# ESandML/SSL4GIE

Hardware: AMD Instinct MI355X
Metric: images/sec/GPU (fwd+bwd) ViT-B 224² bs=256 at 1/2/4/8 MI355X; % MFMA peak (higher is better)
Workload: dtype bf16; 1 GPU; ViT-B MAE pretrain (mae_vit_base_patch16, norm_pix_loss, mask 0.75) fwd+bwd+grad-allreduce+AdamW, 224x224 synthetic N(0,1) images resident in HBM; batch_per_gpu=256, global_batch=256, parallelism=dp1, optimizer=AdamW(0.9,0.95) wd 0.05 (ssl4gie_amd.optim.ArenaAdamW)

## Files before the change

### include/ssl4gie_hip.h

```cpp
#ifndef SSL4GIE_HIP_H
#define SSL4GIE_HIP_H
#include <stddef.h>
#include <stdint.h>
#ifdef __cplusplus
extern "C" {
#endif

#define SSL4GIE_F32 0
#define SSL4GIE_BF16 1
#define SSL4GIE_EARG 1000
#define SSL4GIE_EPEER 1001

int ssl4gie_abi_version(void);

int ssl4gie_layernorm_fwd(const float* x, const float* gamma, const float* beta, void* y,
                          int y_dtype, float* mean, float* rstd, int rows, int cols, float eps,
                          void* stream);
size_t ssl4gie_layernorm_bwd_workspace_bytes(int rows, int cols);
int ssl4gie_layernorm_bwd(const void* dy, int dy_dtype, const float* x, const float* gamma,
                          const float* mean, const float* rstd, const float* dres, float* dx,
                          void* dx_lp, int lp_dtype, float* dgamma, float* dbeta, int accumulate,
                          float* workspace, int rows, int cols, void* stream);

size_t ssl4gie_colsum_workspace_bytes(int rows, int cols);
int ssl4gie_colsum(const void* x, int dtype, float* out, int accumulate, float* workspace,
                   int rows, int cols, long long ld, void* stream);

enum {
    SSL4GIE_EPI_NONE = 0,
    SSL4GIE_EPI_BIAS = 1,
    SSL4GIE_EPI_BIAS_GELU = 2,
    SSL4GIE_EPI_BIAS_RESIDUAL = 3,
    SSL4GIE_EPI_DGELU = 4,
    SSL4GIE_EPI_BIAS_GELU_GRAD = 5,
    SSL4GIE_EPI_MUL_AUX = 6,
    SSL4GIE_EPI_RELU_MASK_AUX = 7,
    SSL4GIE_EPI_ADD_AUX = 8,
    SSL4GIE_EPI_AFFINE_AUX_RELU = 9
};
typedef struct ssl4gie_conv3x3_geom {
    int B, H, W, C;
    int stride;
    int relu;
} ssl4gie_conv3x3_geom;

typedef struct ssl4gie_gemm_desc {
    int M, N, K;
    int batch1, batch2;
    const void* A;
    long long sAm, sAk, sAb1, sAb2;
    const void* B;
    long long sBk, sBn, sBb1, sBb2;
    void* C;
    long long ldc, sCb1, sCb2;
    int dtype_ab;
    int dtype_c;
    float alpha;
    int epilogue;
    const float* bias;
    const float* residual;
    long long ldr;
    const void* aux;
    void* out2;
    int accumulate;
    float* colsum_a;
    const ssl4gie_conv3x3_geom* conv;
    float* colstats;
    const float* scale;
    int relu;
} ssl4gie_gemm_desc;
size_t ssl4gie_gemm_workspace_bytes(const ssl4gie_gemm_desc* d);
int ssl4gie_gemm(const ssl4gie_gemm_desc* d, void* workspace, size_t workspace_bytes,
                 void* stream);
size_t ssl4gie_gemm_tn_pair_workspace_bytes(const ssl4gie_gemm_desc* a, const ssl4gie_gemm_desc* b);
int ssl4gie_gemm_tn_pair(const ssl4gie_gemm_desc* a, const ssl4gie_gemm_desc* b, void* workspace,
                         size_t workspace_bytes, void* stream);
size_t ssl4gie_gemm_tn_group_workspace_bytes(const ssl4gie_gemm_desc* descs, int n);
int ssl4gie_gemm_tn_group(const ssl4gie_gemm_desc* descs, int n, void* workspace,
                          size_t workspace_bytes, void* stream);

size_t ssl4gie_attn_workspace_bytes(int dtype, int B, int N, int H, int hd);
int ssl4gie_attn_fwd(const void* qkv, void* out, float* lse, int dtype, int B, int N, int H,
                     int hd, void* workspace, void* stream);
int ssl4gie_attn_bwd(const void* qkv, const void* out, const void* dout, const float* lse,
                     void* dqkv, int dtype, int B, int N, int H, int hd, void* workspace,
                     void* stream);

int ssl4gie_cast(const float* src, void* dst, int dst_dtype, long long n, void* stream);
int ssl4gie_cast_transpose(const float* src, void* dst, int dst_dtype, int rows, int cols,
                           void* stream);
int ssl4gie_cast_transpose_batch(const float* src, void* dst, const long long* mat_off,
                                 const int* mat_rows, const int* mat_cols, const int* tile_start,
                                 int S, int total_tiles, void* stream);
int ssl4gie_add_cast(const float* a, const float* b, float* out, void* out_lp, int lp_dtype,
                     long long n, void* stream);

int ssl4gie_mask_argsort(const float* noise, long long* ids_shuffle, long long* ids_restore,
                         float* mask, int B, int L, int len_keep, void* stream);
int ssl4gie_patch_gather(const float* img, const long long* ids, void* out, int out_dtype,
                         int B, int C, int H, int W, int p, int nsel, long long ids_stride,
                         int order, void* stream);
int ssl4gie_tokens_assemble(const void* y, int y_dtype, const float* cls, const float* pos,
                            const long long* ids, long long ids_stride, float* x, int B,
                            int nsel, int D, void* stream);
int ssl4gie_tokens_assemble_bwd(const float* dx, void* dy, int dy_dtype, float* dcls,
                                int accumulate, int B, int nsel, int D, void* stream);
int ssl4gie_decoder_assemble(const void* y, int y_dtype, const float* mask_token,
                             const float* dpos, const long long* ids_restore, float* xd, int B,
                             int L, int nkeep, int D, void* stream);
size_t ssl4gie_decoder_assemble_bwd_workspace_bytes(int B, int L, int D);
int ssl4gie_decoder_assemble_bwd(const float* dxd, const long long* ids_shuffle, void* dy,
                                 int dy_dtype, float* dmask_token, int accumulate,
                                 float* workspace, int B, int L, int nkeep, int D, void* stream);
int ssl4gie_mae_loss(const float* pred, const float* img, const float* mask, float* per_patch,
                     float* dpred, const float* gpp, float gscale_host, int norm_pix,
                     int has_cls, int B, int C, int H, int W, int p, void* stream);

typedef struct ssl4gie_block_weights {
    const float *ln1_g, *ln1_b, *ln2_g, *ln2_b;
    const float *bqkv, *bproj, *bfc1, *bfc2;
    const void *wqkv, *wproj, *wfc1, *wfc2;
    const void *wqkv_t, *wproj_t, *wfc1_t, *wfc2_t;
} ssl4gie_block_weights;
typedef struct ssl4gie_block_grads {
    float *ln1_g, *ln1_b, *ln2_g, *ln2_b;
    float *bqkv, *bproj, *bfc1, *bfc2;
    float *wqkv, *wproj, *wfc1, *wfc2;
} ssl4gie_block_grads;
typedef struct ssl4gie_block_act {
    float *mean1, *rstd1, *mean2, *rstd2;
    void* h1;
    void* qkv;
    void* attn;
    float* lse;
    float* xmid;
    void* h2;
    void* u;
    void* g;
} ssl4gie_block_act;
typedef struct ssl4gie_block_dims {
    int B, N, D, H, F;
    int dtype;
    float eps;
} ssl4gie_block_dims;
size_t ssl4gie_block_workspace_bytes(const ssl4gie_block_dims* d);
int ssl4gie_block_fwd(const ssl4gie_block_dims* d, const ssl4gie_block_weights* w,
                      const ssl4gie_block_act* a, const float* x_in, float* x_out,
                      void* workspace, void* stream);
#define SSL4GIE_BWD_ACCUMULATE 1
#define SSL4GIE_BWD_NO_JOIN 4
#define SSL4GIE_BWD_SLOT(s) (((s) & 3) << 4)
int ssl4gie_block_bwd(const ssl4gie_block_dims* d, const ssl4gie_block_weights* w,
                      const ssl4gie_block_act* a, const ssl4gie_block_grads* g,
                      const float* x_in, const float* dx_out, const void* dx_out_lp,
                      float* dx_in, void* dx_in_lp, int accumulate, void* workspace,
                      void* stream);
size_t ssl4gie_block_dp_workspace_bytes(const ssl4gie_block_dims* d);
int ssl4gie_block_fwd_dp(const ssl4gie_block_dims* d, const ssl4gie_block_weights* w,
                         const ssl4gie_block_act* a, const float* x_in, float* x_out,
                         const float* s_attn, const float* s_mlp, void* workspace, void* stream);
int ssl4gie_block_bwd_dp(const ssl4gie_block_dims* d, const ssl4gie_block_weights* w,
                         const ssl4gie_block_act* a, const ssl4gie_block_grads* g,
                         const float* x_in, const float* dx_out, const void* dx_out_lp,
                         float* dx_in, void* dx_in_lp, const float* s_attn, const float* s_mlp,
                         int accumulate, void* workspace, void* stream);
int ssl4gie_drop_path_add(const float* res, const float* t, const float* s, float* out, int B,
                          long long per_sample, void* stream);
int ssl4gie_drop_path_scale_cast(const float* dx, const float* s, void* out, int out_dtype, int B,
                                 long long per_sample, void* stream);
int ssl4gie_mixup(float* x, const float* lam, const int* box, const unsigned char* use_cutmix, int B, int C,
                  int H, int W, void* stream);
int ssl4gie_mixup_target(const long long* target, const float* lam, float* out, int B, int C,
                         float on, float off, void* stream);
int ssl4gie_set_wgrad_stream(int on);
int ssl4gie_wgrad_wait(int slot, void* stream);
int ssl4gie_set_compute_cus(int n);

int ssl4gie_conv3x3_weight_pack(const float* w, void* out, int dtype, int Cout, int Cin, int mode, int ld,
                                void* stream);
int ssl4gie_conv3x3_weight_pack_batch(const void* const* w, void* const* out, const int* Cout, const int* Cin,
                                      const int* mode, const int* ld, int n, int dtype, void* stream);
int ssl4gie_conv3x3_wgrad_unpack(const float* dw2, float* dw, int Cout, int Cin, int ld, int accumulate,
                                 void* stream);
int ssl4gie_im2col3x3(const void* x, void* cols, int dtype, int B, int H, int W, int C, int stride,
                      int relu, long long ld, void* stream);
int ssl4gie_col2im3x3(const void* dcols, void* dx, int dtype, int B, int H, int W, int C,
                      int stride, long long ld, void* stream);
int ssl4gie_conv3x3_direct_ok(int B, int H, int W, int Cin, int Cout);
int ssl4gie_conv3x3_direct_tiles(int B, int H, int W);
int ssl4gie_conv3x3_direct_fwd(const void* x, const void* w2, const float* bias,
                               const void* relu_mask, void* y, float* colstats, int B, int H, int W,
                               int Cin, int Cout, int relu_in, void* stream);
int ssl4gie_conv3x3_direct_wgrad_ok(int B, int H, int W, int Cin, int Cout);
size_t ssl4gie_conv3x3_direct_wgrad_workspace_bytes(int B, int H, int W, int Cin, int Cout);
int ssl4gie_conv3x3_direct_wgrad(const void* dy, const void* x, float* dw2, float* dbias,
                                 void* workspace, size_t workspace_bytes, int B, int H, int W, int Cin,
                                 int Cout, int relu_in, int accumulate, void* stream);
size_t ssl4gie_stem7x7_packed_bytes(int B, int H, int W);
int ssl4gie_stem7x7_pack(const float* img, void* packed, int B, int H, int W, void* stream);
int ssl4gie_stem7x7_tiles(int B, int H, int W);
int ssl4gie_stem7x7_fwd(const void* packed, const void* w2s, void* y, float* colstats, int B, int H,
                        int W, void* stream);
size_t ssl4gie_stem7x7_wgrad_workspace_bytes(int B, int H, int W);
int ssl4gie_stem7x7_wgrad(const void* dy, const void* packed, float* dw2s, void* workspace,
                          size_t workspace_bytes, int B, int H, int W, int accumulate, void* stream);
int ssl4gie_stem3x3_tiles(int B, int H, int W);
int ssl4gie_stem3x3_fwd(const float* img, const float* weight, void* y, float* colstats, int dtype, int B,
                        int H, int W, int C0, void* stream);
size_t ssl4gie_stem3x3_wgrad_workspace_bytes(int dtype, int B, int H, int W, int C0);
int ssl4gie_stem3x3_wgrad(const void* dy, const float* img, float* dweight, void* workspace,
                          size_t workspace_bytes, int dtype, int B, int H, int W, int C0, int accumulate,
                          void* stream);
int ssl4gie_bilinear2x_fwd(const void* x, void* y, int dtype, int B, int H, int W, int C,
                           void* stream);
int ssl4gie_bilinear2x_bwd(const void* dy, void* dx, int dtype, int B, int H, int W, int C,
                           void* stream);
int ssl4gie_im2col3x3_dil(const void* x, void* cols, int dtype, int B, int H, int W, int C, int dilation,
                          long long ld, void* stream);
int ssl4gie_dwconv3x3_fwd(const void* x, const float* w, void* y, int dtype, int B, int H, int W, int C,
                          int dilation, int flip, void* stream);
size_t ssl4gie_dwconv3x3_wgrad_workspace_bytes(int dtype, int B, int H, int W, int C);
int ssl4gie_dwconv3x3_wgrad(const void* dy, const void* x, float* dweight, void* workspace, size_t workspace_bytes,
                            int dtype, int B, int H, int W, int C, int dilation, int accumulate, void* stream);
int ssl4gie_bilinear_up_ac_fwd(const void* x, void* y, int dtype, int B, int H, int W, int C, int scale,
                               void* stream);
int ssl4gie_bilinear_up_ac_bwd(const void* dy, void* dx, int dtype, int B, int H, int W, int C, int scale,
                               void* stream);
int ssl4gie_chan_copy(const void* src, long long lds, void* dst, long long ldd, int dtype, long long rows, int C,
                      long long rep, void* stream);
int ssl4gie_pixel_shuffle(const void* g, const float* bias, void* y, int dtype, int B, int H, int W,
                          int k, int C, void* stream);
int ssl4gie_pixel_unshuffle(const void* dy, void* dg, int dtype, int B, int H, int W, int k, int C,
                            void* stream);
int ssl4gie_tokens_to_map(const float* z, void* x, int dtype, int B, int L, int D, void* stream);
int ssl4gie_map_to_tokens(const void* dx, float* dz, int dtype, int B, int L, int D, void* stream);
int ssl4gie_eltwise(int op, const void* a, const void* b, const void* c, void* out, int dtype,
                    long long n, void* stream);
int ssl4gie_depth_head_fwd(const void* x, const float* w, const float* bias, float* y, int dtype,
                           long long M, int C, void* stream);
size_t ssl4gie_depth_head_bwd_workspace_bytes(long long M, int C);
int ssl4gie_depth_head_bwd(const void* x, const float* w, const float* y, const float* dy, void* dx,
                           float* dw, float* db, int accumulate, float* workspace, int dtype,
                           long long M, int C, void* stream);

int ssl4gie_stem_im2col7x7(const float* img, void* cols, int dtype, int B, int H, int W,
                           long long ld, void* stream);
int ssl4gie_subsample2(const void* x, void* y, int dtype, int B, int H, int W, int C, int backward,
                       void* stream);
enum { SSL4GIE_BN_FROM_X = 0, SSL4GIE_BN_FROM_PARTIALS = 1, SSL4GIE_BN_FROM_STATS = 2, SSL4GIE_BN_FROM_COEF = 3 };
enum { SSL4GIE_BN_MASK_NONE = 0, SSL4GIE_BN_MASK_Y = 1, SSL4GIE_BN_MASK_X = 2, SSL4GIE_BN_MASK_BITS = 3 };
size_t ssl4gie_bn_workspace_bytes(long long rows, int C);
int ssl4gie_bn_fwd(int source, const void* x, const float* partial, int parts, const float* gamma,
                   const float* beta, const void* res, void* y, unsigned char* relu_bits, float* coef, float* mean,
                   float* rstd, float* running_mean, float* running_var, float momentum, float eps, int relu,
                   float* workspace, int dtype, long long rows, int C, void* stream);
int ssl4gie_bn_stats(const void* x, const float* partial, int parts, float* mean, float* var, float* workspace,
                     int dtype, long long rows, int C, void* stream);
int ssl4gie_bn_bwd(const void* dy, int mask_kind, const void* mask, const void* x, const float* gamma,
                   const float* beta, const float* mean, const float* rstd, void* dx, void* dres, float* dgamma,
                   float* dbeta, int accumulate, float* workspace, int dtype, long long rows, int C, void* stream);
int ssl4gie_bn_bwd_reduce(const void* dy, int mask_kind, const void* mask, const void* x, const float* gamma,
                          const float* beta, const float* mean, const float* rstd, void* dres, float* sums,
                          float* workspace, int dtype, long long rows, int C, void* stream);
int ssl4gie_bn_bwd_apply(const void* dy, int mask_kind, const void* mask, const void* x, const float* gamma,
                         const float* beta, const float* mean, const float* rstd, const float* sums, float inv_count,
                         void* dx, float* workspace, int dtype, long long rows, int C, void* stream);
int ssl4gie_bn_combine_stats(const float* gathered, int world, int C, float eps, float momentum,
                             float* running_mean, float* running_var, float* mean, float* rstd, float* total,
                             void* stream);
int ssl4gie_ema_update(float* dst, const float* src, float m, long long n, void* stream);
int ssl4gie_maxpool3x3s2_fwd(const void* x, void* y, unsigned char* arg, int dtype, int B, int H,
                             int W, int C, void* stream);
int ssl4gie_maxpool3x3s2_bwd(const void* dy, const unsigned char* arg, void* dx, int dtype, int B,
                             int H, int W, int C, void* stream);
int ssl4gie_bn_maxpool3x3s2_fwd(const void* x, const float* coef, int relu, void* y, unsigned char* arg,
                                int dtype, int B, int H, int W, int C, void* stream);
int ssl4gie_avgpool_fwd(const void* x, float* y, int dtype, int B, int HW, int C, void* stream);
int ssl4gie_avgpool_bwd(const float* dy, void* dx, int dtype, int B, int HW, int C, void* stream);

int ssl4gie_adamw_arena(float* p, const float* g, float* m, float* v, const long long* seg_start,
                        const float* seg_lr, const float* seg_wd, int S, float beta1, float beta2,
                        float eps, int step, long long n, void* stream);
int ssl4gie_adamw_arena_lp(float* p, const float* g, float* m, float* v, const long long* seg_start,
                           const float* seg_lr, const float* seg_wd, int S, float beta1, float beta2,
                           float eps, int step, long long n, void* lp_bf16, void* stream);
int ssl4gie_adamw_arena_range(float* p, const float* g, float* m, float* v, const long long* seg_start,
                              const float* seg_lr, const float* seg_wd, int S, float beta1, float beta2,
                              float eps, int step, long long lo, long long hi, void* lp_bf16,
                              void* stream);
size_t ssl4gie_grad_norm_workspace_bytes(void);
int ssl4gie_grad_norm_arena(const float* g, const long long* seg_start, const float* seg_mask, int S,
                            float inv_scale, float max_norm, void* workspace, float* ctl, long long n,
                            void* stream);
int ssl4gie_grad_scale_arena(float* g, const long long* seg_start, const float* seg_mask, int S,
                             const float* ctl, long long n, void* stream);
int ssl4gie_adamw_arena_range_ctl(float* p, const float* g, float* m, float* v, const long long* seg_start,
                                  const float* seg_lr, const float* seg_wd, int S, float beta1, float beta2,
                                  float eps, int* applied, long long lo, long long hi, void* lp_bf16,
                                  const float* ctl, int skip_nonfinite, int advance, void* stream);
size_t ssl4gie_lars_workspace_bytes(int S);
int ssl4gie_lars_arena(float* p, const float* g, float* mu, const long long* seg_start,
                       const float* seg_lr, const float* seg_wd, const float* seg_mat, int S,
                       float momentum, float trust, float* workspace, long long n, void* stream);

int ssl4gie_normalize_u8(const unsigned char* img, float* out, const float* mean, const float* std,
                         int B, int H, int W, void* stream);
#define SSL4GIE_FILTER_BILINEAR 0
#define SSL4GIE_FILTER_BICUBIC 1
int ssl4gie_view_sample_u8(const unsigned char* bank, long long n, int Hs, int Ws, const long long* index,
                           const int* box, const unsigned char* flip, float* out, int B, int S, int filter,
                           const float* mean, const float* std, void* stream);
size_t ssl4gie_color_augment_workspace_bytes(int B, int S);
int ssl4gie_color_augment(const float* x, float* out, int B, int S, const float* factors,
                          const unsigned char* order, const unsigned char* flags, const float* sigma,
                          const float* mean, const float* std, void* workspace, size_t workspace_bytes,
                          void* stream);
int ssl4gie_color_augment_ft(const float* x, float* out, int B, int S, const float* factors,
                             const unsigned char* order, const unsigned char* flags, const float* sigma,
                             const float* mean, const float* std, void* workspace, size_t workspace_bytes,
                             void* stream);
#define SSL4GIE_TGT_U8 0
#define SSL4GIE_TGT_U16 1
#define SSL4GIE_TGT_F32 2
int ssl4gie_paired_warp(const float* img, float* img_out, const void* tgt_bank, int tgt_dtype, long n,
                        const int64_t* index, float* tgt_out, const float* matrix, const uint8_t* flip,
                        const float fill_img[3], float fill_tgt, int B, int S, void* stream);
size_t ssl4gie_det_color_workspace_bytes(int B);
int ssl4gie_det_color(const unsigned char* pixels, long long total, const long long* offsets, const int* sizes,
                      long long n, const long long* index, int B, int max_h, int max_w, const float* factors,
                      const unsigned char* order, const float* sigma, float* scratch, long long plane_stride,
                      void* workspace, size_t workspace_bytes, void* stream);
int ssl4gie_det_geometry(const float* scratch, long long plane_stride, const unsigned char* pixels, long long total,
                         const long long* offsets, const int* sizes, long long n, const long long* index,
                         const unsigned char* geom, float* out, int B, int F, const float* mean, const float* std,
                         void* stream);
int ssl4gie_det_boxes(const float* boxes, const long long* labels, const long long* box_offsets, long long m,
                      const int* sizes, long long n, const long long* index, const unsigned char* geom,
                      const long long* out_start, float* out_boxes, long long* out_labels, long long m_out, int B, int F,
                      int max_boxes, void* stream);

#define SSL4GIE_ERASE_CONST 0
#define SSL4GIE_ERASE_RAND 1
#define SSL4GIE_ERASE_PIXEL 2
int ssl4gie_quantize_u8(const float* x, unsigned char* out, int B, int S, void* stream);
size_t ssl4gie_randaug_layer_workspace_bytes(int B);
int ssl4gie_randaug_layer(const unsigned char* in, unsigned char* out, const unsigned char* op, const float* arg,
                          const double* matrix, const unsigned char* fill, void* workspace, int B, int S, void* stream);
int ssl4gie_normalize_erase_u8(const unsigned char* img, float* out, const float* mean, const float* std,
                               const int* box, int mode, unsigned long long seed, int B, int S, void* stream);

int ssl4gie_maxpool2x2_fwd(const void* x, void* y, int dtype, int B, int H, int W, int C,
                           void* stream);
int ssl4gie_maxpool2x2_bwd(const void* x, const void* dy, void* dx, int dtype, int B, int H, int W,
                           int C, void* stream);
int ssl4gie_gelu_map(const void* x, const void* dy, void* out, int dtype, long long n, void* stream);
size_t ssl4gie_map_layernorm_workspace_bytes(int B);
int ssl4gie_map_layernorm_fwd(const void* x, const float* w, const float* bias, void* y, float* mean,
                              float* rstd, float eps, float* workspace, int dtype, int B, long long M,
                              void* stream);
int ssl4gie_map_layernorm_bwd(const void* x, const void* dy, const float* w, const float* mean,
                              const float* rstd, void* dx, float* dw, float* db, int accumulate,
                              float* workspace, int dtype, int B, long long M, void* stream);

#define SSL4GIE_PROF_KINDS 7
int ssl4gie_prof_begin(int max_launches);
int ssl4gie_prof_collect(double* ms, double* flops, long long* launches);
int ssl4gie_prof_end(void);

size_t ssl4gie_ssi_loss_workspace_bytes(int B, int H, int W);
int ssl4gie_ssi_loss(const float* pred, const float* target, float* loss, float* dpred, int B, int H,
                     int W, float alpha, int scales, void* workspace, void* stream);
size_t ssl4gie_dice_loss_workspace_bytes(int B);
int ssl4gie_dice_loss(const float* logits, const float* target, float* loss, float* dlogits, int B,
                      long long n, float smooth, void* workspace, void* stream);

size_t ssl4gie_infonce_workspace_bytes(int N, int M, int C);
int ssl4gie_infonce_loss(const float* q, const float* k, float* loss, float* dq, int N, int M, int C, float T,
                         int label_offset, void* workspace, void* stream);
size_t ssl4gie_cross_entropy_workspace_bytes(int B, int C);
int ssl4gie_cross_entropy(const float* logits, const long long* target, const float* weight, float* loss,
                          float* dlogits, int B, int C, void* workspace, void* stream);
size_t ssl4gie_soft_cross_entropy_workspace_bytes(int B, int C);
int ssl4gie_soft_cross_entropy(const float* logits, const float* soft_target, const long long* label,
                               float conf, float off, float* loss, float* dlogits, int B, int C,
                               void* workspace, void* stream);
size_t ssl4gie_bt_loss_workspace_bytes(int D);
int ssl4gie_bt_loss(const float* c, float* loss, int D, float lambd, void* workspace, void* stream);
int ssl4gie_bt_loss_grad(const float* c, const float* scale, void* w, void* wt, int dtype, int D, float lambd,
                         void* stream);

#define SSL4GIE_PRED_I64 2
int ssl4gie_seg_counts(const void* logits, int logits_dtype, const void* target, int target_dtype, long long* counts,
                       int B, int Hin, int Win, int H, int W, int sigmoid, void* stream);
int ssl4gie_seg_scores(const long long* counts, int B, float smooth, float* scores, double* accum, void* stream);
int ssl4gie_confusion_update(const void* input, int input_kind, const long long* target, long long* conf,
                             long long* rejected, int B, int C, void* stream);
int ssl4gie_confusion_scores(const long long* conf, int C, float smooth, float* scores, void* stream);
size_t ssl4gie_lower_median_workspace_bytes(void);
int ssl4gie_lower_median_f32(const float* x, long long n, float* out, void* workspace, void* stream);
size_t ssl4gie_depth_eval_workspace_bytes(int B, int S, int H, int W);
int ssl4gie_depth_eval(const float* pred, const float* target, const float* target_og, float* out, int B, int Sh,
                       int Sw, int H, int W, float scale_, void* workspace, void* stream);

#define SSL4GIE_DET_MAP_MAX_PER_IMAGE 1024
#define SSL4GIE_DET_MAP_CLASSES 256
#define SSL4GIE_DET_MAP_CHUNK 256
#define SSL4GIE_DET_MAP_MAX_TOTAL (1 << 24)
size_t ssl4gie_det_map_workspace_bytes(int n_img, long long n_det, long long n_gt);
int ssl4gie_det_map_match(const float* det_boxes, const float* det_scores, const long long* det_labels,
                          const int* det_off, const float* gt_boxes, const long long* gt_labels, const int* gt_off,
                          int n_img, long long n_det, long long n_gt, const double* iou_thresholds, int* rank,
                          unsigned long long* matched, unsigned long long* ignored, int* npig, int* present, int* flag,
                          void* stream);
int ssl4gie_det_map_order(const float* det_scores, const long long* det_labels, const int* rank, long long n_det,
                          unsigned* sorted_idx, int* seg_off, void* workspace, void* stream);
int ssl4gie_det_map_accumulate(const unsigned* sorted_idx, const int* seg_off, const int* rank,
                               const unsigned long long* matched, const unsigned long long* ignored, const int* npig,
                               const int* present, const int* flag, long long n_det, const double* rec_thresholds,
                               double* stats, double* out64, float* out32, int* outi, void* stream);

#define SSL4GIE_NMS_MAX_PER_SEGMENT 4096
#define SSL4GIE_NMS_MAX_TOTAL (1 << 24)
#define SSL4GIE_RPN_MAX_LEVELS 8
#define SSL4GIE_RPN_MAX_ANCHORS 3
size_t ssl4gie_nms_workspace_bytes(long long n, int max_seg);
int ssl4gie_nms_segments(const float* boxes, const unsigned char* valid, const int* seg_off, int n_seg, long long n,
                         int max_seg, float thr, int* keep_rank, int* count, void* workspace, void* stream);
int ssl4gie_rpn_decode(const float* const* head, const int* grids, const int* k_off, const float* base_anchors, int L,
                       int A, int ld, const long long* topk_idx, int B, int F, float min_size, float score_thresh,
                       float* boxes, float* scores, unsigned char* valid, void* stream);
int ssl4gie_roi_decode(const float* proposals, const float* logits, int ld_logits, const float* deltas, int ld_deltas,
                       int K, int C, float wx, float wy, float ww, float wh, float W, float H, float min_size,
                       float score_thresh, float* boxes, float* scores, unsigned char* valid, void* stream);
int ssl4gie_roi_align_fwd(const float* const* maps, const int* map_hw, const float* scales, int B, int C,
                          const float* rois, const int* roi_batch, int K, void* out, int out_dtype, int* levels,
                          void* stream);
int ssl4gie_roi_align_bwd(float* const* dmaps, const int* map_hw, const float* scales, int B, int C, const float* rois,
                          const int* roi_batch, int K, const void* dy, int dy_dtype, void* stream);

typedef struct ssl4gie_ar_handle ssl4gie_ar_handle;
size_t ssl4gie_allreduce_direct_blob_bytes(void);
int ssl4gie_allreduce_direct_init(int rank, int world, size_t max_elems, void* export_blob,
                                  ssl4gie_ar_handle** out);
int ssl4gie_allreduce_direct_connect(ssl4gie_ar_handle* h, const void* all_blobs);
int ssl4gie_allreduce_direct_enqueue(ssl4gie_ar_handle* h, float* grad, size_t n_elems, float scale,
                                     void* stream);
int ssl4gie_allgather_direct_enqueue(ssl4gie_ar_handle* h, const float* src, size_t n_elems, float* dst,
                                     void* stream);
unsigned ssl4gie_allreduce_direct_error(const ssl4gie_ar_handle* h);
int ssl4gie_allreduce_direct_set_timeout(ssl4gie_ar_handle* h, double seconds);
int ssl4gie_allreduce_direct_destroy(ssl4gie_ar_handle* h);

// ... 5 lines not shown
```

### ssl4gie_amd/Models/mae/models_mae.py

```python
from __future__ import annotations

from functools import partial

import torch
import torch.nn as nn

from ... import ops
from ...engine import DecoderAssembleFn, EngineModule, MaeLossFn, PatchEmbedFn
from ..vit_layers import Block, PatchEmbed
from .util.pos_embed import get_2d_sincos_pos_embed


class MaskedAutoencoderViT(EngineModule):

    def __init__(self, img_size=224, patch_size=16, in_chans=3,
                 embed_dim=1024, depth=24, num_heads=16,
                 decoder_embed_dim=512, decoder_depth=8, decoder_num_heads=16,
                 mlp_ratio=4., norm_layer=nn.LayerNorm, norm_pix_loss=False):
        super().__init__()
        self.in_chans = in_chans
        self.num_heads = num_heads
        self.decoder_num_heads = decoder_num_heads

        self.patch_embed = PatchEmbed(img_size, patch_size, in_chans, embed_dim)
        n = self.patch_embed.num_patches
        self.cls_token = nn.Parameter(torch.zeros(1, 1, embed_dim))
        self.pos_embed = nn.Parameter(torch.zeros(1, n + 1, embed_dim), requires_grad=False)
        self.blocks = nn.ModuleList([Block(embed_dim, num_heads, mlp_ratio, qkv_bias=True,
                                           norm_layer=norm_layer) for _ in range(depth)])
        self.norm = norm_layer(embed_dim)

        self.decoder_embed = nn.Linear(embed_dim, decoder_embed_dim, bias=True)
        self.mask_token = nn.Parameter(torch.zeros(1, 1, decoder_embed_dim))
        self.decoder_pos_embed = nn.Parameter(torch.zeros(1, n + 1, decoder_embed_dim),
                                              requires_grad=False)
        self.decoder_blocks = nn.ModuleList([Block(decoder_embed_dim, decoder_num_heads, mlp_ratio,
                                                   qkv_bias=True, norm_layer=norm_layer)
                                             for _ in range(decoder_depth)])
        self.decoder_norm = norm_layer(decoder_embed_dim)
        self.decoder_pred = nn.Linear(decoder_embed_dim, patch_size ** 2 * in_chans, bias=True)

        self.norm_pix_loss = norm_pix_loss
        self.initialize_weights()

    def initialize_weights(self):
        grid = int(self.patch_embed.num_patches ** .5)
        with torch.no_grad():
            for name in ("pos_embed", "decoder_pos_embed"):
                prm = getattr(self, name)
                table = get_2d_sincos_pos_embed(prm.shape[-1], grid, cls_token=True)
                prm.copy_(torch.from_numpy(table).float().unsqueeze(0))
        w = self.patch_embed.proj.weight.data
        nn.init.xavier_uniform_(w.view(w.shape[0], -1))
        nn.init.normal_(self.cls_token, std=.02)
        nn.init.normal_(self.mask_token, std=.02)
        for m in self.modules():
            if isinstance(m, nn.Linear):
                nn.init.xavier_uniform_(m.weight)
                if m.bias is not None:
                    nn.init.zeros_(m.bias)
            elif isinstance(m, nn.LayerNorm):
                nn.init.ones_(m.weight)
                nn.init.zeros_(m.bias)

    def patchify(self, imgs):
        p = self.patch_embed.patch_size[0]
        assert imgs.shape[2] == imgs.shape[3] and imgs.shape[2] % p == 0
        n, c = imgs.shape[0], imgs.shape[1]
        out = ops.patch_gather(imgs.contiguous().float(), p, order=1)
        return out.view(n, -1, p * p * c)

    def unpatchify(self, x):
        p = self.patch_embed.patch_size[0]
        h = w = int(x.shape[1] ** .5)
        assert h * w == x.shape[1]
        c = x.shape[2] // (p * p)
        return x.reshape(x.shape[0], h, w, p, p, c).permute(0, 5, 1, 3, 2, 4).reshape(
            x.shape[0], c, h * p, w * p)

    def _masking(self, n, mask_ratio, device, noise=None):
        L = self.patch_embed.num_patches
        keep = int(L * (1 - mask_ratio))
        if noise is None:
            noise = torch.rand(n, L, device=device)
        noise = noise.to(device=device, dtype=torch.float32).contiguous()
        assert noise.shape == (n, L)
        ids_shuffle, ids_restore, mask = ops.mask_argsort(noise, keep)
        return ids_shuffle, ids_restore, mask, keep

    def random_masking(self, x, mask_ratio, noise=None):
        n, L, d = x.shape
        ids_shuffle, ids_restore, mask, keep = self._masking(n, mask_ratio, x.device, noise)
        idx = ids_shuffle[:, :keep].unsqueeze(-1).expand(-1, -1, d)
        return torch.gather(x, 1, idx), mask, ids_restore

    def forward_encoder(self, x, mask_ratio, noise=None):
        self._prepare()
        p = self.patch_embed.patch_size[0]
        assert x.shape[2] == self.patch_embed.img_size[0] and x.shape[3] == self.patch_embed.img_size[1]
        ids_shuffle, ids_restore, mask, keep = self._masking(x.shape[0], mask_ratio, x.device, noise)
        self._ids_shuffle = ids_shuffle
        tok = PatchEmbedFn.apply(x.float(), self.patch_embed.proj.weight, self.patch_embed.proj.bias,
                                 self.cls_token, self.pos_embed, ids_shuffle, keep, p, self.dtype_,
                                 self.sink(), self._lp)
        tok, _ = self._blocks(self.blocks, tok, self.num_heads, self.norm.eps)
        latent = self._ln(tok, self.norm)
        return latent, mask, ids_restore

    def forward_decoder(self, x, ids_restore, _full=False):
        self._prepare()
        keep = x.shape[1] - 1
        ids_shuffle = getattr(self, "_ids_shuffle", None)
        if ids_shuffle is None or ids_shuffle.shape != ids_restore.shape:
            ids_shuffle = torch.argsort(ids_restore, dim=1)
        if x.dtype != self.dtype_:
            x = x.to(self.dtype_)
        y = self._linear(x, self.decoder_embed)
        xd = DecoderAssembleFn.apply(y, self.mask_token, self.decoder_pos_embed, ids_restore,
                                     ids_shuffle, keep, self.sink())
        xd, _ = self._blocks(self.decoder_blocks, xd, self.decoder_num_heads, self.decoder_norm.eps)
        h = self._ln(xd, self.decoder_norm)
        full = self._linear(h, self.decoder_pred, out_dtype=torch.float32)
        return full if _full else full[:, 1:, :]

    def forward_loss(self, imgs, pred, mask):
        p = self.patch_embed.patch_size[0]
        per_patch = MaeLossFn.apply(pred, imgs.contiguous().float(), mask, p,
                                    bool(self.norm_pix_loss))
        return per_patch.sum() / mask.sum()

    def forward(self, imgs, mask_ratio=0.75, noise=None):
        latent, mask, ids_restore = self.forward_encoder(imgs, mask_ratio, noise=noise)
        full = self.forward_decoder(latent, ids_restore, _full=True)
        loss = self.forward_loss(imgs, full, mask)
        return loss, full[:, 1:, :], mask


def _mae(embed_dim, depth, num_heads, patch_size=16, **kwargs):
    return MaskedAutoencoderViT(patch_size=patch_size, embed_dim=embed_dim, depth=depth,
                                num_heads=num_heads, decoder_embed_dim=512, decoder_depth=8,
                                decoder_num_heads=16, mlp_ratio=4,
                                norm_layer=partial(nn.LayerNorm, eps=1e-6), **kwargs)


def mae_vit_base_patch16_dec512d8b(**kwargs):
    return _mae(768, 12, 12, **kwargs)


def mae_vit_large_patch16_dec512d8b(**kwargs):
    return _mae(1024, 24, 16, **kwargs)


def mae_vit_huge_patch14_dec512d8b(**kwargs):
    return _mae(1280, 32, 16, patch_size=14, **kwargs)


mae_vit_base_patch16 = mae_vit_base_patch16_dec512d8b
mae_vit_large_patch16 = mae_vit_large_patch16_dec512d8b
mae_vit_huge_patch14 = mae_vit_huge_patch14_dec512d8b
```

### ssl4gie_amd/_lib.py

```python
from __future__ import annotations

import ctypes as C
import os

_HERE = os.path.dirname(os.path.abspath(__file__))
LIB_PATH = os.path.join(_HERE, "libssl4gie_hip.so")
ABI_VERSION = 12

PROF_KINDS = 7

F32, BF16 = 0, 1
BWD_ACCUMULATE, BWD_NO_JOIN = 1, 4
EPI_NONE, EPI_BIAS, EPI_BIAS_GELU, EPI_BIAS_RESIDUAL, EPI_DGELU, EPI_BIAS_GELU_GRAD, EPI_MUL_AUX, \
    EPI_RELU_MASK_AUX, EPI_ADD_AUX, EPI_AFFINE_AUX_RELU = range(10)
BN_FROM_X, BN_FROM_PARTIALS, BN_FROM_STATS, BN_FROM_COEF = range(4)
FILTER_BILINEAR, FILTER_BICUBIC = 0, 1
TGT_U8, TGT_U16, TGT_F32 = range(3)
DET_MAP_MAX_PER_IMAGE, DET_MAP_CLASSES, DET_MAP_CHUNK = 1024, 256, 256
NMS_MAX_PER_SEGMENT = 4096
PRED_I64 = 2
ERASE_CONST, ERASE_RAND, ERASE_PIXEL = range(3)
BN_MASK_NONE, BN_MASK_Y, BN_MASK_X, BN_MASK_BITS = range(4)

vp, i32, i64, f32, sz = C.c_void_p, C.c_int, C.c_longlong, C.c_float, C.c_size_t


class Conv3x3Geom(C.Structure):
    _fields_ = [("B", i32), ("H", i32), ("W", i32), ("C", i32), ("stride", i32), ("relu", i32)]


class GemmDesc(C.Structure):
    _fields_ = [
        ("M", i32), ("N", i32), ("K", i32), ("batch1", i32), ("batch2", i32),
        ("A", vp), ("sAm", i64), ("sAk", i64), ("sAb1", i64), ("sAb2", i64),
        ("B", vp), ("sBk", i64), ("sBn", i64), ("sBb1", i64), ("sBb2", i64),
        ("C", vp), ("ldc", i64), ("sCb1", i64), ("sCb2", i64),
        ("dtype_ab", i32), ("dtype_c", i32), ("alpha", f32), ("epilogue", i32),
        ("bias", vp), ("residual", vp), ("ldr", i64), ("aux", vp), ("out2", vp),
        ("accumulate", i32), ("colsum_a", vp), ("conv", C.POINTER(Conv3x3Geom)),
        ("colstats", vp), ("scale", vp), ("relu", i32),
    ]


_W_F32 = ("ln1_g", "ln1_b", "ln2_g", "ln2_b", "bqkv", "bproj", "bfc1", "bfc2")
_W_LP = ("wqkv", "wproj", "wfc1", "wfc2", "wqkv_t", "wproj_t", "wfc1_t", "wfc2_t")
_G_ALL = _W_F32 + ("wqkv", "wproj", "wfc1", "wfc2")
_ACT = ("mean1", "rstd1", "mean2", "rstd2", "h1", "qkv", "attn", "lse", "xmid", "h2", "u", "g")


class BlockWeights(C.Structure):
    _fields_ = [(n, vp) for n in _W_F32 + _W_LP]


class BlockGrads(C.Structure):
    _fields_ = [(n, vp) for n in _G_ALL]


class BlockAct(C.Structure):
    _fields_ = [(n, vp) for n in _ACT]


class BlockDims(C.Structure):
    _fields_ = [("B", i32), ("N", i32), ("D", i32), ("H", i32), ("F", i32), ("dtype", i32),
                ("eps", f32)]


PROTOTYPES = {
    "ssl4gie_abi_version": (i32, []),
    "ssl4gie_layernorm_fwd": (i32, [vp, vp, vp, vp, i32, vp, vp, i32, i32, f32, vp]),
    "ssl4gie_layernorm_bwd_workspace_bytes": (sz, [i32, i32]),
    "ssl4gie_layernorm_bwd": (i32, [vp, i32, vp, vp, vp, vp, vp, vp, vp, i32, vp, vp, i32, vp,
                                    i32, i32, vp]),
    "ssl4gie_colsum_workspace_bytes": (sz, [i32, i32]),
    "ssl4gie_colsum": (i32, [vp, i32, vp, i32, vp, i32, i32, i64, vp]),
    "ssl4gie_gemm_workspace_bytes": (sz, [C.POINTER(GemmDesc)]),
    "ssl4gie_gemm": (i32, [C.POINTER(GemmDesc), vp, sz, vp]),
    "ssl4gie_attn_workspace_bytes": (sz, [i32, i32, i32, i32, i32]),
    "ssl4gie_attn_fwd": (i32, [vp, vp, vp, i32, i32, i32, i32, i32, vp, vp]),
    "ssl4gie_attn_bwd": (i32, [vp, vp, vp, vp, vp, i32, i32, i32, i32, i32, vp, vp]),
    "ssl4gie_cast": (i32, [vp, vp, i32, i64, vp]),
    "ssl4gie_cast_transpose": (i32, [vp, vp, i32, i32, i32, vp]),
    "ssl4gie_cast_transpose_batch": (i32, [vp, vp, vp, vp, vp, vp, i32, i32, vp]),
    "ssl4gie_add_cast": (i32, [vp, vp, vp, vp, i32, i64, vp]),
    "ssl4gie_mask_argsort": (i32, [vp, vp, vp, vp, i32, i32, i32, vp]),
    "ssl4gie_patch_gather": (i32, [vp, vp, vp, i32, i32, i32, i32, i32, i32, i32, i64, i32, vp]),
    "ssl4gie_tokens_assemble": (i32, [vp, i32, vp, vp, vp, i64, vp, i32, i32, i32, vp]),
    "ssl4gie_tokens_assemble_bwd": (i32, [vp, vp, i32, vp, i32, i32, i32, i32, vp]),
    "ssl4gie_decoder_assemble": (i32, [vp, i32, vp, vp, vp, vp, i32, i32, i32, i32, vp]),
    "ssl4gie_decoder_assemble_bwd_workspace_bytes": (sz, [i32, i32, i32]),
    "ssl4gie_decoder_assemble_bwd": (i32, [vp, vp, vp, i32, vp, i32, vp, i32, i32, i32, i32, vp]),
    "ssl4gie_mae_loss": (i32, [vp, vp, vp, vp, vp, vp, f32, i32, i32, i32, i32, i32, i32, i32, vp]),
    "ssl4gie_im2col3x3": (i32, [vp, vp, i32, i32, i32, i32, i32, i32, i32, i64, vp]),
    "ssl4gie_col2im3x3": (i32, [vp, vp, i32, i32, i32, i32, i32, i32, i64, vp]),
    "ssl4gie_conv3x3_direct_ok": (i32, [i32, i32, i32, i32, i32]),
    "ssl4gie_conv3x3_direct_tiles": (i32, [i32, i32, i32]),
    "ssl4gie_conv3x3_direct_fwd": (i32, [vp, vp, vp, vp, vp, vp, i32, i32, i32, i32, i32, i32, vp]),
    "ssl4gie_conv3x3_direct_wgrad_ok": (i32, [i32, i32, i32, i32, i32]),
    "ssl4gie_conv3x3_direct_wgrad_workspace_bytes": (sz, [i32, i32, i32, i32, i32]),
    "ssl4gie_conv3x3_direct_wgrad": (i32, [vp, vp, vp, vp, vp, sz, i32, i32, i32, i32, i32, i32, i32, vp]),
    "ssl4gie_stem7x7_packed_bytes": (sz, [i32, i32, i32]),
    "ssl4gie_stem7x7_pack": (i32, [vp, vp, i32, i32, i32, vp]),
    "ssl4gie_stem7x7_tiles": (i32, [i32, i32, i32]),
    "ssl4gie_stem7x7_fwd": (i32, [vp, vp, vp, vp, i32, i32, i32, vp]),
    "ssl4gie_stem7x7_wgrad_workspace_bytes": (sz, [i32, i32, i32]),
    "ssl4gie_stem7x7_wgrad": (i32, [vp, vp, vp, vp, sz, i32, i32, i32, i32, vp]),
    "ssl4gie_stem3x3_tiles": (i32, [i32, i32, i32]),
    "ssl4gie_stem3x3_fwd": (i32, [vp, vp, vp, vp, i32, i32, i32, i32, i32, vp]),
    "ssl4gie_stem3x3_wgrad_workspace_bytes": (sz, [i32, i32, i32, i32, i32]),
    "ssl4gie_stem3x3_wgrad": (i32, [vp, vp, vp, vp, sz, i32, i32, i32, i32, i32, i32, vp]),
    "ssl4gie_bilinear2x_fwd": (i32, [vp, vp, i32, i32, i32, i32, i32, vp]),
    "ssl4gie_bilinear2x_bwd": (i32, [vp, vp, i32, i32, i32, i32, i32, vp]),
    "ssl4gie_im2col3x3_dil": (i32, [vp, vp, i32, i32, i32, i32, i32, i32, i64, vp]),
    "ssl4gie_dwconv3x3_fwd": (i32, [vp, vp, vp, i32, i32, i32, i32, i32, i32, i32, vp]),
    "ssl4gie_dwconv3x3_wgrad_workspace_bytes": (sz, [i32, i32, i32, i32, i32]),
    "ssl4gie_dwconv3x3_wgrad": (i32, [vp, vp, vp, vp, sz, i32, i32, i32, i32, i32, i32, i32, vp]),
    "ssl4gie_bilinear_up_ac_fwd": (i32, [vp, vp, i32, i32, i32, i32, i32, i32, vp]),
    "ssl4gie_bilinear_up_ac_bwd": (i32, [vp, vp, i32, i32, i32, i32, i32, i32, vp]),
    "ssl4gie_chan_copy": (i32, [vp, i64, vp, i64, i32, i64, i32, i64, vp]),
    "ssl4gie_pixel_shuffle": (i32, [vp, vp, vp, i32, i32, i32, i32, i32, i32, vp]),
    "ssl4gie_pixel_unshuffle": (i32, [vp, vp, i32, i32, i32, i32, i32, i32, vp]),
    "ssl4gie_tokens_to_map": (i32, [vp, vp, i32, i32, i32, i32, vp]),
    "ssl4gie_map_to_tokens": (i32, [vp, vp, i32, i32, i32, i32, vp]),
    "ssl4gie_eltwise": (i32, [i32, vp, vp, vp, vp, i32, i64, vp]),
    "ssl4gie_depth_head_fwd": (i32, [vp, vp, vp, vp, i32, i64, i32, vp]),
    "ssl4gie_depth_head_bwd_workspace_bytes": (sz, [i64, i32]),
    "ssl4gie_depth_head_bwd": (i32, [vp, vp, vp, vp, vp, vp, vp, i32, vp, i32, i64, i32, vp]),
    "ssl4gie_stem_im2col7x7": (i32, [vp, vp, i32, i32, i32, i32, i64, vp]),
    "ssl4gie_subsample2": (i32, [vp, vp, i32, i32, i32, i32, i32, i32, vp]),
    "ssl4gie_bn_workspace_bytes": (sz, [i64, i32]),
    "ssl4gie_bn_fwd": (i32, [i32, vp, vp, i32, vp, vp, vp, vp, vp, vp, vp, vp, vp, vp, f32, f32, i32, vp, i32, i64, i32,
                             vp]),
    "ssl4gie_bn_stats": (i32, [vp, vp, i32, vp, vp, vp, i32, i64, i32, vp]),
    "ssl4gie_bn_bwd": (i32, [vp, i32, vp, vp, vp, vp, vp, vp, vp, vp, vp, vp, i32, vp, i32, i64, i32, vp]),
    "ssl4gie_bn_bwd_reduce": (i32, [vp, i32, vp, vp, vp, vp, vp, vp, vp, vp, vp, i32, i64, i32, vp]),
    "ssl4gie_bn_bwd_apply": (i32, [vp, i32, vp, vp, vp, vp, vp, vp, vp, f32, vp, vp, i32, i64, i32, vp]),
    "ssl4gie_ema_update": (i32, [vp, vp, f32, i64, vp]),
    "ssl4gie_maxpool3x3s2_fwd": (i32, [vp, vp, vp, i32, i32, i32, i32, i32, vp]),
    "ssl4gie_bn_maxpool3x3s2_fwd": (i32, [vp, vp, i32, vp, vp, i32, i32, i32, i32, i32, vp]),
    "ssl4gie_maxpool3x3s2_bwd": (i32, [vp, vp, vp, i32, i32, i32, i32, i32, vp]),
    "ssl4gie_avgpool_fwd": (i32, [vp, vp, i32, i32, i32, i32, vp]),
    "ssl4gie_avgpool_bwd": (i32, [vp, vp, i32, i32, i32, i32, vp]),
    "ssl4gie_adamw_arena": (i32, [vp, vp, vp, vp, vp, vp, vp, i32, f32, f32, f32, i32, i64, vp]),
    "ssl4gie_adamw_arena_lp": (i32, [vp, vp, vp, vp, vp, vp, vp, i32, f32, f32, f32, i32, i64, vp, vp]),
    "ssl4gie_adamw_arena_range": (i32, [vp, vp, vp, vp, vp, vp, vp, i32, f32, f32, f32, i32, i64, i64, vp, vp]),
    "ssl4gie_adamw_arena_range_ctl": (i32, [vp, vp, vp, vp, vp, vp, vp, i32, f32, f32, f32, vp, i64, i64, vp, vp,
                                            i32, i32, vp]),
    "ssl4gie_grad_norm_workspace_bytes": (sz, []),
    "ssl4gie_grad_norm_arena": (i32, [vp, vp, vp, i32, f32, f32, vp, vp, i64, vp]),
    "ssl4gie_grad_scale_arena": (i32, [vp, vp, vp, i32, vp, i64, vp]),
    "ssl4gie_lars_workspace_bytes": (sz, [i32]),
    "ssl4gie_lars_arena": (i32, [vp, vp, vp, vp, vp, vp, vp, i32, f32, f32, vp, i64, vp]),
    "ssl4gie_normalize_u8": (i32, [vp, vp, C.POINTER(C.c_float), C.POINTER(C.c_float), i32, i32, i32, vp]),
    "ssl4gie_view_sample_u8": (i32, [vp, i64, i32, i32, vp, vp, vp, vp, i32, i32, i32, C.POINTER(C.c_float),
                                     C.POINTER(C.c_float), vp]),
    "ssl4gie_quantize_u8": (i32, [vp, vp, i32, i32, vp]),
    "ssl4gie_randaug_layer_workspace_bytes": (sz, [i32]),
    "ssl4gie_randaug_layer": (i32, [vp, vp, vp, vp, vp, C.POINTER(C.c_ubyte), vp, i32, i32, vp]),
    "ssl4gie_normalize_erase_u8": (i32, [vp, vp, C.POINTER(C.c_float), C.POINTER(C.c_float), vp, i32, C.c_ulonglong, i32,
                                         i32, vp]),
    "ssl4gie_color_augment_workspace_bytes": (sz, [i32, i32]),
    "ssl4gie_color_augment": (i32, [vp, vp, i32, i32, vp, vp, vp, vp, C.POINTER(C.c_float), C.POINTER(C.c_float), vp, sz,
                                    vp]),
    "ssl4gie_color_augment_ft": (i32, [vp, vp, i32, i32, vp, vp, vp, vp, C.POINTER(C.c_float), C.POINTER(C.c_float), vp,
                                       sz, vp]),
    "ssl4gie_paired_warp": (i32, [vp, vp, vp, i32, C.c_long, vp, vp, vp, vp, C.POINTER(C.c_float), f32, i32, i32, vp]),
    "ssl4gie_det_color_workspace_bytes": (sz, [i32]),
    "ssl4gie_det_color": (i32, [vp, i64, vp, vp, i64, vp, i32, i32, i32, vp, vp, vp, vp, i64, vp, sz, vp]),
    "ssl4gie_det_geometry": (i32, [vp, i64, vp, i64, vp, vp, i64, vp, vp, vp, i32, i32, C.POINTER(C.c_float),
                                   C.POINTER(C.c_float), vp]),
    "ssl4gie_det_boxes": (i32, [vp, vp, vp, i64, vp, i64, vp, vp, vp, vp, vp, i64, i32, i32, i32, vp]),
    "ssl4gie_maxpool2x2_fwd": (i32, [vp, vp, i32, i32, i32, i32, i32, vp]),
    "ssl4gie_maxpool2x2_bwd": (i32, [vp, vp, vp, i32, i32, i32, i32, i32, vp]),
    "ssl4gie_gelu_map": (i32, [vp, vp, vp, i32, i64, vp]),
    "ssl4gie_map_layernorm_workspace_bytes": (sz, [i32]),
    "ssl4gie_map_layernorm_fwd": (i32, [vp, vp, vp, vp, vp, vp, f32, vp, i32, i32, i64, vp]),
    "ssl4gie_map_layernorm_bwd": (i32, [vp, vp, vp, vp, vp, vp, vp, vp, i32, vp, i32, i32, i64, vp]),
    "ssl4gie_gemm_tn_pair_workspace_bytes": (sz, [vp, vp]),
    "ssl4gie_gemm_tn_pair": (i32, [vp, vp, vp, sz, vp]),
    "ssl4gie_gemm_tn_group_workspace_bytes": (sz, [vp, i32]),
    "ssl4gie_gemm_tn_group": (i32, [vp, i32, vp, sz, vp]),
    "ssl4gie_wgrad_wait": (i32, [i32, vp]),
    "ssl4gie_set_wgrad_stream": (i32, [i32]),
    "ssl4gie_set_compute_cus": (i32, [i32]),
    "ssl4gie_ssi_loss_workspace_bytes": (sz, [i32, i32, i32]),
    "ssl4gie_ssi_loss": (i32, [vp, vp, vp, vp, i32, i32, i32, f32, i32, vp, vp]),
    "ssl4gie_dice_loss_workspace_bytes": (sz, [i32]),
    "ssl4gie_dice_loss": (i32, [vp, vp, vp, vp, i32, i64, f32, vp, vp]),
    "ssl4gie_infonce_workspace_bytes": (sz, [i32, i32, i32]),
    "ssl4gie_infonce_loss": (i32, [vp, vp, vp, vp, i32, i32, i32, f32, i32, vp, vp]),
    "ssl4gie_cross_entropy_workspace_bytes": (sz, [i32, i32]),
    "ssl4gie_cross_entropy": (i32, [vp, vp, vp, vp, vp, i32, i32, vp, vp]),
    "ssl4gie_bt_loss_workspace_bytes": (sz, [i32]),
    "ssl4gie_bt_loss": (i32, [vp, vp, i32, f32, vp, vp]),
    "ssl4gie_bt_loss_grad": (i32, [vp, vp, vp, vp, i32, i32, f32, vp]),
    "ssl4gie_seg_counts": (i32, [vp, i32, vp, i32, vp, i32, i32, i32, i32, i32, i32, vp]),
    "ssl4gie_seg_scores": (i32, [vp, i32, f32, vp, vp, vp]),
    "ssl4gie_confusion_update": (i32, [vp, i32, vp, vp, vp, i32, i32, vp]),
    "ssl4gie_confusion_scores": (i32, [vp, i32, f32, vp, vp]),
    "ssl4gie_lower_median_workspace_bytes": (sz, []),
    "ssl4gie_lower_median_f32": (i32, [vp, i64, vp, vp, vp]),
    "ssl4gie_depth_eval_workspace_bytes": (sz, [i32, i32, i32, i32]),
    "ssl4gie_depth_eval": (i32, [vp, vp, vp, vp, i32, i32, i32, i32, i32, f32, vp, vp]),
    "ssl4gie_det_map_workspace_bytes": (sz, [i32, i64, i64]),
    "ssl4gie_det_map_match": (i32, [vp, vp, vp, vp, vp, vp, vp, i32, i64, i64, C.POINTER(C.c_double), vp, vp, vp, vp, vp,
                                    vp, vp]),
    "ssl4gie_det_map_order": (i32, [vp, vp, vp, i64, vp, vp, vp, vp]),
    "ssl4gie_det_map_accumulate": (i32, [vp, vp, vp, vp, vp, vp, vp, vp, i64, C.POINTER(C.c_double), vp, vp, vp, vp,
                                         vp]),
    "ssl4gie_nms_workspace_bytes": (sz, [i64, i32]),
    "ssl4gie_nms_segments": (i32, [vp, vp, vp, i32, i64, i32, f32, vp, vp, vp, vp]),
    "ssl4gie_rpn_decode": (i32, [C.POINTER(vp), C.POINTER(i32), C.POINTER(i32), C.POINTER(f32), i32, i32, i32, vp, i32,
                                 i32, f32, f32, vp, vp, vp, vp]),
    "ssl4gie_roi_decode": (i32, [vp, vp, i32, vp, i32, i32, i32, f32, f32, f32, f32, f32, f32, f32, f32, vp, vp, vp, vp]),
    "ssl4gie_roi_align_fwd": (i32, [C.POINTER(vp), C.POINTER(i32), C.POINTER(f32), i32, i32, vp, vp, i32, vp, i32, vp,
                                    vp]),
    "ssl4gie_roi_align_bwd": (i32, [C.POINTER(vp), C.POINTER(i32), C.POINTER(f32), i32, i32, vp, vp, i32, vp, i32, vp]),
    "ssl4gie_allreduce_direct_blob_bytes": (sz, []),
    "ssl4gie_allreduce_direct_init": (i32, [i32, i32, sz, vp, C.POINTER(vp)]),
    "ssl4gie_allreduce_direct_connect": (i32, [vp, vp]),
    "ssl4gie_allreduce_direct_enqueue": (i32, [vp, vp, sz, f32, vp]),
    "ssl4gie_allgather_direct_enqueue": (i32, [vp, vp, sz, vp, vp]),
    "ssl4gie_bn_combine_stats": (i32, [vp, i32, i32, f32, f32, vp, vp, vp, vp, vp, vp]),
    "ssl4gie_allreduce_direct_error": (C.c_uint, [vp]),
    "ssl4gie_allreduce_direct_set_timeout": (i32, [vp, C.c_double]),
    "ssl4gie_allreduce_direct_destroy": (i32, [vp]),
    "ssl4gie_conv3x3_weight_pack_batch": (i32, [vp, vp, vp, vp, vp, vp, i32, i32, vp]),
    "ssl4gie_conv3x3_weight_pack": (i32, [vp, vp, i32, i32, i32, i32, i32, vp]),
    "ssl4gie_conv3x3_wgrad_unpack": (i32, [vp, vp, i32, i32, i32, i32, vp]),
    "ssl4gie_prof_begin": (i32, [i32]),
    "ssl4gie_prof_collect": (i32, [vp, vp, vp]),
    "ssl4gie_prof_end": (i32, []),
    "ssl4gie_block_workspace_bytes": (sz, [C.POINTER(BlockDims)]),
    "ssl4gie_block_fwd": (i32, [C.POINTER(BlockDims), C.POINTER(BlockWeights),
                                C.POINTER(BlockAct), vp, vp, vp, vp]),
    "ssl4gie_block_bwd": (i32, [C.POINTER(BlockDims), C.POINTER(BlockWeights),
                                C.POINTER(BlockAct), C.POINTER(BlockGrads), vp, vp, vp, vp, vp,
                                i32, vp, vp]),
    "ssl4gie_block_dp_workspace_bytes": (sz, [C.POINTER(BlockDims)]),
    "ssl4gie_block_fwd_dp": (i32, [C.POINTER(BlockDims), C.POINTER(BlockWeights),
                                   C.POINTER(BlockAct), vp, vp, vp, vp, vp, vp]),
    "ssl4gie_block_bwd_dp": (i32, [C.POINTER(BlockDims), C.POINTER(BlockWeights),
                                   C.POINTER(BlockAct), C.POINTER(BlockGrads), vp, vp, vp, vp, vp,
                                   vp, vp, i32, vp, vp]),
    "ssl4gie_drop_path_add": (i32, [vp, vp, vp, vp, i32, i64, vp]),
    "ssl4gie_drop_path_scale_cast": (i32, [vp, vp, vp, i32, i32, i64, vp]),
    "ssl4gie_mixup": (i32, [vp, vp, vp, vp, i32, i32, i32, i32, vp]),
    "ssl4gie_mixup_target": (i32, [vp, vp, vp, i32, i32, f32, f32, vp]),
    "ssl4gie_soft_cross_entropy_workspace_bytes": (sz, [i32, i32]),
    "ssl4gie_soft_cross_entropy": (i32, [vp, vp, vp, f32, f32, vp, vp, i32, i32, vp, vp]),
}

_lib = None


class HipExtensionMissing(RuntimeError):
    pass


def load():
    global _lib
    if _lib is not None:
        return _lib
    if not os.path.exists(LIB_PATH):
        raise HipExtensionMissing(
            f"{LIB_PATH} not found: build it with `make -C ssl4gie_amd/csrc` "
            "(or `python -c 'import __graft_entry__ as g; g.build()'`). "
            "ssl4gie_amd has no CPU / eager fallback.")
    lib = C.CDLL(LIB_PATH)
    for name, (res, args) in PROTOTYPES.items():
        fn = getattr(lib, name)
        fn.restype = res
        fn.argtypes = args
    got = lib.ssl4gie_abi_version()
    if got != ABI_VERSION:
        raise HipExtensionMissing(
            f"{LIB_PATH} has ABI revision {got}, this package binds revision {ABI_VERSION}: "
            "rebuild it (`make -C ssl4gie_amd/csrc`)")
    _lib = lib
    return lib


def check(rc: int, what: str):
    if rc != 0:
        kind = {1000: "invalid argument",
                1001: "a peer of the direct all-reduce did not arrive in time (sticky)"}.get(rc, f"hipError_t {rc}")
        raise RuntimeError(f"libssl4gie_hip: {what} failed ({kind})")
```

### ssl4gie_amd/csrc/mae_ops.hip

```cpp
#include "common.h"
#include "ssl4gie_hip.h"
#include "internal.h"

template <typename T>
__global__ void cast_kernel(const float* __restrict__ src, T* __restrict__ dst, long long n) {
    const long long i = ((long long)blockIdx.x * blockDim.x + threadIdx.x) * 4;
    if (i + 3 < n) {
        st4(dst + i, ld4(src + i));
    } else {
        for (long long j = i; j < n; ++j) Elem<T>::st(dst + j, src[j]);
    }
}
template <typename T>
__global__ __launch_bounds__(256) void cast_transpose_kernel(const float* __restrict__ src,
                                                             T* __restrict__ dst, int rows,
                                                             int cols) {
    __shared__ float tile[32][33];
    const int tx = threadIdx.x & 31, ty = threadIdx.x >> 5;
    const int r0 = blockIdx.y * 32, c0 = blockIdx.x * 32;
#pragma unroll
    for (int i = 0; i < 4; ++i) {
        const int r = r0 + ty + i * 8, c = c0 + tx;
        tile[ty + i * 8][tx] = (r < rows && c < cols) ? src[(size_t)r * cols + c] : 0.f;
    }
// ... 218 lines not shown
    if (B == 0) return 0;
    hipStream_t st = (hipStream_t)stream;
    dim3 grid(B * (nsel + 1)), block(D / 4 < 256 ? 64 * ((D / 4 + 63) / 64) : 256);
    if (y_dtype == SSL4GIE_BF16)
        hipLaunchKernelGGL(tokens_assemble_kernel<bf16_t>, grid, block, 0, st, (const bf16_t*)y,
                           cls, pos, ids, ids_stride, x, nsel, D);
    else if (y_dtype == SSL4GIE_F32)
        hipLaunchKernelGGL(tokens_assemble_kernel<float>, grid, block, 0, st, (const float*)y, cls,
                           pos, ids, ids_stride, x, nsel, D);
    else
        return ARG_ERR;
    LAUNCH_CHECK();
    return 0;
}

template <typename T>
__global__ void tokens_assemble_bwd_kernel(const float* __restrict__ dx, T* __restrict__ dy,
                                           int nsel, int D) {
    const int row = blockIdx.x;
    const int b = row / nsel, j = row % nsel;
    const float* s = dx + ((size_t)b * (nsel + 1) + 1 + j) * D;
    T* d = dy + (size_t)row * D;
    for (int k = threadIdx.x * 4; k < D; k += blockDim.x * 4) st4(d + k, ld4(s + k));
}
__global__ __launch_bounds__(1024) void strided_rowsum_kernel(const float* __restrict__ src, float* __restrict__ out,
                                                              int nrows, size_t stride, int D, int accumulate) {
    __shared__ float part[16][64];
    const int dl = threadIdx.x & 63, rg = threadIdx.x >> 6;
    const int d = blockIdx.x * 64 + dl;
    float s = 0.f;
    if (d < D)
        for (int b = rg; b < nrows; b += 16) s += src[(size_t)b * stride + d];
    part[rg][dl] = s;
    __syncthreads();
    if (rg == 0 && d < D) {
        float t = 0.f;
#pragma unroll
        for (int r = 0; r < 16; ++r) t += part[r][dl];
        out[d] = accumulate ? out[d] + t : t;
    }
}
extern "C" int ssl4gie_tokens_assemble_bwd(const float* dx, void* dy, int dy_dtype, float* dcls,
                                           int accumulate, int B, int nsel, int D, void* stream) {
    REQUIRE(dx && B >= 0 && nsel > 0 && D > 0 && D % 4 == 0);
    if (B == 0) return 0;
    hipStream_t st = (hipStream_t)stream;
    if (dy) {
        dim3 grid(B * nsel), block(D / 4 < 256 ? 64 * ((D / 4 + 63) / 64) : 256);
        if (dy_dtype == SSL4GIE_BF16)
            hipLaunchKernelGGL(tokens_assemble_bwd_kernel<bf16_t>, grid, block, 0, st, dx, (bf16_t*)dy, nsel, D);
        else if (dy_dtype == SSL4GIE_F32)
            hipLaunchKernelGGL(tokens_assemble_bwd_kernel<float>, grid, block, 0, st, dx, (float*)dy, nsel, D);
        else
            return ARG_ERR;
        LAUNCH_CHECK();
    }
    if (dcls) {
        hipLaunchKernelGGL(strided_rowsum_kernel, dim3((D + 63) / 64), dim3(1024), 0, st, dx, dcls,
                           B, (size_t)(nsel + 1) * D, D, accumulate);
        LAUNCH_CHECK();
    }
    return 0;
}

template <typename T>
__global__ void decoder_assemble_kernel(const T* __restrict__ y, const float* __restrict__ mtok,
                                        const float* __restrict__ dpos,
                                        const long long* __restrict__ ids_restore,
                                        float* __restrict__ xd, int L, int nkeep, int D) {
    const int row = blockIdx.x;
    const int b = row / (L + 1), t = row % (L + 1);
    float* xr = xd + (size_t)row * D;
    const float* pr = dpos + (size_t)t * D;
    const T* src = nullptr;
    if (t == 0) {
        src = y + (size_t)b * (nkeep + 1) * D;
    } else {
        const int r = (int)ids_restore[(size_t)b * L + t - 1];
        if (r < nkeep) src = y + ((size_t)b * (nkeep + 1) + 1 + r) * D;
    }
    for (int d = threadIdx.x * 4; d < D; d += blockDim.x * 4) {
        const f32x4 v = src ? ld4(src + d) : ld4(mtok + d);
        st4(xr + d, v + ld4(pr + d));
    }
}
extern "C" int ssl4gie_decoder_assemble(const void* y, int y_dtype, const float* mask_token,
                                        const float* dpos, const long long* ids_restore,
                                        float* xd, int B, int L, int nkeep, int D, void* stream) {
    REQUIRE(y && mask_token && dpos && ids_restore && xd && B >= 0 && L > 0 && nkeep >= 0);
    REQUIRE(nkeep <= L && D > 0 && D % 4 == 0);
    if (B == 0) return 0;
    hipStream_t st = (hipStream_t)stream;
    dim3 grid(B * (L + 1)), block(D / 4 < 256 ? 64 * ((D / 4 + 63) / 64) : 256);
    if (y_dtype == SSL4GIE_BF16)
        hipLaunchKernelGGL(decoder_assemble_kernel<bf16_t>, grid, block, 0, st, (const bf16_t*)y,
                           mask_token, dpos, ids_restore, xd, L, nkeep, D);
    else if (y_dtype == SSL4GIE_F32)
        hipLaunchKernelGGL(decoder_assemble_kernel<float>, grid, block, 0, st, (const float*)y,
                           mask_token, dpos, ids_restore, xd, L, nkeep, D);
    else
        return ARG_ERR;
    LAUNCH_CHECK();
    return 0;
}

#define DAB_Y 8
template <typename T>
__global__ void decoder_assemble_bwd_kernel(const float* __restrict__ dxd,
                                            const long long* __restrict__ ids_shuffle,
                                            T* __restrict__ dy, float* __restrict__ partial,
                                            int L, int nkeep, int D) {
    const int b = blockIdx.x, y = blockIdx.y;
    const float* base = dxd + (size_t)b * (L + 1) * D;
    T* dyb = dy + (size_t)b * (nkeep + 1) * D;
    for (int d = threadIdx.x * 4; d < D; d += blockDim.x * 4) {
        if (y == 0) st4(dyb + d, ld4(base + d));
        for (int j = y; j < nkeep; j += DAB_Y) {
            const int pos = (int)ids_shuffle[(size_t)b * L + j];
            st4(dyb + (size_t)(1 + j) * D + d, ld4(base + (size_t)(1 + pos) * D + d));
        }
        f32x4 acc = {0, 0, 0, 0};
        for (int j = nkeep + y; j < L; j += DAB_Y) {
            const int pos = (int)ids_shuffle[(size_t)b * L + j];
            acc += ld4(base + (size_t)(1 + pos) * D + d);
        }
        st4(partial + ((size_t)b * DAB_Y + y) * D + d, acc);
    }
}
extern "C" size_t ssl4gie_decoder_assemble_bwd_workspace_bytes(int B, int L, int D) {
    (void)L;
    return (size_t)B * DAB_Y * D * sizeof(float);
}
extern "C" int ssl4gie_decoder_assemble_bwd(const float* dxd, const long long* ids_shuffle,
                                            void* dy, int dy_dtype, float* dmask_token,
                                            int accumulate, float* workspace, int B, int L,
                                            int nkeep, int D, void* stream) {
    REQUIRE(dxd && ids_shuffle && dy && dmask_token && workspace && B >= 0 && L > 0);
    REQUIRE(nkeep >= 0 && nkeep <= L && D > 0 && D % 4 == 0);
    if (B == 0) return 0;
    hipStream_t st = (hipStream_t)stream;
    dim3 grid(B, DAB_Y), block(D / 4 < 256 ? 64 * ((D / 4 + 63) / 64) : 256);
    if (dy_dtype == SSL4GIE_BF16)
        hipLaunchKernelGGL(decoder_assemble_bwd_kernel<bf16_t>, grid, block, 0, st, dxd,
                           ids_shuffle, (bf16_t*)dy, workspace, L, nkeep, D);
    else if (dy_dtype == SSL4GIE_F32)
        hipLaunchKernelGGL(decoder_assemble_bwd_kernel<float>, grid, block, 0, st, dxd,
                           ids_shuffle, (float*)dy, workspace, L, nkeep, D);
    else
        return ARG_ERR;
    LAUNCH_CHECK();
    return ssl4gie_internal_reduce_partials(workspace, dmask_token, B * DAB_Y, D, (size_t)D, accumulate, st);
}

template <int NV>
__global__ __launch_bounds__(256) void mae_loss_kernel(
    const float* __restrict__ pred, const float* __restrict__ img, const float* __restrict__ mask,
    float* __restrict__ per_patch, float* __restrict__ dpred, const float* __restrict__ gpp,
    float gscale_host, int norm_pix, int has_cls, int B, int C, int H, int W, int p) {
    const int lane = threadIdx.x & 63;
    const int gw = W / p, L = (H / p) * gw, P = C * p * p, R = L + has_cls;
    const long long row = (long long)blockIdx.x * 4 + (threadIdx.x >> 6);
    if (row >= (long long)B * R) return;
    const int b = (int)(row / R), t = (int)(row % R);
    float* dr = dpred ? dpred + (size_t)row * P : nullptr;
    if (has_cls && t == 0) {
        if (dr)
            for (int k = 4 * lane; k < P; k += 256) st4(dr + k, f32x4{0.f, 0.f, 0.f, 0.f});
        return;
    }
    const int l = t - has_cls, gy = l / gw, gx = l % gw;
    const float* ib = img + (size_t)b * C * H * W + (size_t)(gy * p) * W + gx * p;
    const float* pr = pred + (size_t)row * P;
    f32x4 tv[NV], pv[NV];
    float s = 0.f;
#pragma unroll
    for (int i = 0; i < NV; ++i) {
        const int k = 4 * lane + 256 * i;
        tv[i] = f32x4{0.f, 0.f, 0.f, 0.f};
        pv[i] = f32x4{0.f, 0.f, 0.f, 0.f};
        if (k < P) {
            pv[i] = ld4(pr + k);
#pragma unroll
            for (int j = 0; j < 4; ++j) {
                const int kk = k + j, c = kk % C, pix = kk / C, py = pix / p, px = pix - py * p;
                tv[i][j] = ib[((size_t)c * H + py) * W + px];
            }
            s += (tv[i][0] + tv[i][1]) + (tv[i][2] + tv[i][3]);
        }
    }
    if (norm_pix) {
        const float mean = wave_sum(s) / (float)P;
        float q = 0.f;
#pragma unroll
        for (int i = 0; i < NV; ++i)
            if (4 * lane + 256 * i < P) {
                const f32x4 d = tv[i] - mean;
                q += (d[0] * d[0] + d[1] * d[1]) + (d[2] * d[2] + d[3] * d[3]);
            }
        const float inv = rsqrtf(wave_sum(q) / (float)(P - 1) + 1.0e-6f);
#pragma unroll
        for (int i = 0; i < NV; ++i) tv[i] = (tv[i] - mean) * inv;
    }
    const float m = mask[(size_t)b * L + l];
    float e = 0.f;
#pragma unroll
    for (int i = 0; i < NV; ++i)
        if (4 * lane + 256 * i < P) {
            const f32x4 d = pv[i] - tv[i];
            e += (d[0] * d[0] + d[1] * d[1]) + (d[2] * d[2] + d[3] * d[3]);
        }
    e = wave_sum(e) / (float)P;
    if (per_patch && lane == 0) per_patch[(size_t)b * L + l] = e * m;
    if (dr) {
        const float gs = gscale_host * (gpp ? gpp[(size_t)b * L + l] : 1.f) * m * 2.0f / (float)P;
#pragma unroll
        for (int i = 0; i < NV; ++i)
            if (4 * lane + 256 * i < P) st4(dr + 4 * lane + 256 * i, (pv[i] - tv[i]) * gs);
    }
}
extern "C" int ssl4gie_mae_loss(const float* pred, const float* img, const float* mask,
                                float* per_patch, float* dpred, const float* gpp,
                                float gscale_host, int norm_pix, int has_cls, int B, int C, int H,
                                int W, int p, void* stream) {
    REQUIRE(pred && img && mask && B >= 0 && C > 0 && p > 0 && H % p == 0 && W % p == 0);
    REQUIRE(has_cls == 0 || has_cls == 1);
    const int P = C * p * p;
    REQUIRE(P <= 64 * 16 && P % 4 == 0);
    if (B == 0) return 0;
    const long long rows = (long long)B * ((H / p) * (W / p) + has_cls);
    dim3 grid((unsigned)((rows + 3) / 4)), block(256);
    hipStream_t st = (hipStream_t)stream;
    if (P <= 64 * 4)
        hipLaunchKernelGGL(mae_loss_kernel<1>, grid, block, 0, st, pred, img, mask, per_patch, dpred,
                           gpp, gscale_host, norm_pix, has_cls, B, C, H, W, p);
    else if (P <= 64 * 12)
        hipLaunchKernelGGL(mae_loss_kernel<3>, grid, block, 0, st, pred, img, mask, per_patch,
                           dpred, gpp, gscale_host, norm_pix, has_cls, B, C, H, W, p);
    else
        hipLaunchKernelGGL(mae_loss_kernel<4>, grid, block, 0, st, pred, img, mask, per_patch,
                           dpred, gpp, gscale_host, norm_pix, has_cls, B, C, H, W, p);
    LAUNCH_CHECK();
    return 0;
}


__global__ void normalize_u8_kernel(const unsigned char* __restrict__ img, float* __restrict__ out,
                                    f32x4 scale, f32x4 shift, int HW, long long total4) {
    const long long idx = (long long)blockIdx.x * blockDim.x + threadIdx.x;
    if (idx >= total4) return;
    const long long b = idx / (HW / 4);
    const int p = (int)(idx % (HW / 4)) * 4;
    const unsigned* src = (const unsigned*)(img + ((size_t)b * HW + p) * 3);
    const unsigned w0 = src[0], w1 = src[1], w2 = src[2];
    unsigned char px[12];
#pragma unroll
    for (int j = 0; j < 4; ++j) { px[j] = (w0 >> (8 * j)) & 0xff; px[4 + j] = (w1 >> (8 * j)) & 0xff; px[8 + j] = (w2 >> (8 * j)) & 0xff; }
#pragma unroll
    for (int c = 0; c < 3; ++c) {
        f32x4 v;
#pragma unroll
        for (int j = 0; j < 4; ++j) v[j] = (float)px[3 * j + c] * scale[c] + shift[c];
        st4(out + ((size_t)b * 3 + c) * HW + p, v);
    }
}
extern "C" int ssl4gie_normalize_u8(const unsigned char* img, float* out, const float* mean,
                                    const float* std, int B, int H, int W, void* stream) {
    REQUIRE(img && out && mean && std && B > 0 && H > 0 && W > 0 && ((long long)H * W) % 4 == 0);
    for (int c = 0; c < 3; ++c) REQUIRE(std[c] > 0.f);
    const int HW = H * W;
    const long long total4 = (long long)B * (HW / 4);
    f32x4 scale = {1.f / (255.f * std[0]), 1.f / (255.f * std[1]), 1.f / (255.f * std[2]), 0.f};
    f32x4 shift = {-mean[0] / std[0], -mean[1] / std[1], -mean[2] / std[2], 0.f};
    hipLaunchKernelGGL(normalize_u8_kernel, dim3((unsigned)((total4 + 255) / 256)), dim3(256), 0,
                       (hipStream_t)stream, img, out, scale, shift, HW, total4);
    LAUNCH_CHECK();
    return 0;
}
```

### ssl4gie_amd/csrc/optim_ops.hip

```cpp
#include "reduce.h"
#include "ssl4gie_hip.h"

namespace {
DEVI int find_seg(const long long* __restrict__ seg_start, int S, long long i) {
    int lo = 0, hi = S;
    while (hi - lo > 1) {
        const int mid = (lo + hi) >> 1;
        if (seg_start[mid] <= i) lo = mid;
        else hi = mid;
    }
    return lo;
}
DEVI int block_seg(const long long* __restrict__ seg_start, int S, long long i, long long block_first) {
    __shared__ int s0;
    if (threadIdx.x == 0) s0 = find_seg(seg_start, S, block_first);
    __syncthreads();
    int s = s0;
    while (s + 1 < S && seg_start[s + 1] <= i) ++s;
    return s;
}
}

template <bool CTL>
__global__ __launch_bounds__(256) void adamw_arena_kernel(
    float* __restrict__ p, const float* __restrict__ g, float* __restrict__ m, float* __restrict__ v,
    const long long* __restrict__ seg_start, const float* __restrict__ seg_lr,
    const float* __restrict__ seg_wd, int S, float b1, float b2, float eps, float bc1, float rsqrt_bc2,
    long long n, bf16_t* __restrict__ lp, long long lo, const float* __restrict__ ctl,
    const int* __restrict__ applied, int skip) {
    __shared__ float bc[2];
    float coef = 1.f;
    if (CTL) {
        if (skip && ctl[2] != 0.f) return;
        coef = ctl[1];
        if (threadIdx.x == 0) {
            const float t = (float)(*applied + 1);
            bc[0] = 1.f - powf(b1, t);
            bc[1] = 1.f / sqrtf(1.f - powf(b2, t));
        }
    }
    const long long first = lo + (long long)blockIdx.x * blockDim.x * 4;
    const long long i = first + threadIdx.x * 4;
    const int s = block_seg(seg_start, S, i < n ? i : n - 4, first);
    if (i >= n) return;
    const float lr = seg_lr[s];
    if (lr < 0.f) return;
    if (CTL) { bc1 = bc[0]; rsqrt_bc2 = bc[1]; }
    const float wd = seg_wd[s];
    f32x4 pp = ld4(p + i), mm = ld4(m + i), vv = ld4(v + i);
    f32x4 gg = ld4(g + i);
    if (CTL) gg *= coef;
    const float step = lr / bc1;
#pragma unroll
    for (int j = 0; j < 4; ++j) {
        float x = pp[j] * (1.f - lr * wd);
        const float mj = b1 * mm[j] + (1.f - b1) * gg[j];
        const float vj = b2 * vv[j] + (1.f - b2) * gg[j] * gg[j];
        x -= step * mj / (sqrtf(vj) * rsqrt_bc2 + eps);
        pp[j] = x; mm[j] = mj; vv[j] = vj;
    }
    st4(p + i, pp);
    st4(m + i, mm);
    st4(v + i, vv);
    if (lp) st4(lp + i, pp);
}
__global__ void adamw_advance_kernel(int* __restrict__ applied, const float* __restrict__ ctl, int skip) {
    if (!(skip && ctl[2] != 0.f)) *applied += 1;
}

#define GN_BLOCKS 2048
__global__ __launch_bounds__(256) void grad_norm_partial_kernel(
    const float* __restrict__ g, const long long* __restrict__ seg_start,
    const float* __restrict__ seg_mask, int S, float inv_scale, long long n, long long per_block,
    double* __restrict__ part_sum, int* __restrict__ part_bad) {
    __shared__ double red[4];
    __shared__ int redb[4];
    f32x4 acc = {0.f, 0.f, 0.f, 0.f};
    unsigned bad = 0;
    const long long lo = (long long)blockIdx.x * per_block;
    const long long hi = lo + per_block < n ? lo + per_block : n;
    long long i = lo + threadIdx.x * 4;
    if (i < hi) {
        int s = find_seg(seg_start, S, i);
        long long next = seg_start[s + 1];
        bool active = seg_mask[s] >= 0.f;
        for (; i < hi; i += 4096) {
            bool on[4];
#pragma unroll
            for (int u = 0; u < 4; ++u) {
                const long long k = i + u * 1024;
                on[u] = false;
                if (k < hi) {
                    while (k >= next && s + 1 < S) {
                        ++s;
                        next = seg_start[s + 1];
                        active = seg_mask[s] >= 0.f;
                    }
                    on[u] = active;
                }
            }
            f32x4 gg[4];
#pragma unroll
            for (int u = 0; u < 4; ++u) {
                gg[u] = f32x4{0.f, 0.f, 0.f, 0.f};
                if (on[u]) gg[u] = ld4(g + i + u * 1024);
            }
#pragma unroll
            for (int u = 0; u < 4; ++u)
#pragma unroll
                for (int j = 0; j < 4; ++j) {
                    bad |= ((__float_as_uint(gg[u][j]) & 0x7f800000u) == 0x7f800000u);
                    const float x = inv_scale * gg[u][j];
                    acc[j] += x * x;
                }
        }
    }
    double a = ((double)acc[0] + (double)acc[1]) + ((double)acc[2] + (double)acc[3]);
#pragma unroll
    for (int o = 32; o > 0; o >>= 1) a += __shfl_xor(a, o, 64);
    const int wbad = __any((int)bad);
    if ((threadIdx.x & 63) == 0) { red[threadIdx.x >> 6] = a; redb[threadIdx.x >> 6] = wbad; }
    __syncthreads();
    if (threadIdx.x == 0) {
        part_sum[blockIdx.x] = block_get<SumOrder::Pairwise>(red);
        part_bad[blockIdx.x] = (redb[0] | redb[1] | redb[2] | redb[3]) != 0;
    }
}
__global__ __launch_bounds__(256) void grad_norm_final_kernel(
    const double* __restrict__ part_sum, const int* __restrict__ part_bad, float max_norm,
    float* __restrict__ ctl) {
    __shared__ double red[4];
    __shared__ int redb[4];
    double a = 0.0;
    int bad = 0;
    for (int k = threadIdx.x; k < GN_BLOCKS; k += 256) {
        a += part_sum[k];
        bad |= part_bad[k];
    }
#pragma unroll
    for (int o = 32; o > 0; o >>= 1) a += __shfl_xor(a, o, 64);
    bad = __any(bad);
    if ((threadIdx.x & 63) == 0) { red[threadIdx.x >> 6] = a; redb[threadIdx.x >> 6] = bad; }
    __syncthreads();
    if (threadIdx.x == 0) {
        const float norm = (float)sqrt(block_get<SumOrder::Pairwise>(red));
        float coef = 1.f;
        if (max_norm > 0.f) {
            coef = max_norm / (norm + 1e-6f);
            coef = coef > 1.f ? 1.f : coef;
        }
        ctl[0] = norm;
        ctl[1] = coef;
        ctl[2] = (redb[0] | redb[1] | redb[2] | redb[3]) ? 1.f : 0.f;
        ctl[3] = 0.f;
    }
}
__global__ __launch_bounds__(256) void grad_scale_kernel(
    float* __restrict__ g, const long long* __restrict__ seg_start, const float* __restrict__ seg_mask,
    int S, const float* __restrict__ ctl, long long n) {
    const float coef = ctl[1];
    if (coef == 1.f) return;
    const long long first = (long long)blockIdx.x * blockDim.x * 4;
    const long long i = first + threadIdx.x * 4;
    const int s = block_seg(seg_start, S, i < n ? i : n - 4, first);
    if (i >= n) return;
    if (seg_mask[s] < 0.f) return;
    st4(g + i, ld4(g + i) * coef);
}

#define LARS_PARTS 32
__global__ __launch_bounds__(256) void lars_norm_partial_kernel(
    const float* __restrict__ p, const float* __restrict__ g, const long long* __restrict__ seg_start,
    const float* __restrict__ seg_lr, const float* __restrict__ seg_wd, const float* __restrict__ seg_mat,
    float* __restrict__ partial) {
    __shared__ float red[2][4];
    const int s = blockIdx.y, part = blockIdx.x;
    float a = 0.f, b = 0.f;
    if (seg_lr[s] >= 0.f && seg_mat[s] != 0.f) {
        const long long lo = seg_start[s], hi = seg_start[s + 1];
        const float wd = seg_wd[s];
        for (long long i = lo + ((long long)part * 256 + threadIdx.x) * 4; i < hi; i += (long long)LARS_PARTS * 1024) {
            const f32x4 pp = ld4(p + i), gg = ld4(g + i);
#pragma unroll
            for (int j = 0; j < 4; ++j) {
                const float d = gg[j] + wd * pp[j];
                a += pp[j] * pp[j];
                b += d * d;
            }
        }
    }
    a = wave_sum(a);
    b = wave_sum(b);
    block_put(a, red[0]); block_put(b, red[1]);
    __syncthreads();
    if (threadIdx.x == 0) {
        partial[((size_t)s * LARS_PARTS + part) * 2] = block_get<SumOrder::Sequential>(red[0]);
        partial[((size_t)s * LARS_PARTS + part) * 2 + 1] = block_get<SumOrder::Sequential>(red[1]);
    }
}
__global__ void lars_trust_kernel(const float* __restrict__ partial, const float* __restrict__ seg_mat,
                                  float* __restrict__ q, float trust, int S) {
    const int s = blockIdx.x * blockDim.x + threadIdx.x;
    if (s >= S) return;
    float a = 0.f, b = 0.f;
    for (int k = 0; k < LARS_PARTS; ++k) {
        a += partial[((size_t)s * LARS_PARTS + k) * 2];
        b += partial[((size_t)s * LARS_PARTS + k) * 2 + 1];
    }
    const float pn = sqrtf(a), un = sqrtf(b);
    q[s] = (seg_mat[s] != 0.f && pn > 0.f && un > 0.f) ? trust * pn / un : 1.f;
}
__global__ __launch_bounds__(256) void lars_apply_kernel(
    float* __restrict__ p, const float* __restrict__ g, float* __restrict__ mu,
    const long long* __restrict__ seg_start, const float* __restrict__ seg_lr,
    const float* __restrict__ seg_wd, const float* __restrict__ seg_mat, const float* __restrict__ q,
    int S, float momentum, long long n) {
    const long long first = (long long)blockIdx.x * blockDim.x * 4;
    const long long i = first + threadIdx.x * 4;
    const int s = block_seg(seg_start, S, i < n ? i : n - 4, first);
    if (i >= n) return;
    const float lr = seg_lr[s];
    if (lr < 0.f) return;
    const bool mat = seg_mat[s] != 0.f;
    const float wd = mat ? seg_wd[s] : 0.f, qq = mat ? q[s] : 1.f;
    f32x4 pp = ld4(p + i), mm = ld4(mu + i);
    const f32x4 gg = ld4(g + i);
#pragma unroll
    for (int j = 0; j < 4; ++j) {
        const float dp = (gg[j] + wd * pp[j]) * qq;
        mm[j] = momentum * mm[j] + dp;
        pp[j] -= lr * mm[j];
    }
    st4(p + i, pp);
    st4(mu + i, mm);
}

extern "C" int ssl4gie_adamw_arena_range(float* p, const float* g, float* m, float* v,
                                         const long long* seg_start, const float* seg_lr,
                                         const float* seg_wd, int S, float beta1, float beta2, float eps,
                                         int step, long long lo, long long hi, void* lp_bf16,
                                         void* stream) {
    REQUIRE(p && g && m && v && seg_start && seg_lr && seg_wd && S > 0 && step > 0 && lo >= 0 && hi >= lo &&
            lo % 4 == 0 && hi % 4 == 0);
    if (hi == lo) return 0;
    const float bc1 = 1.f - powf(beta1, (float)step), bc2 = 1.f - powf(beta2, (float)step);
    hipLaunchKernelGGL(adamw_arena_kernel<false>, dim3((unsigned)(((hi - lo) / 4 + 255) / 256)), dim3(256), 0,
                       (hipStream_t)stream, p, g, m, v, seg_start, seg_lr, seg_wd, S, beta1, beta2, eps,
                       bc1, 1.f / sqrtf(bc2), hi, (bf16_t*)lp_bf16, lo, (const float*)nullptr,
                       (const int*)nullptr, 0);
    LAUNCH_CHECK();
    return 0;
}
extern "C" int ssl4gie_adamw_arena_range_ctl(float* p, const float* g, float* m, float* v,
                                             const long long* seg_start, const float* seg_lr,
                                             const float* seg_wd, int S, float beta1, float beta2,
                                             float eps, int* applied, long long lo, long long hi,
                                             void* lp_bf16, const float* ctl, int skip_nonfinite,
                                             int advance, void* stream) {
    REQUIRE(p && g && m && v && seg_start && seg_lr && seg_wd && S > 0 && applied && ctl && lo >= 0 &&
            hi >= lo && lo % 4 == 0 && hi % 4 == 0);
    if (hi > lo) {
        hipLaunchKernelGGL(adamw_arena_kernel<true>, dim3((unsigned)(((hi - lo) / 4 + 255) / 256)), dim3(256),
                           0, (hipStream_t)stream, p, g, m, v, seg_start, seg_lr, seg_wd, S, beta1, beta2,
                           eps, 0.f, 0.f, hi, (bf16_t*)lp_bf16, lo, ctl, (const int*)applied,
                           skip_nonfinite != 0);
        LAUNCH_CHECK();
    }
    if (advance) {
        hipLaunchKernelGGL(adamw_advance_kernel, dim3(1), dim3(1), 0, (hipStream_t)stream, applied, ctl,
                           skip_nonfinite != 0);
        LAUNCH_CHECK();
    }
    return 0;
}
extern "C" size_t ssl4gie_grad_norm_workspace_bytes(void) {
    return (size_t)GN_BLOCKS * (sizeof(double) + sizeof(int));
}
extern "C" int ssl4gie_grad_norm_arena(const float* g, const long long* seg_start, const float* seg_mask,
                                       int S, float inv_scale, float max_norm, void* workspace,
                                       float* ctl, long long n, void* stream) {
    REQUIRE(g && seg_start && seg_mask && S > 0 && workspace && ctl && n > 0 && n % 4 == 0 &&
            (uintptr_t)workspace % 8 == 0);
    double* part_sum = (double*)workspace;
    int* part_bad = (int*)(part_sum + GN_BLOCKS);
    const long long per_block = ((n + 1023) / 1024 + GN_BLOCKS - 1) / GN_BLOCKS * 1024;
    hipLaunchKernelGGL(grad_norm_partial_kernel, dim3(GN_BLOCKS), dim3(256), 0, (hipStream_t)stream, g,
                       seg_start, seg_mask, S, inv_scale, n, per_block, part_sum, part_bad);
    LAUNCH_CHECK();
    hipLaunchKernelGGL(grad_norm_final_kernel, dim3(1), dim3(256), 0, (hipStream_t)stream,
                       (const double*)part_sum, (const int*)part_bad, max_norm, ctl);
    LAUNCH_CHECK();
    return 0;
}
extern "C" int ssl4gie_grad_scale_arena(float* g, const long long* seg_start, const float* seg_mask, int S,
                                        const float* ctl, long long n, void* stream) {
    REQUIRE(g && seg_start && seg_mask && S > 0 && ctl && n > 0 && n % 4 == 0);
    hipLaunchKernelGGL(grad_scale_kernel, dim3((unsigned)((n / 4 + 255) / 256)), dim3(256), 0,
                       (hipStream_t)stream, g, seg_start, seg_mask, S, ctl, n);
    LAUNCH_CHECK();
    return 0;
}
extern "C" int ssl4gie_adamw_arena_lp(float* p, const float* g, float* m, float* v,
                                      const long long* seg_start, const float* seg_lr,
                                      const float* seg_wd, int S, float beta1, float beta2, float eps,
                                      int step, long long n, void* lp_bf16, void* stream) {
    REQUIRE(n >= 0);
    return ssl4gie_adamw_arena_range(p, g, m, v, seg_start, seg_lr, seg_wd, S, beta1, beta2, eps, step, 0, n,
                                     lp_bf16, stream);
}
extern "C" int ssl4gie_adamw_arena(float* p, const float* g, float* m, float* v,
                                   const long long* seg_start, const float* seg_lr,
                                   const float* seg_wd, int S, float beta1, float beta2, float eps,
                                   int step, long long n, void* stream) {
    return ssl4gie_adamw_arena_lp(p, g, m, v, seg_start, seg_lr, seg_wd, S, beta1, beta2, eps, step, n,
                                  nullptr, stream);
}
extern "C" size_t ssl4gie_lars_workspace_bytes(int S) {
    return ((size_t)S * LARS_PARTS * 2 + S) * sizeof(float);
}
extern "C" int ssl4gie_lars_arena(float* p, const float* g, float* mu, const long long* seg_start,
                                  const float* seg_lr, const float* seg_wd, const float* seg_mat, int S,
                                  float momentum, float trust, float* workspace, long long n,
                                  void* stream) {
    REQUIRE(p && g && mu && seg_start && seg_lr && seg_wd && seg_mat && workspace && S > 0 && S <= 65535 &&
            n >= 0 && n % 4 == 0);
    if (n == 0) return 0;
    hipStream_t st = (hipStream_t)stream;
    float* partial = workspace;
    float* q = workspace + (size_t)S * LARS_PARTS * 2;
    hipLaunchKernelGGL(lars_norm_partial_kernel, dim3(LARS_PARTS, S), dim3(256), 0, st, p, g, seg_start,
                       seg_lr, seg_wd, seg_mat, partial);
    LAUNCH_CHECK();
    hipLaunchKernelGGL(lars_trust_kernel, dim3((S + 255) / 256), dim3(256), 0, st, partial, seg_mat, q,
                       trust, S);
    LAUNCH_CHECK();
    hipLaunchKernelGGL(lars_apply_kernel, dim3((unsigned)((n / 4 + 255) / 256)), dim3(256), 0, st, p, g, mu,
                       seg_start, seg_lr, seg_wd, seg_mat, q, S, momentum, n);
    LAUNCH_CHECK();
    return 0;
}
```

### ssl4gie_amd/engine.py

```python
from __future__ import annotations

import ctypes as C
import contextlib
import os
import weakref
from dataclasses import dataclass
from typing import Callable, List, Optional, Sequence

import torch
import torch.nn as nn

from . import _lib, ops
from ._lib import BlockAct, BlockDims, BlockGrads, BlockWeights


def default_dtype():
    v = os.environ.get("SSL4GIE_PRECISION", "bf16").lower()
    return torch.float32 if v in ("fp32", "f32", "float32") else torch.bfloat16


def _align(n, a=256):
    return (n + a - 1) // a * a


_ARENAS = weakref.WeakSet()


def arena_of(params):
    params = list(params)
    if not params:
        return None
    for a in list(_ARENAS):
        if all(a.owns(p) for p in params):
            return a
    return None


class ParamArena:

    def __init__(self, params: Sequence[nn.Parameter]):
        params = [p for p in params]
        assert params, "no parameters"
        dev = params[0].device
        self.params = params
        self.offsets = []
        off = 0
        for p in params:
            assert p.dtype == torch.float32 and p.device == dev
            self.offsets.append(off)
            off += _align(p.numel(), 64)
        self.numel = off
        self.data = torch.zeros(off, dtype=torch.float32, device=dev)
        self.grad = torch.zeros(off, dtype=torch.float32, device=dev)
        self._index = {}
        with torch.no_grad():
            for p, o in zip(params, self.offsets):
                v = self._shaped(self.data[o:o + p.numel()], p)
                v.copy_(p.data)
                p.data = v
                self._index[id(p)] = o
        self.device = dev
        self._grad_norm_state = None
        _ARENAS.add(self)

    @staticmethod
    def _shaped(flat, p):
        if p.ndim == 3 and not p.is_contiguous() and p.permute(1, 2, 0).is_contiguous():
            C, H, W = p.shape
            return flat.view(H, W, C).permute(2, 0, 1)
        return flat.view(p.shape)

    def owns(self, p) -> bool:
        o = self._index.get(id(p))
        return o is not None and p.data_ptr() == self.data.data_ptr() + 4 * o

    def intact(self) -> bool:
        return all(self.owns(p) for p in self.params)

    def grad_view(self, p) -> torch.Tensor:
        o = self._index[id(p)]
        return self._shaped(self.grad[o:o + p.numel()], p)

    def lp_views(self, p, dtype):
        assert dtype == torch.bfloat16
        if getattr(self, "_lp_stamp", None) != weights_epoch():
            self._refresh_lp()
        o = self._index[id(p)]
        rows = p.shape[0]
        cols = p.numel() // rows
        return (self._lp[o:o + p.numel()].view(rows, cols), self._lpt[o:o + p.numel()].view(cols, rows))

    def lp_flat_for_update(self):
        if getattr(self, "_lp_stamp", None) != weights_epoch():
            self._refresh_lp()
        return self._lp

    def lp_flat_is_current(self):
        self._lp_flat_stamp = weights_epoch()
        self._lp_flat_versions = [p._version for p in self.params]

    def _refresh_lp(self):
        L = _lib.load()
        if getattr(self, "_lp", None) is None:
            self._lp = torch.empty(self.numel, dtype=torch.bfloat16, device=self.device)
            self._lpt = torch.zeros(self.numel, dtype=torch.bfloat16, device=self.device)
            mats = [(o, p.shape[0], p.numel() // p.shape[0]) for p, o in zip(self.params, self.offsets)
                    if p.ndim >= 2]
            starts = [0]
            for _, r, c in mats:
                starts.append(starts[-1] + ((r + 63) // 64) * ((c + 63) // 64))
            dev = self.device
            self._lp_tab = (torch.tensor([m[0] for m in mats], dtype=torch.int64, device=dev),
                            torch.tensor([m[1] for m in mats], dtype=torch.int32, device=dev),
                            torch.tensor([m[2] for m in mats], dtype=torch.int32, device=dev),
                            torch.tensor(starts, dtype=torch.int32, device=dev), len(mats), starts[-1])
        flat_ok = getattr(self, "_lp_flat_stamp", None) == weights_epoch() and \
            getattr(self, "_lp_flat_versions", None) == [p._version for p in self.params]
        if not flat_ok:
            _lib.check(L.ssl4gie_cast(ops.ptr(self.data), ops.ptr(self._lp), _lib.BF16, self.numel,
                                      ops.stream()), "cast(arena)")
        off, rows, cols, ts, S, total = self._lp_tab
        if S:
            _lib.check(L.ssl4gie_cast_transpose_batch(ops.ptr(self.data), ops.ptr(self._lpt), ops.ptr(off),
                                                      ops.ptr(rows), ops.ptr(cols), ops.ptr(ts), S, total,
                                                      ops.stream()), "cast_transpose_batch")
        self._lp_stamp = weights_epoch()
        self._lp_versions = {id(p): p._version for p in self.params}

    def span(self, params: Sequence[nn.Parameter]):
        os_ = [self._index[id(p)] for p in params]
        ends = [self._index[id(p)] + _align(p.numel(), 64) for p in params]
        return min(os_), max(ends)


_WEIGHTS_EPOCH = [0]


def weights_epoch() -> int:
    return _WEIGHTS_EPOCH[0]


_EPOCH_TOUCHED = {}


def bump_weights_epoch(touched=None):
    _WEIGHTS_EPOCH[0] += 1
    _EPOCH_TOUCHED[_WEIGHTS_EPOCH[0]] = None if touched is None else frozenset(id(p) for p in touched)
    for e in [e for e in _EPOCH_TOUCHED if e < _WEIGHTS_EPOCH[0] - 16]:
        del _EPOCH_TOUCHED[e]


def touched_since(epoch: int):
    out = set()
    for e in range(epoch + 1, _WEIGHTS_EPOCH[0] + 1):
        t = _EPOCH_TOUCHED.get(e, None)
        if t is None:
            return None
        out |= t
    return out


try:
    from torch.optim.optimizer import register_optimizer_step_post_hook as _reg_post_hook
    _reg_post_hook(lambda opt, _args, _kwargs: bump_weights_epoch(
        touched=[p for g in opt.param_groups for p in g["params"]]))
except ImportError:
    pass


class LPCache:

    def __init__(self, arena_fn=None):
        self._c = {}
        self._arena_fn = arena_fn
        self._conv_recipes, self._conv_epoch = {}, None

    def get(self, p: torch.Tensor, dtype, need_t: bool = True):
        w2d = p.detach()
        w2d = w2d.view(w2d.shape[0], -1)
        if dtype == torch.float32:
            return w2d, None
        key = id(p)
        ver = (p._version, p.data_ptr(), dtype, weights_epoch())
        ent = self._c.get(key)
        if ent is None or ent[0] != ver or ent[3]() is not p:
            a = self._arena_fn() if self._arena_fn is not None else None
            if a is not None and dtype == torch.bfloat16 and a.owns(p):
                w, wt = a.lp_views(p, dtype)
                if a._lp_versions.get(key) != p._version:
                    ops.cast(w2d, dtype, out=w)
                    ops.cast_transpose(w2d, dtype, out=wt)
                    a._lp_versions[key] = p._version
            else:
                w = ops.cast(w2d, dtype)
                wt = ops.cast_transpose(w2d, dtype)
            ent = (ver, w, wt, weakref.ref(p))
            self._c[key] = ent
        return ent[1], ent[2]

    def derived(self, params, tag: str, dtype, fn, recipe=None):
        ps = params if isinstance(params, tuple) else (params,)
        key = (id(ps[0]), tag)
        ver = (tuple((p._version, p.data_ptr()) for p in ps), dtype, weights_epoch())
        if recipe is not None and key not in self._conv_recipes:
            self._conv_recipes[key] = (weakref.ref(ps[0]), recipe[0], recipe[1], dtype)
        ent = self._c.get(key)
        if ent is None or ent[0] != ver:
            with torch.no_grad():
                t = fn(*[p.detach() for p in ps])
                if isinstance(t, torch.Tensor):
                    t = ops.cast(t.contiguous(), dtype) if t.dtype != dtype else t.contiguous()
            ent = self._c[key] = (ver, t)
        return ent[1]

    def refresh_conv_operands(self):
        epoch = weights_epoch()
        seen = self._conv_epoch
        if not self._conv_recipes or seen == epoch:
            return
        self._conv_epoch = epoch
        moved = touched_since(seen) if seen is not None else None
        items, dead = [], []
        for key, (ref, mode, ld, dtype) in self._conv_recipes.items():
            p = ref()
            if p is None:
                dead.append(key)
                continue
            ver = (((p._version, p.data_ptr()),), dtype, epoch)
            ent = self._c.get(key)
            if ent is not None and ent[0] == ver:
                continue
            if ent is not None and moved is not None and key[0] not in moved and ent[0][:2] == ver[:2]:
                self._c[key] = (ver, ent[1])
                continue
            if not p.is_cuda or p.dtype != torch.float32 or not p.is_contiguous() or p.dim() != 4:
                continue
            items.append((key, ver, p, mode, ld, dtype))
        for key in dead:
            self._conv_recipes.pop(key, None)
            self._c.pop(key, None)
        for dtype in {it[5] for it in items}:
            group = [it for it in items if it[5] == dtype]
            outs = ops.conv3x3_weight_pack_batch([it[2].detach() for it in group], dtype, [it[3] for it in group],
                                                 [it[4] for it in group])
            for it, t in zip(group, outs):
                self._c[it[0]] = (it[1], t)


_GLOBAL_LP = LPCache()


class GradSink:

    def __init__(self, arena: Optional[ParamArena]):
        self.arena = arena
        self._written = set()
        self.tracker = None

    def note_done(self, params):
        if self.tracker is not None:
            self.tracker(params)

    def new_pass(self):
        self._written.clear()

    def plan(self, params: Sequence[Optional[torch.Tensor]]):
        live = [p for p in params if p is not None and p.requires_grad]
        arena = self.arena
        if arena is not None and all(arena.owns(p) for p in live):
            views = {id(p): arena.grad_view(p) for p in live}
            tg = [views[id(p)] if (p is not None and p.requires_grad) else None for p in params]
            has = [p.grad is not None for p in live]
            if live and all(has):
                if not all(p.grad.data_ptr() == views[id(p)].data_ptr() for p in live):
                    raise RuntimeError("p.grad was replaced by a tensor outside the gradient arena")
                return tg, True, [None] * len(params)
            if any(has):
                raise RuntimeError("mixed .grad state (some None, some set) is not supported")
            seen = [id(p) in self._written for p in live]
            if live and all(seen):
                return tg, True, [None] * len(params)
            if any(seen):
                raise RuntimeError("parameters of one node were written by different earlier nodes")
            self._written.update(id(p) for p in live)
            return tg, False, list(tg)
        tg = [torch.empty_like(p) if (p is not None and p.requires_grad) else None for p in params]
        return tg, False, list(tg)


BLOCK_PARAM_ORDER = ("norm1.weight", "norm1.bias", "attn.qkv.weight", "attn.qkv.bias",
                     "attn.proj.weight", "attn.proj.bias", "norm2.weight", "norm2.bias",
                     "mlp.fc1.weight", "mlp.fc1.bias", "mlp.fc2.weight", "mlp.fc2.bias")
_NP = len(BLOCK_PARAM_ORDER)


@dataclass
class StackCfg:
    heads: int
    eps: float
    dtype: torch.dtype
    taps: tuple
    need_bwd: bool
    sink: GradSink
    lp: LPCache
    on_block_grads: Optional[Callable[[int], None]] = None
    drop: Optional[tuple] = None


def _block_params(blk):
    return [blk.norm1.weight, blk.norm1.bias, blk.attn.qkv.weight, blk.attn.qkv.bias,
            blk.attn.proj.weight, blk.attn.proj.bias, blk.norm2.weight, blk.norm2.bias,
            blk.mlp.fc1.weight, blk.mlp.fc1.bias, blk.mlp.fc2.weight, blk.mlp.fc2.bias]


def _weights_struct(ps, cfg: StackCfg) -> tuple:
    n1w, n1b, wqkv, bqkv, wproj, bproj, n2w, n2b, wfc1, bfc1, wfc2, bfc2 = ps
    keep = []
    w = BlockWeights()
    w.ln1_g, w.ln1_b, w.ln2_g, w.ln2_b = (ops.ptr(t) for t in (n1w, n1b, n2w, n2b))
    w.bqkv, w.bproj, w.bfc1, w.bfc2 = (ops.ptr(t) for t in (bqkv, bproj, bfc1, bfc2))
    for name, p in (("wqkv", wqkv), ("wproj", wproj), ("wfc1", wfc1), ("wfc2", wfc2)):
        a, at = cfg.lp.get(p, cfg.dtype)
        keep += [a, at]
        setattr(w, name, ops.ptr(a))
        setattr(w, name + "_t", ops.ptr(at))
    return w, keep


class _ActArena:

    def __init__(self, B, N, D, H, F, es):
        T = B * N
        self.sizes = [("mean1", T * 4), ("rstd1", T * 4), ("mean2", T * 4), ("rstd2", T * 4),
                      ("h1", T * D * es), ("qkv", T * 3 * D * es), ("attn", T * D * es),
                      ("lse", B * H * N * 4), ("xmid", T * D * 4), ("h2", T * D * es),
                      ("u", T * F * es), ("g", T * F * es)]
        self.total = sum(_align(s) for _, s in self.sizes)

    def struct(self, base_ptr: int) -> BlockAct:
        a = BlockAct()
        off = 0
        for name, s in self.sizes:
            setattr(a, name, base_ptr + off)
            off += _align(s)
        return a


class BlockStackFn(torch.autograd.Function):

    @staticmethod
    def forward(ctx, x, cfg: StackCfg, *params):
        L = _lib.load()
        depth = len(params) // _NP
        B, N, D = x.shape
        F = params[8].shape[0]
        assert x.dtype == torch.float32 and x.is_cuda
        assert D % cfg.heads == 0 and params[2].shape == (3 * D, D)
        x = x.contiguous()
        es = 2 if cfg.dtype == torch.bfloat16 else 4
        dims = BlockDims(B, N, D, cfg.heads, F, ops.code(cfg.dtype), float(cfg.eps))
        drop = cfg.drop
        if drop is not None:
            scales, use = drop
            assert scales.is_cuda and scales.dtype == torch.float32 and scales.is_contiguous() and \
                tuple(scales.shape) == (depth, 2, B) and len(use) == depth, "drop_scales: fp32 device [depth, 2, B]"
            sptr = [(scales[i, 0].data_ptr(), scales[i, 1].data_ptr()) if use[i] else (0, 0) for i in range(depth)]
        wsb = (L.ssl4gie_block_dp_workspace_bytes if drop is not None else L.ssl4gie_block_workspace_bytes)(C.byref(dims))
        assert wsb > 0
        ws = torch.empty(wsb, dtype=torch.uint8, device=x.device)
        layout = _ActArena(B, N, D, cfg.heads, F, es)
        nact = depth if cfg.need_bwd else 1
        acts = torch.empty(nact * layout.total, dtype=torch.uint8, device=x.device)
        xs = [x]
        keepalive = []
        wstructs = []
        st = ops.stream()
        for i in range(depth):
            w, keep = _weights_struct(params[i * _NP:(i + 1) * _NP], cfg)
            keepalive += keep
            wstructs.append(w)
            a = layout.struct(acts.data_ptr() + (i if cfg.need_bwd else 0) * layout.total)
            xo = torch.empty_like(x)
            if drop is not None:
                _lib.check(L.ssl4gie_block_fwd_dp(C.byref(dims), C.byref(w), C.byref(a), xs[-1].data_ptr(),
                                                  xo.data_ptr(), sptr[i][0], sptr[i][1], ws.data_ptr(), st),
                           f"block_fwd_dp[{i}]")
            else:
                _lib.check(L.ssl4gie_block_fwd(C.byref(dims), C.byref(w), C.byref(a), xs[-1].data_ptr(),
                                               xo.data_ptr(), ws.data_ptr(), st), f"block_fwd[{i}]")
            xs.append(xo)
        outs = [xs[depth]] + [xs[t + 1] for t in cfg.taps]
        if cfg.need_bwd:
            ctx.cfg, ctx.dims, ctx.layout = cfg, dims, layout
            ctx.acts, ctx.xs, ctx.ws = acts, xs, ws
            ctx.wstructs, ctx.keepalive = wstructs, keepalive
            ctx.params = params
            ctx.depth = depth
            ctx.sptr = sptr if drop is not None else None
        return tuple(outs)

    @staticmethod
    def backward(ctx, *gouts):
        L = _lib.load()
        cfg, dims, layout, depth = ctx.cfg, ctx.dims, ctx.layout, ctx.depth
        x0 = ctx.xs[0]
        lp = cfg.dtype if cfg.dtype != torch.float32 else None
        tap_g = {t: g for t, g in zip(cfg.taps, gouts[1:]) if g is not None}
        st = ops.stream()
        targets, accumulate, returns = cfg.sink.plan(ctx.params)
        dx = gouts[0]
        if dx is None:
            dx = torch.zeros_like(x0)
        dx = dx.contiguous()
        pending_tap = tap_g.pop(depth - 1, None)
        dx, dx_lp = ops.add_cast(dx, pending_tap, want_f32=True, lp_dtype=lp)
        nojoin = lp is not None and depth > 1
        if nojoin:
            ring = [ctx.ws, torch.empty_like(ctx.ws)]
            keep = [[], []]
        sptr = ctx.sptr

        def block_bwd(i, a, g, dx, dx_lp, dxn, dxn_lp, flags, ws):
            head = (C.byref(dims), C.byref(ctx.wstructs[i]), C.byref(a), C.byref(g), ctx.xs[i].data_ptr(),
                    dx.data_ptr(), ops.ptr(dx_lp), dxn.data_ptr(), ops.ptr(dxn_lp))
            if sptr is not None:
                return L.ssl4gie_block_bwd_dp(*head, sptr[i][0], sptr[i][1], flags, ws.data_ptr(), st)
            return L.ssl4gie_block_bwd(*head, flags, ws.data_ptr(), st)
        for i in range(depth - 1, -1, -1):
            if i != depth - 1 and i in tap_g:
                dx, dx_lp = ops.add_cast(dx, tap_g[i].contiguous(), want_f32=True, lp_dtype=lp)
            g = BlockGrads()
            tg = targets[i * _NP:(i + 1) * _NP]
            scratch = []
            for name, t, p in zip(("ln1_g", "ln1_b", "wqkv", "bqkv", "wproj", "bproj", "ln2_g",
                                   "ln2_b", "wfc1", "bfc1", "wfc2", "bfc2"), tg,
                                  ctx.params[i * _NP:(i + 1) * _NP]):
                if t is None:
                    t = torch.empty_like(p)
                    scratch.append(t)
                setattr(g, name, t.data_ptr())
            a = layout.struct(ctx.acts.data_ptr() + i * layout.total)
            dxn = torch.empty_like(x0)
            next_scales_dx = sptr is not None and i > 0 and sptr[i - 1][1] != 0
            dxn_lp = torch.empty(x0.shape, dtype=lp, device=x0.device) if lp and not next_scales_dx else None
            if nojoin:
                k = (depth - 1 - i) % 2
                _lib.check(L.ssl4gie_wgrad_wait(k, st), "wgrad_wait")
                keep[k].clear()
                _lib.check(block_bwd(i, a, g, dx, dx_lp, dxn, dxn_lp, int(accumulate) | _lib.BWD_NO_JOIN | (k << 4),
                                     ring[k]), f"block_bwd[{i}]")
                keep[k] += [dx, dx_lp, scratch]
                if cfg.on_block_grads is not None:
                    cfg.on_block_grads(i)
            else:
                _lib.check(block_bwd(i, a, g, dx, dx_lp, dxn, dxn_lp, int(accumulate), ctx.ws), f"block_bwd[{i}]")
                if cfg.on_block_grads is not None:
                    cfg.on_block_grads(i)
            dx, dx_lp = dxn, dxn_lp
        if nojoin:
            for slot in (0, 1):
                _lib.check(L.ssl4gie_wgrad_wait(slot, st), "wgrad_wait")
            keep[0].clear(); keep[1].clear()
        ctx.acts = ctx.xs = ctx.ws = ctx.keepalive = None
        return (dx, None) + tuple(returns)


_KEEP_TABLES = {}


def draw_drop_scales(rates: Sequence[float], B: int, device) -> torch.Tensor:
    rates = tuple(float(r) for r in rates)
    assert all(0.0 <= r < 1.0 for r in rates), "drop_path rates must lie in [0, 1)"
    key = (str(device), rates)
    keep = _KEEP_TABLES.get(key)
    if keep is None:
        keep = _KEEP_TABLES[key] = torch.tensor([1.0 - r for r in rates], dtype=torch.float32).view(-1, 1, 1).to(
            device, non_blocking=True)
    return torch.bernoulli(keep.expand(len(rates), 2, B)).div_(keep).contiguous()


def run_blocks(blocks: Sequence[nn.Module], x: torch.Tensor, heads: int, eps: float, dtype,
               sink: GradSink, taps: Sequence[int] = (), lp: LPCache = None,
               on_block_grads=None, drop_scales: Optional[torch.Tensor] = None):
    params: List[torch.Tensor] = []
    for b in blocks:
        params += _block_params(b)
    need = torch.is_grad_enabled() and (x.requires_grad or any(p.requires_grad for p in params))
    drop = None
    if drop_scales is not None:
        drop = (drop_scales.contiguous(), (True,) * len(blocks))
    elif need:
        rates = [float(getattr(b, "drop_path", 0.0)) if b.training else 0.0 for b in blocks]
        if any(r > 0.0 for r in rates):
            drop = (draw_drop_scales(rates, x.shape[0], x.device), tuple(r > 0.0 for r in rates))
    cfg = StackCfg(heads=heads, eps=eps, dtype=dtype, taps=tuple(taps), need_bwd=need, sink=sink,
                   lp=lp or _GLOBAL_LP, on_block_grads=on_block_grads, drop=drop)
    outs = BlockStackFn.apply(x, cfg, *params)
    return outs[0], list(outs[1:])


class LayerNormFn(torch.autograd.Function):

    @staticmethod
    def forward(ctx, x, gamma, beta, eps, out_dtype, sink):
        x = x.contiguous()
        y, mean, rstd = ops.layernorm_fwd(x, gamma.detach(), beta.detach(), eps, out_dtype)
        ctx.save_for_backward(x, gamma, beta, mean, rstd)
        ctx.sink = sink
        return y

    @staticmethod
    def backward(ctx, dy):
        x, gamma, beta, mean, rstd = ctx.saved_tensors
        (tg, tb), acc, rets = ctx.sink.plan([gamma, beta])
        if tg is None or tb is None:
            tg = tg if tg is not None else torch.empty_like(gamma)
            tb = tb if tb is not None else torch.empty_like(beta)
        dx, _, _, _ = ops.layernorm_bwd(dy.contiguous(), x, gamma.detach(), mean, rstd,
                                        dgamma=tg, dbeta=tb, accumulate=acc)
        return dx, rets[0], rets[1], None, None, None


class GradJoin:

    __slots__ = ("adder_claimed", "pending")

    def __init__(self):
        self.adder_claimed = False
        self.pending = None

    @staticmethod
    def for_tensor(x):
        return GradJoin() if (torch.is_grad_enabled() and x.requires_grad) else None

    def claim(self) -> str:
        if not self.adder_claimed:
            self.adder_claimed = True
            return "adder"
        return "depositor"

    def deposit(self, g):
        self.pending = g if self.pending is None else self.pending + g

    def take(self):
        g, self.pending = self.pending, None
        return g


_WGRAD_SIDE = os.environ.get("SSL4GIE_CONV_WGRAD_STREAM", "1") != "0"
_WG = {"stream": None}


def set_wgrad_side(on: bool) -> bool:
    global _WGRAD_SIDE
    prev, _WGRAD_SIDE = _WGRAD_SIDE, bool(on)
    return prev


SAFE_POST_ACC_HOOK_IDS = set()


def _wgrad_join():
    if _WG["stream"] is not None:
        torch.cuda.current_stream().wait_stream(_WG["stream"])


def wgrad_fork(sink, params, *operands):
    if not _WGRAD_SIDE or not operands or operands[0] is None or not operands[0].is_cuda:
        return None
    live = [p for p in params if p is not None and p.requires_grad]
    arena = getattr(sink, "arena", None)
    if arena is None or not live or not all(arena.owns(p) for p in live):
        return None
    if torch.is_grad_enabled() or any(getattr(p, "_backward_hooks", None) for p in live):
        return None
    for p in live:
        hooks = getattr(p, "_post_accumulate_grad_hooks", None)
        if hooks and any(k not in SAFE_POST_ACC_HOOK_IDS for k in hooks):
            return None
    if _WG["stream"] is None:
        _WG["stream"] = torch.cuda.Stream()
    side = _WG["stream"]
    side.wait_stream(torch.cuda.current_stream())
    for t in operands:
        if t is not None and t.is_cuda:
            t.record_stream(side)
    from torch.autograd import Variable
    Variable._execution_engine.queue_callback(_wgrad_join)
    return side


class LinearFn(torch.autograd.Function):

    @staticmethod
    def forward(ctx, x, weight, bias, dtype, out_dtype, sink, lp, want_stats=False, join=None):
        ctx.join, ctx.join_role = join, (join.claim() if join is not None else None)
        shp = x.shape
        x2 = x.contiguous().view(-1, shp[-1])
        assert x2.dtype == dtype
        w, wt = lp.get(weight, dtype)
        ctx.save_for_backward(x2, weight, bias)
        ctx.wlp, ctx.wt, ctx.sink, ctx.dtype, ctx.shp = w, wt, sink, dtype, shp
        if want_stats:
            stats = None
            if bias is None and out_dtype == dtype and ops.colstats_ok(x2.shape[0], w.shape[0], w.shape[1], dtype):
                y, stats = ops.linear_fwd(x2, w, None, out_dtype=out_dtype, colstats=True)
                ctx.mark_non_differentiable(stats)
                ctx.set_materialize_grads(False)
            else:
                y = ops.linear_fwd(x2, w, bias.detach() if bias is not None else None, out_dtype=out_dtype)
            return y.view(*shp[:-1], w.shape[0]), stats
        y = ops.linear_fwd(x2, w, bias.detach() if bias is not None else None, out_dtype=out_dtype)
        return y.view(*shp[:-1], w.shape[0])

    @staticmethod
    def backward(ctx, dy, *unused):
        if dy is None:
            return (None,) * 9
        x2, weight, bias = ctx.saved_tensors
        dy2 = dy.contiguous().view(-1, dy.shape[-1])
        if dy2.dtype != ctx.dtype:
            _, dy2 = ops.add_cast(dy2, None, want_f32=False, lp_dtype=ctx.dtype)
        (tw, tb), acc, rets = ctx.sink.plan([weight, bias])
        dx = None
        if ctx.needs_input_grad[0]:
            other = ctx.join.take() if ctx.join_role == "adder" else None
            if other is not None and ops.add_aux_ok(dy2.shape[0], x2.shape[1], dy2.shape[1], ctx.dtype,
                                                    ctx.wt is not None):
                dx = ops.linear_bwd_data(dy2, ctx.wlp, ctx.wt, add_aux=other.contiguous()).view(ctx.shp)
            else:
                dx = ops.linear_bwd_data(dy2, ctx.wlp, ctx.wt).view(ctx.shp)
                if other is not None:
                    dx = dx + other.view(ctx.shp)
            if ctx.join_role == "depositor":
                ctx.join.deposit(dx)
                dx = None
        if tw is not None:
            side = wgrad_fork(ctx.sink, (weight, bias), dy2, x2, weight, bias)
            with (torch.cuda.stream(side) if side is not None else contextlib.nullcontext()):
                ops.linear_bwd_weight(dy2, x2, out=tw, accumulate=acc, bias_out=tb)
        elif tb is not None:
            ops.colsum(dy2, out=tb, accumulate=acc)
        return dx, rets[0], rets[1], None, None, None, None, None, None


class MatmulNTFn(torch.autograd.Function):

    @staticmethod
    def forward(ctx, a, b):
        a2, b2 = a.contiguous().float(), b.contiguous().float()
        ctx.save_for_backward(a2, b2)
        return ops.linear_fwd(a2, b2, None, out_dtype=torch.float32)

    @staticmethod
    def backward(ctx, dy):
        a2, b2 = ctx.saved_tensors
        dy2 = dy.contiguous().float()
        da = ops.linear_bwd_data(dy2, b2, out_dtype=torch.float32) if ctx.needs_input_grad[0] else None
        db = ops.linear_bwd_weight(dy2, a2) if ctx.needs_input_grad[1] else None
        return da, db


def _assemble_tokens(y, cls, pos, B, nsel, ids=None):
    return ops.tokens_assemble(y, cls.detach().contiguous().view(-1),
                               pos.detach().contiguous().view(-1, pos.shape[-1]), B, nsel, ids=ids)


def _assemble_tokens_bwd(dx, dtype, tc, tpos, acc):
    if tpos is not None:
        dpos = dx.sum(0, keepdim=True)
        if acc:
            tpos.add_(dpos)
        else:
            tpos.copy_(dpos)
    return ops.tokens_assemble_bwd(dx, dtype, dcls_out=tc, accumulate=acc)


class TokensAssembleFn(torch.autograd.Function):

    @staticmethod
    def forward(ctx, y, cls, pos, B, dtype, sink):
        y = y.contiguous()
        x = _assemble_tokens(y, cls, pos, B, y.shape[0] // B)
        ctx.save_for_backward(cls, pos)
        ctx.sink, ctx.dtype = sink, dtype
        return x

    @staticmethod
    def backward(ctx, dx):
        cls, pos = ctx.saved_tensors
        pos_grad = pos.requires_grad
        tgs, acc, rets = ctx.sink.plan([cls] + ([pos] if pos_grad else []))
        dy = _assemble_tokens_bwd(dx.contiguous(), ctx.dtype, tgs[0], tgs[1] if pos_grad else None, acc)
        return dy, rets[0], (rets[1] if pos_grad else None), None, None, None


class PatchEmbedFn(torch.autograd.Function):

    @staticmethod
    def forward(ctx, imgs, weight, bias, cls, pos, ids, nsel, p, dtype, sink, lp):
        B = imgs.shape[0]
        imgs = imgs.contiguous()
        cols = ops.patch_gather(imgs, p, ids=ids, nsel=nsel, out_dtype=dtype)
        w, _ = lp.get(weight, dtype)
        y = ops.linear_fwd(cols, w, bias.detach(), out_dtype=dtype)
        nsel_eff = cols.shape[0] // B
        x = _assemble_tokens(y, cls, pos, B, nsel_eff, ids=ids)
        ctx.save_for_backward(cols, weight, bias, cls, pos)
        ctx.sink, ctx.dtype = sink, dtype
        ctx.pos_grad = pos.requires_grad and ids is None
        if pos.requires_grad and ids is not None:
            raise NotImplementedError("masked patch embedding with a trainable pos_embed")
        return x

    @staticmethod
    def backward(ctx, dx):
        cols, weight, bias, cls, pos = ctx.saved_tensors
        plist = [weight, bias, cls] + ([pos] if ctx.pos_grad else [])
        tgs, acc, rets = ctx.sink.plan(plist)
        tw, tb, tc = tgs[:3]
        dy = _assemble_tokens_bwd(dx.contiguous(), ctx.dtype, tc, tgs[3] if ctx.pos_grad else None, acc)
        if tw is not None:
            ops.linear_bwd_weight(dy, cols, out=tw, accumulate=acc, bias_out=tb)
        elif tb is not None:
            ops.colsum(dy, out=tb, accumulate=acc)
        return (None, rets[0], rets[1], rets[2], rets[3] if ctx.pos_grad else None) + (None,) * 6


class PatchEmbedDetFn(torch.autograd.Function):

    @staticmethod
    def forward(ctx, imgs, weight, bias, ids, p, dtype, sink, lp):
        cols = ops.patch_gather(imgs.contiguous(), p, ids=ids.contiguous(), out_dtype=dtype)
        w, _ = lp.get(weight, dtype)
        y = ops.linear_fwd(cols, w, bias.detach(), out_dtype=torch.float32)
        ctx.save_for_backward(cols, weight, bias)
        ctx.sink, ctx.dtype = sink, dtype
        return y

    @staticmethod
    def backward(ctx, dy):
        cols, weight, bias = ctx.saved_tensors
        (tw, tb), acc, rets = ctx.sink.plan([weight, bias])
        dy = dy.contiguous()
        dyl = dy if ctx.dtype == torch.float32 else ops.cast(dy, ctx.dtype)
        if tw is not None:
            ops.linear_bwd_weight(dyl, cols, out=tw, accumulate=acc, bias_out=tb)
        elif tb is not None:
            ops.colsum(dyl, out=tb, accumulate=acc)
        return (None, rets[0], rets[1]) + (None,) * 5


class DecoderAssembleFn(torch.autograd.Function):

    @staticmethod
    def forward(ctx, y, mask_token, dpos, ids_restore, ids_shuffle, nkeep, sink):
        xd = ops.decoder_assemble(y.contiguous(), mask_token.detach().contiguous().view(-1),
                                  dpos.detach().contiguous().view(-1, dpos.shape[-1]),
                                  ids_restore, nkeep)
        ctx.save_for_backward(mask_token, ids_shuffle)
        ctx.nkeep, ctx.sink, ctx.ydtype = nkeep, sink, y.dtype
        return xd

    @staticmethod
    def backward(ctx, dxd):
        mask_token, ids_shuffle = ctx.saved_tensors
        (tm,), acc, rets = ctx.sink.plan([mask_token])
        if tm is None:
            tm = torch.empty_like(mask_token)
        dy = ops.decoder_assemble_bwd(dxd.contiguous(), ids_shuffle, ctx.nkeep, ctx.ydtype,
                                      dmask_out=tm, accumulate=acc)
        return dy, rets[0], None, None, None, None, None


class MaeLossFn(torch.autograd.Function):

    @staticmethod
    def forward(ctx, pred_full, imgs, mask, p, norm_pix):
        pred_full = pred_full.contiguous()
        per_patch = ops.mae_loss_fwd(pred_full, imgs, mask, p, norm_pix)
        ctx.save_for_backward(pred_full, imgs, mask)
        ctx.p, ctx.norm_pix = p, norm_pix
        return per_patch

    @staticmethod
    def backward(ctx, gpp):
        pred_full, imgs, mask = ctx.saved_tensors
        dpred = ops.mae_loss_bwd(pred_full, imgs, mask, ctx.p, ctx.norm_pix, gpp.contiguous())
        return dpred, None, None, None, None


class EngineModule(nn.Module):

    engine_dtype = None

    def __init__(self):
        super().__init__()
        self._arena: Optional[ParamArena] = None
        self._lp = LPCache(self._arena_nocheck)
        self._sink = None
        object.__setattr__(self, "_root", None)

    def adopt(self, child: "EngineModule"):
        object.__setattr__(child, "_root", self)
        return child

    def set_precision(self, name_or_dtype):
        if isinstance(name_or_dtype, str):
            name_or_dtype = {"bf16": torch.bfloat16, "fp32": torch.float32,
                             "f32": torch.float32}[name_or_dtype.lower()]
        assert name_or_dtype in (torch.bfloat16, torch.float32)
        self.engine_dtype = name_or_dtype
        return self

    @property
    def dtype_(self):
        if self._root is not None:
            return self._root.dtype_
        return self.engine_dtype or default_dtype()

    def arena(self) -> ParamArena:
        if self._root is not None:
            return self._root.arena()
        ps = list(self.parameters())
        a = self._arena
        if a is None or len(a.params) != len(ps) or any(x is not y for x, y in zip(a.params, ps)) \
                or not a.intact():
            if not ps[0].is_cuda:
                raise RuntimeError("ssl4gie_amd models run on the HIP device only: call .cuda() "
                                   "first (there is no CPU fallback)")
            old = {id(p): p.grad for p in ps}
            self._arena = a = ParamArena(ps)
            self._sink = GradSink(a)
            for p in ps:
                g = old[id(p)]
                if g is not None:
                    v = a.grad_view(p)
                    v.copy_(g)
                    p.grad = v
        return a

    def _arena_nocheck(self) -> Optional[ParamArena]:
        return self._root._arena_nocheck() if self._root is not None else self._arena

    def _prepare(self):
        _lib.load()
        self.arena()
        self.sink().new_pass()
        self.lp_cache.refresh_conv_operands()

    def sink(self) -> GradSink:
        if self._root is not None:
            return self._root.sink()
        if self._arena is None:
            self.arena()
        return self._sink

    @property
    def lp_cache(self) -> LPCache:
        return self._root.lp_cache if self._root is not None else self._lp

    def _ln(self, x, norm: nn.LayerNorm, out_dtype=None):
        return LayerNormFn.apply(x, norm.weight, norm.bias, norm.eps, out_dtype or self.dtype_,
                                 self.sink())

    def _linear(self, x, lin: nn.Linear, out_dtype=None):
        return LinearFn.apply(x, lin.weight, lin.bias, self.dtype_, out_dtype or self.dtype_,
                              self.sink(), self._lp)

    def _blocks(self, blocks, x, heads, eps, taps=(), drop_scales=None):
        sink = self.sink()
        hook = None
        if sink.tracker is not None:
            blist = list(blocks)
            hook = lambda i: sink.note_done(_block_params(blist[i]))
        return run_blocks(blocks, x, heads, eps, self.dtype_, sink, taps=taps, lp=self._lp,
                          on_block_grads=hook, drop_scales=drop_scales)
```

### ssl4gie_amd/ops.py

```python
from __future__ import annotations

import ctypes as C

import os

import torch

from . import _lib
from ._lib import BF16, F32, GemmDesc
from .conv_plan import colstats_ok, conv_out_hw, gather_fwd_ok, gather_wgrad_ok, k_pad

_TORCH2CODE = {torch.float32: F32, torch.bfloat16: BF16}
_CODE2TORCH = {F32: torch.float32, BF16: torch.bfloat16}


def code(dtype) -> int:
    try:
        return _TORCH2CODE[dtype]
    except KeyError:
        raise TypeError(f"unsupported dtype {dtype}; the HIP path computes in fp32 or bf16")


def torch_dtype(c: int):
    return _CODE2TORCH[c]
# ... 334 lines not shown
    return out


def bt_loss(c, lambd):
    _dev(c)
    _f32(c)
    D = c.shape[0]
    assert c.shape == (D, D)
    L = _lib.load()
    ws = torch.empty(L.ssl4gie_bt_loss_workspace_bytes(D), dtype=torch.uint8, device=c.device)
    loss = torch.empty((), dtype=torch.float32, device=c.device)
    _lib.check(L.ssl4gie_bt_loss(ptr(c), ptr(loss), D, float(lambd), ptr(ws), stream()), "bt_loss")
    return loss


def bt_loss_grad(c, scale, dtype, lambd):
    _dev(c)
    _f32(c)
    D = c.shape[0]
    assert c.shape == (D, D)
    scale = scale.to(device=c.device, dtype=torch.float32).reshape(()).contiguous()
    w = torch.empty(D, D, dtype=dtype, device=c.device)
    wt = torch.empty(D, D, dtype=dtype, device=c.device)
    _lib.check(_lib.load().ssl4gie_bt_loss_grad(ptr(c), ptr(scale), ptr(w), ptr(wt), code(dtype), D, float(lambd),
                                                stream()), "bt_loss_grad")
    return w, wt


def add_cast(a, b=None, want_f32=True, lp_dtype=None):
    _dev(a, b)
    _f32(a, b)
    assert b is None or b.shape == a.shape
    out = torch.empty_like(a) if want_f32 else None
    out_lp = torch.empty(a.shape, dtype=lp_dtype, device=a.device) if lp_dtype is not None else None
    _lib.check(_lib.load().ssl4gie_add_cast(ptr(a), ptr(b), ptr(out), ptr(out_lp),
                                            code(lp_dtype) if lp_dtype is not None else 0,
                                            a.numel(), stream()), "add_cast")
    return out, out_lp


def mask_argsort(noise, len_keep):
    _dev(noise)
    _f32(noise)
    B, Lp = noise.shape
    ids_shuffle = torch.empty(B, Lp, dtype=torch.int64, device=noise.device)
    ids_restore = torch.empty_like(ids_shuffle)
    mask = torch.empty(B, Lp, dtype=torch.float32, device=noise.device)
    _lib.check(_lib.load().ssl4gie_mask_argsort(ptr(noise), ptr(ids_shuffle), ptr(ids_restore),
                                                ptr(mask), B, Lp, int(len_keep), stream()),
               "mask_argsort")
    return ids_shuffle, ids_restore, mask


def patch_gather(img, p, ids=None, nsel=None, out_dtype=torch.float32, order=0):
    _dev(img, ids)
    _f32(img)
    B, Cc, H, W = img.shape
    npatch = (H // p) * (W // p)
    if ids is not None:
        assert ids.dtype == torch.int64 and ids.shape[0] == B and ids.dim() == 2
        ids_stride = ids.shape[1]
        nsel = nsel if nsel is not None else ids.shape[1]
        assert nsel <= ids.shape[1]
    else:
        ids_stride, nsel = 0, npatch
    out = torch.empty(B * nsel, Cc * p * p, dtype=out_dtype, device=img.device)
    _lib.check(_lib.load().ssl4gie_patch_gather(ptr(img), ptr(ids), ptr(out), code(out_dtype), B,
                                                Cc, H, W, p, nsel, ids_stride, order, stream()),
               "patch_gather")
    return out


def tokens_assemble(y2d, cls, pos, B, nsel, ids=None):
    _dev(y2d, cls, pos, ids)
    _f32(cls, pos)
    D = y2d.shape[1]
    assert y2d.shape[0] == B * nsel and cls.numel() == D and pos.shape[-1] == D
    ids_stride = 0
    if ids is not None:
        assert ids.dtype == torch.int64 and ids.shape[0] == B and ids.shape[1] >= nsel
        ids_stride = ids.shape[1]
        assert pos.numel() // D >= 1 + ids.shape[1]
    else:
        assert pos.numel() // D >= 1 + nsel
    x = torch.empty(B, nsel + 1, D, dtype=torch.float32, device=y2d.device)
    _lib.check(_lib.load().ssl4gie_tokens_assemble(ptr(y2d), code(y2d.dtype), ptr(cls), ptr(pos),
                                                   ptr(ids), ids_stride, ptr(x), B, nsel, D,
                                                   stream()), "tokens_assemble")
    return x


def tokens_assemble_bwd(dx, lp_dtype, dcls_out=None, accumulate=False):
    _dev(dx, dcls_out)
    _f32(dx, dcls_out)
    B, n1, D = dx.shape
    assert dcls_out is None or dcls_out.numel() == D
    dy = torch.empty(B * (n1 - 1), D, dtype=lp_dtype, device=dx.device)
    _lib.check(_lib.load().ssl4gie_tokens_assemble_bwd(ptr(dx), ptr(dy), code(lp_dtype),
                                                       ptr(dcls_out), int(accumulate), B, n1 - 1,
                                                       D, stream()), "tokens_assemble_bwd")
    return dy


def decoder_assemble(y, mask_token, dpos, ids_restore, nkeep):
    _dev(y, mask_token, dpos, ids_restore)
    _f32(mask_token, dpos)
    B, Lp = ids_restore.shape
    D = y.shape[-1]
    assert y.numel() == B * (nkeep + 1) * D and mask_token.numel() == D
    assert dpos.numel() == (Lp + 1) * D and ids_restore.dtype == torch.int64
    xd = torch.empty(B, Lp + 1, D, dtype=torch.float32, device=y.device)
    _lib.check(_lib.load().ssl4gie_decoder_assemble(ptr(y), code(y.dtype), ptr(mask_token),
                                                    ptr(dpos), ptr(ids_restore), ptr(xd), B, Lp,
                                                    nkeep, D, stream()), "decoder_assemble")
    return xd


def decoder_assemble_bwd(dxd, ids_shuffle, nkeep, lp_dtype, dmask_out, accumulate=False):
    _dev(dxd, ids_shuffle, dmask_out)
    _f32(dxd, dmask_out)
    B, L1, D = dxd.shape
    Lp = L1 - 1
    assert ids_shuffle.shape == (B, Lp) and ids_shuffle.dtype == torch.int64
    assert dmask_out.numel() == D
    L = _lib.load()
    dy = torch.empty(B, nkeep + 1, D, dtype=lp_dtype, device=dxd.device)
    ws = torch.empty(L.ssl4gie_decoder_assemble_bwd_workspace_bytes(B, Lp, D), dtype=torch.uint8,
                     device=dxd.device)
    _lib.check(L.ssl4gie_decoder_assemble_bwd(ptr(dxd), ptr(ids_shuffle), ptr(dy), code(lp_dtype),
                                              ptr(dmask_out), int(accumulate), ptr(ws), B, Lp,
                                              nkeep, D, stream()), "decoder_assemble_bwd")
    return dy


def _loss_geom(pred, img, mask, p):
    B, Cc, H, W = img.shape
    Lp = (H // p) * (W // p)
    assert mask.shape == (B, Lp) and pred.dim() == 3 and pred.shape[0] == B
    assert pred.shape[2] == Cc * p * p and pred.shape[1] in (Lp, Lp + 1)
    return B, Cc, H, W, int(pred.shape[1] == Lp + 1)


def mae_loss_fwd(pred, img, mask, p, norm_pix):
    _dev(pred, img, mask)
    _f32(pred, img, mask)
    B, Cc, H, W, has_cls = _loss_geom(pred, img, mask, p)
    per_patch = torch.empty_like(mask)
    _lib.check(_lib.load().ssl4gie_mae_loss(ptr(pred), ptr(img), ptr(mask), ptr(per_patch), 0, 0,
                                            1.0, int(norm_pix), has_cls, B, Cc, H, W, p, stream()),
               "mae_loss")
    return per_patch


def mae_loss_bwd(pred, img, mask, p, norm_pix, gpp, gscale_host=1.0):
    _dev(pred, img, mask, gpp)
    _f32(pred, img, mask, gpp)
    assert gpp is None or gpp.shape == mask.shape
    B, Cc, H, W, has_cls = _loss_geom(pred, img, mask, p)
    dpred = torch.empty_like(pred)
    _lib.check(_lib.load().ssl4gie_mae_loss(ptr(pred), ptr(img), ptr(mask), 0, ptr(dpred),
                                            ptr(gpp), float(gscale_host), int(norm_pix), has_cls,
                                            B, Cc, H, W, p, stream()), "mae_loss(bwd)")
    return dpred


def _nhwc(x):
    _dev(x)
    assert x.dim() == 4, "expected [B, H, W, C]"
    return x.shape


def im2col3x3(x, stride=1, relu=False, ld=None):
    B, H, W, C = _nhwc(x)
    Ho, Wo = conv_out_hw(H, W, stride)
    ld = ld or k_pad(9 * C, x.dtype)
    cols = torch.empty(B * Ho * Wo, ld, dtype=x.dtype, device=x.device)
    _lib.check(_lib.load().ssl4gie_im2col3x3(ptr(x), ptr(cols), code(x.dtype), B, H, W, C, stride,
                                             int(relu), ld, stream()), "im2col3x3")
    return cols


def conv3x3_implicit_ok(x, stride, n_out=None, wgrad=False):
    return x.is_contiguous() and (gather_wgrad_ok if wgrad else gather_fwd_ok)(*x.shape, n_out, stride, x.dtype)


def _geom(x, stride, relu):
    B, H, W, C_ = x.shape
    g = _lib.Conv3x3Geom()
    g.B, g.H, g.W, g.C, g.stride, g.relu = B, H, W, C_, stride, int(relu)
    return g


def conv3x3_fwd(x, w2, bias=None, stride=1, relu=False, relu_mask=None, colstats=False):
    _dev(x, w2, bias, relu_mask)
    B, H, W, Cin = _nhwc(x)
    Cout, K = w2.shape
    assert K == 9 * Cin and w2.dtype == x.dtype and w2.is_contiguous()
    assert conv3x3_implicit_ok(x, stride, Cout)
    Ho, Wo = conv_out_hw(H, W, stride)
    M = B * Ho * Wo
    d = _desc(M, Cout, K, code(x.dtype), code(x.dtype))
    g = _geom(x, stride, relu)
    d.conv = C.pointer(g)
    d.A, d.sAm, d.sAk = ptr(x), K, 1
    d.B, d.sBk, d.sBn = ptr(w2), 1, K
    y = torch.empty(M, Cout, dtype=x.dtype, device=x.device)
    d.C, d.ldc = ptr(y), Cout
    if bias is not None:
        _f32(bias)
        assert bias.numel() == Cout
        d.epilogue, d.bias = _lib.EPI_BIAS, ptr(bias)
    if relu_mask is not None:
        assert bias is None and not relu and relu_mask.dtype == x.dtype and relu_mask.is_contiguous() \
            and relu_mask.numel() == M * Cout
        d.epilogue, d.aux = _lib.EPI_RELU_MASK_AUX, ptr(relu_mask)
    if colstats:
        assert bias is None and relu_mask is None
        stats = torch.empty((M + 127) // 128, 2, Cout, dtype=torch.float32, device=x.device)
        d.colstats = ptr(stats)
        gemm_raw(d, x.device)
        return y.view(B, Ho, Wo, Cout), stats
    gemm_raw(d, x.device)
    return y.view(B, Ho, Wo, Cout)


def conv3x3_bwd_weight(dy2d, x, stride=1, relu=False, bias_out=None):
    _dev(dy2d, x, bias_out)
    B, H, W, Cin = _nhwc(x)
    T, Cout = dy2d.shape
    Ho, Wo = conv_out_hw(H, W, stride)
    assert T == B * Ho * Wo and dy2d.dtype == x.dtype and dy2d.is_contiguous()
    assert conv3x3_implicit_ok(x, stride, Cout, wgrad=True)
    out = torch.empty(Cout, 9 * Cin, dtype=torch.float32, device=x.device)
    d = _desc(Cout, 9 * Cin, T, code(x.dtype), F32)
    g = _geom(x, stride, relu)
    d.conv = C.pointer(g)
    d.A, d.sAm, d.sAk = ptr(dy2d), 1, Cout
    d.B, d.sBk, d.sBn = ptr(x), 9 * Cin, 1
    d.C, d.ldc = ptr(out), 9 * Cin
    if bias_out is not None:
        assert bias_out.dtype == torch.float32 and bias_out.numel() == Cout
        d.colsum_a = ptr(bias_out)
    gemm_raw(d, x.device)
    return out


def conv3x3_direct_fwd(x, w2, bias=None, relu=False, relu_mask=None, colstats=False):
    _dev(x, w2, bias, relu_mask)
    B, H, W, Cin = _nhwc(x)
    Cout, K = w2.shape
    assert K == 9 * Cin and w2.dtype == x.dtype == torch.bfloat16 and w2.is_contiguous() and x.is_contiguous()
    if bias is not None:
        _f32(bias)
        assert bias.numel() == Cout
    if relu_mask is not None:
        assert relu_mask.dtype == x.dtype and relu_mask.is_contiguous() and relu_mask.numel() == B * H * W * Cout
    y = torch.empty(B, H, W, Cout, dtype=x.dtype, device=x.device)
    L = _lib.load()
    stats = None
    if colstats:
        assert relu_mask is None
        stats = torch.empty(L.ssl4gie_conv3x3_direct_tiles(B, H, W), 2, Cout, dtype=torch.float32, device=x.device)
    _lib.check(L.ssl4gie_conv3x3_direct_fwd(ptr(x), ptr(w2), ptr(bias), ptr(relu_mask), ptr(y), ptr(stats),
                                            B, H, W, Cin, Cout, int(relu), stream()), "conv3x3_direct_fwd")
    return (y, stats) if colstats else y


def conv3x3_direct_wgrad(dy, x, relu=False, bias_out=None):
    _dev(dy, x, bias_out)
    if bias_out is not None:
        assert bias_out.dtype == torch.float32 and bias_out.numel() == dy.shape[-1]
    B, H, W, Cin = _nhwc(x)
    Cout = dy.shape[-1]
    assert dy.numel() == B * H * W * Cout and dy.dtype == x.dtype and dy.is_contiguous()
    lib = _lib.load()
    nbytes = lib.ssl4gie_conv3x3_direct_wgrad_workspace_bytes(B, H, W, Cin, Cout)
    assert nbytes > 0, "conv3x3_direct_wgrad: unsupported geometry"
    ws = torch.empty(nbytes, dtype=torch.uint8, device=x.device)
    out = torch.empty(Cout, 9 * Cin, dtype=torch.float32, device=x.device)
    _lib.check(lib.ssl4gie_conv3x3_direct_wgrad(ptr(dy), ptr(x), ptr(out), ptr(bias_out), ptr(ws), nbytes, B, H, W, Cin,
                                                Cout, int(relu), 0, stream()), "conv3x3_direct_wgrad")
    return out


def stem7x7_pack(imgs):
    _dev(imgs)
    _f32(imgs)
    B, Cc, H, W = imgs.shape
    assert Cc == 3 and imgs.is_contiguous()
    L = _lib.load()
    nb = L.ssl4gie_stem7x7_packed_bytes(B, H, W)
    assert nb > 0, "stem7x7: unsupported image size"
    out = torch.empty(nb // 2, dtype=torch.bfloat16, device=imgs.device)
    _lib.check(L.ssl4gie_stem7x7_pack(ptr(imgs), ptr(out), B, H, W, stream()), "stem7x7_pack")
    return out


def _pack_shape(w, mode, ld):
    Cout, Cin = w.shape[:2]
    ld = 9 * (Cout if mode == 1 else Cin) if ld is None else ld
    return Cout, Cin, ld, ((Cout, ld) if mode == 0 else ((Cin, ld) if mode == 1 else (ld, Cout)))


def conv3x3_weight_pack(weight, dtype, mode, ld=None):
    _dev(weight)
    assert weight.dtype == torch.float32 and weight.dim() == 4 and weight.shape[2:] == (3, 3)
    w = weight.contiguous()
    Cout, Cin, ld, shape = _pack_shape(w, mode, ld)
    out = torch.empty(shape, dtype=dtype, device=w.device)
    _lib.check(_lib.load().ssl4gie_conv3x3_weight_pack(ptr(w), ptr(out), code(dtype), Cout, Cin, mode, ld, stream()),
               "conv3x3_weight_pack")
    return out


def conv3x3_weight_pack_batch(weights, dtype, modes, lds):
# ... 1236 lines not shown
```

### ssl4gie_amd/optim.py

```python
from __future__ import annotations

import ctypes as C

import torch

from . import _lib
from .engine import ParamArena, bump_weights_epoch
from .ops import ptr, stream


def _adopt_grads(a, params):
    base, index = a.grad.data_ptr(), a._index
    for p in params:
        g = p.grad
        if g is not None and g.data_ptr() != base + 4 * index[id(p)]:
            v = a.grad_view(p)
            v.copy_(g)
            p.grad = v


class _GradNorm:

    def __init__(self, dev):
        L = _lib.load()
# ... 17 lines not shown
        a = target._arena()
        start, mask, _, _, S = target._build_tables(a)
        gn = target._grad_norm(a)
    else:
        from .parallel import before_optimizer_step
        before_optimizer_step()
        if not isinstance(target, ParamArena) and not hasattr(target, "arena"):
            raise TypeError("get_grad_norm_ / clip_grad_norm_ take an engine model, a parallel.DataParallel "
                            f"or an arena optimizer, not {type(target).__name__}")
        a = target if isinstance(target, ParamArena) else target.arena()
        _adopt_grads(a, a.params)
        chosen = None if parameters is None else {id(p) for p in parameters}
        active = tuple(p.grad is not None and (chosen is None or id(p) in chosen) for p in a.params)
        st = a._grad_norm_state
        if st is None or st["active"] != active:
            host = (torch.tensor(list(a.offsets) + [a.numel], dtype=torch.int64).pin_memory(),
                    torch.tensor([1.0 if on else -1.0 for on in active]).pin_memory())
            gn = st["gn"] if st is not None else _GradNorm(a.data.device)
            st = {"active": active, "host": host, "gn": gn,
                  "dev": tuple(h.to(a.data.device, non_blocking=True) for h in host)}
            a._grad_norm_state = st
        (start, mask), S, gn = st["dev"], len(a.params), st["gn"]
    gn.run(a, start, mask, S, max_norm)
    if max_norm is not None:
        gn.scale(a, start, mask, S)
    return gn


@torch.no_grad()
def get_grad_norm_(model_or_optimizer):
    return _norm_pass(model_or_optimizer, None).norm


@torch.no_grad()
def clip_grad_norm_(model_or_optimizer, max_norm):
    return _norm_pass(model_or_optimizer, float(max_norm)).norm


class _ArenaOptimizer:
    def __init__(self, model, params, defaults):
        self.model = model
        if isinstance(params, (list, tuple)) and params and isinstance(params[0], dict):
            groups = [dict(g) for g in params]
        else:
            groups = [{"params": list(params)}]
        for g in groups:
            g["params"] = list(g["params"])
            for k, v in defaults.items():
                g.setdefault(k, v)
        self.param_groups = groups
        self.defaults = dict(defaults)
        self._tables_key = None
        self._hyper = None
        self._gn = None
        self.step_count = 0

    def _arena(self):
        from .parallel import before_optimizer_step
        before_optimizer_step()
        a = self.model.arena()
        own = [p for g in self.param_groups for p in g["params"]]
        assert all(a.owns(p) for p in own), "every optimised parameter must live in the model's arena"
        _adopt_grads(a, own)
        return a

    def _grad_norm(self, a):
        if self._gn is None or self._gn.ctl.device != a.data.device:
            self._gn = _GradNorm(a.data.device)
        return self._gn

    def _build_tables(self, a):
        n = len(a.params)
        group_of = {}
        for gi, g in enumerate(self.param_groups):
            for p in g["params"]:
                group_of[id(p)] = gi
        active = tuple(id(p) in group_of and p.requires_grad and p.grad is not None for p in a.params)
        hyper = tuple((g["lr"], g["weight_decay"]) for g in self.param_groups)
        layout_key = (id(a), active)
        if layout_key != self._tables_key:
            dev = a.data.device
            pin = dev.type == "cuda"
            start = torch.tensor(list(a.offsets) + [a.numel], dtype=torch.int64)
            mat = torch.tensor([1.0 if (active[i] and p.ndim > 1) else 0.0 for i, p in enumerate(a.params)])
            if pin:
                start, mat = start.pin_memory(), mat.pin_memory()
            self._host_layout = (start, mat)
            self._host = (torch.empty(n, pin_memory=pin), torch.empty(n, pin_memory=pin))
            self._dev = [start.to(dev, non_blocking=pin), torch.empty(n, device=dev), torch.empty(n, device=dev),
                         mat.to(dev, non_blocking=pin)]
            self._gidx = [group_of.get(id(p), -1) if active[i] else -1 for i, p in enumerate(a.params)]
            self._tables_key, self._hyper = layout_key, None
        if hyper != self._hyper:
            lr_h, wd_h = self._host
            lrs = [hyper[gi][0] if gi >= 0 else -1.0 for gi in self._gidx]
            wds = [hyper[gi][1] if gi >= 0 else 0.0 for gi in self._gidx]
            lr_h.copy_(torch.tensor(lrs))
            wd_h.copy_(torch.tensor(wds))
            self._dev[1].copy_(lr_h, non_blocking=True)
            self._dev[2].copy_(wd_h, non_blocking=True)
            self._hyper = hyper
        return tuple(self._dev) + (n,)

    def _state_buffers(self):
        raise NotImplementedError

    def state_dict(self):
        groups = [{k: v for k, v in g.items() if k != "params"} | {"n_params": len(g["params"])}
                  for g in self.param_groups]
        return {"kind": type(self).__name__, "step_count": self.step_count, "param_groups": groups,
                "state": {k: (v.detach().clone() if v is not None else None)
                          for k, v in self._state_buffers().items()}}

    def load_state_dict(self, sd):
        assert sd["kind"] == type(self).__name__, (sd["kind"], type(self).__name__)
        assert len(sd["param_groups"]) == len(self.param_groups)
        for g, saved in zip(self.param_groups, sd["param_groups"]):
            assert saved["n_params"] == len(g["params"]), "parameter groups differ from the saved ones"
            g.update({k: v for k, v in saved.items() if k != "n_params"})
        a = self._arena()
        for k, v in sd["state"].items():
            if v is not None:
                assert v.numel() == a.numel, "optimizer state was saved for a different arena layout"
                setattr(self, k, v.to(a.data.device, torch.float32).clone())
        self.step_count = int(sd["step_count"])
        self._hyper = None

    def zero_grad(self, set_to_none: bool = True):
        for g in self.param_groups:
            for p in g["params"]:
                if set_to_none:
                    p.grad = None
                elif p.grad is not None:
                    p.grad.zero_()


class ArenaAdamW(_ArenaOptimizer):

    def __init__(self, model, params, lr=1e-3, betas=(0.9, 0.999), eps=1e-8, weight_decay=1e-2,
                 overlap_backward=False):
        self._host_steps = 0
        self._dev_steps = None
        self._ctl_plain = None
        super().__init__(model, params, dict(lr=lr, weight_decay=weight_decay))
        self.betas, self.eps = betas, eps
        self.exp_avg = self.exp_avg_sq = None
        self._overlap = bool(overlap_backward)
        self._stream = None
        self._done = []
        self._tables = None
        self._seen = {}
        self._hooked = False
        self._lp = None
        self.last_grad_norm = self.last_found_inf = None

    def _state_buffers(self):
        return {"exp_avg": self.exp_avg, "exp_avg_sq": self.exp_avg_sq}

    @property
    def step_count(self):
        return self._host_steps if self._dev_steps is None else int(self._dev_steps.item())

    @step_count.setter
    def step_count(self, n):
        self._host_steps = int(n)
        if self._dev_steps is not None:
            self._dev_steps.fill_(int(n))

    def _hook(self):
        if self._overlap and not self._hooked:
            sink = self.model.sink()
            if sink.tracker is None:
                sink.tracker = self._on_use_done
                self._hooked = True
            else:
                self._overlap = False

    def zero_grad(self, set_to_none: bool = True):
        super().zero_grad(set_to_none)
        self._hook()
        self._done, self._seen, self._tables = [], {}, None

    def _launch(self, a, lo, hi, st):
        start, lr, wd, _, S = self._tables
        _lib.check(_lib.load().ssl4gie_adamw_arena_range(
            ptr(a.data), ptr(a.grad), ptr(self.exp_avg), ptr(self.exp_avg_sq), ptr(start), ptr(lr), ptr(wd), S,
            self.betas[0], self.betas[1], self.eps, self.step_count + 1, lo, hi, ptr(self._lp), st),
            "adamw_arena_range")

    @torch.no_grad()
    def _on_use_done(self, params):
        if not self._overlap or self.exp_avg is None or self._tables_key is None:
            return
        for p in params:
            n = self._seen.get(id(p), 0) + 1
            self._seen[id(p)] = n
            if n > 1:
                self._overlap = False
                return
        a = self.model.arena()
        lo, hi = a.span(params)
        inside = [q for q, o in zip(a.params, a.offsets) if lo <= o < hi]
        ids = {id(p) for p in params}
        if any(id(q) not in ids for q in inside) or any(lo < h and l < hi for l, h in self._done):
            return
        if self._tables is None:
            self._lp = a.lp_flat_for_update()
            self._tables = self._build_tables_cached(a)
        if self._stream is None:
            self._stream = torch.cuda.Stream(device=a.data.device)
        ev = torch.cuda.Event()
        ev.record(torch.cuda.current_stream(a.data.device))
        self._stream.wait_event(ev)
        L = _lib.load()
        for slot in (0, 1):
            L.ssl4gie_wgrad_wait(slot, self._stream.cuda_stream)
        self._launch(a, lo, hi, self._stream.cuda_stream)
        self._done.append((lo, hi))

    def _build_tables_cached(self, a):
        saved = self._tables_key
        n = len(a.params)
        group_of = {id(p): gi for gi, g in enumerate(self.param_groups) for p in g["params"]}
        hyper = tuple((g["lr"], g["weight_decay"]) for g in self.param_groups)
        if hyper != self._hyper:
            lr_h, wd_h = self._host
            lr_h.copy_(torch.tensor([hyper[gi][0] if gi >= 0 else -1.0 for gi in self._gidx]))
            wd_h.copy_(torch.tensor([hyper[gi][1] if gi >= 0 else 0.0 for gi in self._gidx]))
            self._dev[1].copy_(lr_h, non_blocking=True)
            self._dev[2].copy_(wd_h, non_blocking=True)
            self._hyper = hyper
        assert self._tables_key == saved and group_of is not None
        return tuple(self._dev) + (n,)

    def _step_ctl(self, a, clip_grad, skip_nonfinite):
        start, lr, wd, _, S = self._tables
        dev = a.data.device
        if self._dev_steps is None:
            self._dev_steps = torch.full((1,), self._host_steps, dtype=torch.int32, device=dev)
        elif self._dev_steps.device != dev:
            self._dev_steps = self._dev_steps.to(dev)
        if clip_grad is not None or skip_nonfinite:
            gn = self._grad_norm(a)
            gn.run(a, start, lr, S, clip_grad)
            self.last_grad_norm, self.last_found_inf = gn.norm, gn.found_inf
            ctl = gn.ctl
        else:
            if self._ctl_plain is None or self._ctl_plain.device != dev:
                self._ctl_plain = torch.zeros(4, device=dev)
                self._ctl_plain[1] = 1.0
            ctl = self._ctl_plain
        _lib.check(_lib.load().ssl4gie_adamw_arena_range_ctl(
            ptr(a.data), ptr(a.grad), ptr(self.exp_avg), ptr(self.exp_avg_sq), ptr(start), ptr(lr), ptr(wd), S,
            self.betas[0], self.betas[1], self.eps, ptr(self._dev_steps), 0, a.numel, ptr(self._lp), ptr(ctl),
            int(bool(skip_nonfinite)), 1, stream()), "adamw_arena_range_ctl")

    @torch.no_grad()
    def step(self, clip_grad=None, skip_nonfinite=False):
        ctl_path = clip_grad is not None or skip_nonfinite
        if ctl_path and self._overlap:
            raise ValueError("ArenaAdamW(overlap_backward=True) applies updates while the backward pass is "
                             "still running; clip_grad / skip_nonfinite need the norm of EVERY gradient first")
        a = self._arena()
        if self.exp_avg is None or self.exp_avg.numel() != a.numel:
            self.exp_avg = torch.zeros_like(a.data)
            self.exp_avg_sq = torch.zeros_like(a.data)
        key_before = self._tables_key
        tables = self._build_tables(a)
        if self._done and self._tables_key != key_before:
            raise RuntimeError("ArenaAdamW(overlap_backward=True): the set of parameters with gradients "
                               "changed between steps after part of this step was already applied")
        self._tables = tables
        self._lp = a.lp_flat_for_update() if a.data.is_cuda else None
        if ctl_path or self._dev_steps is not None:
            assert not self._done, "in-backward updates and the device-side step count do not mix"
            self._step_ctl(a, clip_grad, skip_nonfinite)
        else:
            st = stream()
            pos = 0
            for lo, hi in sorted(self._done) + [(a.numel, a.numel)]:
                if lo > pos:
                    self._launch(a, pos, lo, st)
                pos = max(pos, hi)
            if self._done:
                torch.cuda.current_stream(a.data.device).wait_stream(self._stream)
            self.step_count += 1
        self._done, self._seen, self._tables = [], {}, None
        bump_weights_epoch(touched=[p for g in self.param_groups for p in g["params"]])
        if self._lp is not None:
            a.lp_flat_is_current()


class ArenaLARS(_ArenaOptimizer):

    def __init__(self, model, params, lr=0.0, weight_decay=0.0, momentum=0.9, trust_coefficient=0.001):
        super().__init__(model, params, dict(lr=lr, weight_decay=weight_decay))
        self.momentum, self.trust = momentum, trust_coefficient
        self.mu = None
        self._ws = None

    def _state_buffers(self):
        return {"mu": self.mu}

    @torch.no_grad()
    def step(self):
        a = self._arena()
        if self.mu is None or self.mu.numel() != a.numel:
            self.mu = torch.zeros_like(a.data)
        start, lr, wd, mat, S = self._build_tables(a)
        L = _lib.load()
        nbytes = L.ssl4gie_lars_workspace_bytes(S)
        if self._ws is None or self._ws.numel() < nbytes:
            self._ws = torch.empty(nbytes, dtype=torch.uint8, device=a.data.device)
        self.step_count += 1
        _lib.check(L.ssl4gie_lars_arena(ptr(a.data), ptr(a.grad), ptr(self.mu), ptr(start), ptr(lr), ptr(wd),
                                        ptr(mat), S, self.momentum, self.trust, ptr(self._ws), a.numel,
                                        stream()), "lars_arena")
        bump_weights_epoch(touched=[p for g in self.param_groups for p in g["params"]])
```

Measured before the change: 11970 images/sec.

## Fuse decoder pred linear with MAE loss, add tiled AdamW writing transposed bf16 weights

Replaces the separate decoder_pred linear and loss with one autograd function whose backward produces the loss gradient directly in bf16, so an f32 dpred buffer and a cast are no longer needed. It adds a tiled AdamW kernel that updates matrix segments in 64x64 tiles and writes both the bf16 copy and its transpose, so the transposed low-precision weights need not be rebuilt separately each step. It also threads an LpHandoff through blocks and layernorm to pass low-precision activations between layers, and lets a broadcast loss gradient be read with stride 0 instead of being materialised. These changes add code paths and a transpose done through shared memory inside the optimizer.

```diff
diff --git a/include/ssl4gie_hip.h b/include/ssl4gie_hip.h
--- a/include/ssl4gie_hip.h
+++ b/include/ssl4gie_hip.h
@@ -115,6 +115,9 @@
 int ssl4gie_mae_loss(const float* pred, const float* img, const float* mask, float* per_patch,
                      float* dpred, const float* gpp, float gscale_host, int norm_pix,
                      int has_cls, int B, int C, int H, int W, int p, void* stream);
+int ssl4gie_mae_loss_bwd(const float* pred, const float* img, const float* mask, void* dpred,
+                         int dpred_dtype, const float* gpp, int gpp_stride, float gscale_host, int norm_pix,
+                         int has_cls, int B, int C, int H, int W, int p, void* stream);
 
 typedef struct ssl4gie_block_weights {
     const float *ln1_g, *ln1_b, *ln2_g, *ln2_b;
@@ -298,6 +301,19 @@
                                   const float* seg_lr, const float* seg_wd, int S, float beta1, float beta2,
                                   float eps, int* applied, long long lo, long long hi, void* lp_bf16,
                                   const float* ctl, int skip_nonfinite, int advance, void* stream);
+int ssl4gie_adamw_arena_lp_tiled(float* p, const float* g, float* m, float* v, const long long* seg_start,
+                                 const float* seg_lr, const float* seg_wd, const float* seg_mat, int S,
+                                 float beta1, float beta2, float eps, int step, long long n, void* lp_bf16,
+                                 void* lpt_bf16, const long long* mat_off, const int* mat_rows,
+                                 const int* mat_cols, const int* tile_start, int M, int total_tiles,
+                                 const long long* window, int n_windows, void* stream);
+int ssl4gie_adamw_arena_lp_tiled_ctl(float* p, const float* g, float* m, float* v, const long long* seg_start,
+                                     const float* seg_lr, const float* seg_wd, const float* seg_mat, int S,
+                                     float beta1, float beta2, float eps, int* applied, long long n,
+                                     void* lp_bf16, void* lpt_bf16, const long long* mat_off,
+                                     const int* mat_rows, const int* mat_cols, const int* tile_start, int M,
+                                     int total_tiles, const long long* window, int n_windows, const float* ctl,
+                                     int skip_nonfinite, int advance, void* stream);
 size_t ssl4gie_lars_workspace_bytes(int S);
 int ssl4gie_lars_arena(float* p, const float* g, float* mu, const long long* seg_start,
                        const float* seg_lr, const float* seg_wd, const float* seg_mat, int S,
diff --git a/ssl4gie_amd/Models/mae/models_mae.py b/ssl4gie_amd/Models/mae/models_mae.py
--- a/ssl4gie_amd/Models/mae/models_mae.py
+++ b/ssl4gie_amd/Models/mae/models_mae.py
@@ -6,7 +6,7 @@
 import torch.nn as nn
 
 from ... import ops
-from ...engine import DecoderAssembleFn, EngineModule, MaeLossFn, PatchEmbedFn
+from ...engine import DecoderAssembleFn, EngineModule, LpHandoff, MaeLossFn, PatchEmbedFn, PredLossFn
 from ..vit_layers import Block, PatchEmbed
 from .util.pos_embed import get_2d_sincos_pos_embed
 
@@ -103,11 +103,12 @@
         tok = PatchEmbedFn.apply(x.float(), self.patch_embed.proj.weight, self.patch_embed.proj.bias,
                                  self.cls_token, self.pos_embed, ids_shuffle, keep, p, self.dtype_,
                                  self.sink(), self._lp)
-        tok, _ = self._blocks(self.blocks, tok, self.num_heads, self.norm.eps)
-        latent = self._ln(tok, self.norm)
+        hand = LpHandoff() if torch.is_grad_enabled() else None
+        tok, _ = self._blocks(self.blocks, tok, self.num_heads, self.norm.eps, handoff=hand)
+        latent = self._ln(tok, self.norm, handoff=hand)
         return latent, mask, ids_restore
 
-    def forward_decoder(self, x, ids_restore, _full=False):
+    def _decoder_trunk(self, x, ids_restore):
         self._prepare()
         keep = x.shape[1] - 1
         ids_shuffle = getattr(self, "_ids_shuffle", None)
@@ -118,8 +119,12 @@
         y = self._linear(x, self.decoder_embed)
         xd = DecoderAssembleFn.apply(y, self.mask_token, self.decoder_pos_embed, ids_restore,
                                      ids_shuffle, keep, self.sink())
-        xd, _ = self._blocks(self.decoder_blocks, xd, self.decoder_num_heads, self.decoder_norm.eps)
-        h = self._ln(xd, self.decoder_norm)
+        hand = LpHandoff() if torch.is_grad_enabled() else None
+        xd, _ = self._blocks(self.decoder_blocks, xd, self.decoder_num_heads, self.decoder_norm.eps, handoff=hand)
+        return self._ln(xd, self.decoder_norm, handoff=hand)
+
+    def forward_decoder(self, x, ids_restore, _full=False):
+        h = self._decoder_trunk(x, ids_restore)
         full = self._linear(h, self.decoder_pred, out_dtype=torch.float32)
         return full if _full else full[:, 1:, :]
 
@@ -131,8 +136,11 @@
 
     def forward(self, imgs, mask_ratio=0.75, noise=None):
         latent, mask, ids_restore = self.forward_encoder(imgs, mask_ratio, noise=noise)
-        full = self.forward_decoder(latent, ids_restore, _full=True)
-        loss = self.forward_loss(imgs, full, mask)
+        h = self._decoder_trunk(latent, ids_restore)
+        per_patch, full = PredLossFn.apply(h, self.decoder_pred.weight, self.decoder_pred.bias,
+                                           imgs.contiguous().float(), mask, self.patch_embed.patch_size[0],
+                                           bool(self.norm_pix_loss), self.dtype_, self.sink(), self._lp)
+        loss = per_patch.sum() / mask.sum()
         return loss, full[:, 1:, :], mask
 
 
diff --git a/ssl4gie_amd/_lib.py b/ssl4gie_amd/_lib.py
--- a/ssl4gie_amd/_lib.py
+++ b/ssl4gie_amd/_lib.py
@@ -90,6 +90,7 @@
     "ssl4gie_decoder_assemble_bwd_workspace_bytes": (sz, [i32, i32, i32]),
     "ssl4gie_decoder_assemble_bwd": (i32, [vp, vp, vp, i32, vp, i32, vp, i32, i32, i32, i32, vp]),
     "ssl4gie_mae_loss": (i32, [vp, vp, vp, vp, vp, vp, f32, i32, i32, i32, i32, i32, i32, i32, vp]),
+    "ssl4gie_mae_loss_bwd": (i32, [vp, vp, vp, vp, i32, vp, i32, f32, i32, i32, i32, i32, i32, i32, i32, vp]),
     "ssl4gie_im2col3x3": (i32, [vp, vp, i32, i32, i32, i32, i32, i32, i32, i64, vp]),
     "ssl4gie_col2im3x3": (i32, [vp, vp, i32, i32, i32, i32, i32, i32, i64, vp]),
     "ssl4gie_conv3x3_direct_ok": (i32, [i32, i32, i32, i32, i32]),
@@ -145,6 +146,10 @@
     "ssl4gie_adamw_arena_range": (i32, [vp, vp, vp, vp, vp, vp, vp, i32, f32, f32, f32, i32, i64, i64, vp, vp]),
     "ssl4gie_adamw_arena_range_ctl": (i32, [vp, vp, vp, vp, vp, vp, vp, i32, f32, f32, f32, vp, i64, i64, vp, vp,
                                             i32, i32, vp]),
+    "ssl4gie_adamw_arena_lp_tiled": (i32, [vp, vp, vp, vp, vp, vp, vp, vp, i32, f32, f32, f32, i32, i64, vp, vp, vp, vp,
+                                           vp, vp, i32, i32, vp, i32, vp]),
+    "ssl4gie_adamw_arena_lp_tiled_ctl": (i32, [vp, vp, vp, vp, vp, vp, vp, vp, i32, f32, f32, f32, vp, i64, vp, vp, vp,
+                                               vp, vp, vp, i32, i32, vp, i32, vp, i32, i32, vp]),
     "ssl4gie_grad_norm_workspace_bytes": (sz, []),
     "ssl4gie_grad_norm_arena": (i32, [vp, vp, vp, i32, f32, f32, vp, vp, i64, vp]),
     "ssl4gie_grad_scale_arena": (i32, [vp, vp, vp, i32, vp, i64, vp]),
diff --git a/ssl4gie_amd/csrc/mae_ops.hip b/ssl4gie_amd/csrc/mae_ops.hip
--- a/ssl4gie_amd/csrc/mae_ops.hip
+++ b/ssl4gie_amd/csrc/mae_ops.hip
@@ -394,17 +394,17 @@
     return ssl4gie_internal_reduce_partials(workspace, dmask_token, B * DAB_Y, D, (size_t)D, accumulate, st);
 }
 
-template <int NV>
+template <int NV, typename TD = float>
 __global__ __launch_bounds__(256) void mae_loss_kernel(
     const float* __restrict__ pred, const float* __restrict__ img, const float* __restrict__ mask,
-    float* __restrict__ per_patch, float* __restrict__ dpred, const float* __restrict__ gpp,
-    float gscale_host, int norm_pix, int has_cls, int B, int C, int H, int W, int p) {
+    float* __restrict__ per_patch, TD* __restrict__ dpred, const float* __restrict__ gpp,
+    float gscale_host, int norm_pix, int has_cls, int B, int C, int H, int W, int p, int gpp_stride) {
     const int lane = threadIdx.x & 63;
     const int gw = W / p, L = (H / p) * gw, P = C * p * p, R = L + has_cls;
     const long long row = (long long)blockIdx.x * 4 + (threadIdx.x >> 6);
     if (row >= (long long)B * R) return;
     const int b = (int)(row / R), t = (int)(row % R);
-    float* dr = dpred ? dpred + (size_t)row * P : nullptr;
+    TD* dr = dpred ? dpred + (size_t)row * P : nullptr;
     if (has_cls && t == 0) {
         if (dr)
             for (int k = 4 * lane; k < P; k += 256) st4(dr + k, f32x4{0.f, 0.f, 0.f, 0.f});
@@ -454,7 +454,7 @@
     e = wave_sum(e) / (float)P;
     if (per_patch && lane == 0) per_patch[(size_t)b * L + l] = e * m;
     if (dr) {
-        const float gs = gscale_host * (gpp ? gpp[(size_t)b * L + l] : 1.f) * m * 2.0f / (float)P;
+        const float gs = gscale_host * (gpp ? gpp[((size_t)b * L + l) * gpp_stride] : 1.f) * m * 2.0f / (float)P;
 #pragma unroll
         for (int i = 0; i < NV; ++i)
             if (4 * lane + 256 * i < P) st4(dr + 4 * lane + 256 * i, (pv[i] - tv[i]) * gs);
@@ -474,13 +474,51 @@
     hipStream_t st = (hipStream_t)stream;
     if (P <= 64 * 4)
         hipLaunchKernelGGL(mae_loss_kernel<1>, grid, block, 0, st, pred, img, mask, per_patch, dpred,
-                           gpp, gscale_host, norm_pix, has_cls, B, C, H, W, p);
+                           gpp, gscale_host, norm_pix, has_cls, B, C, H, W, p, 1);
     else if (P <= 64 * 12)
         hipLaunchKernelGGL(mae_loss_kernel<3>, grid, block, 0, st, pred, img, mask, per_patch,
-                           dpred, gpp, gscale_host, norm_pix, has_cls, B, C, H, W, p);
+                           dpred, gpp, gscale_host, norm_pix, has_cls, B, C, H, W, p, 1);
     else
         hipLaunchKernelGGL(mae_loss_kernel<4>, grid, block, 0, st, pred, img, mask, per_patch,
-                           dpred, gpp, gscale_host, norm_pix, has_cls, B, C, H, W, p);
+                           dpred, gpp, gscale_host, norm_pix, has_cls, B, C, H, W, p, 1);
+    LAUNCH_CHECK();
+    return 0;
+}
+template <typename TD>
+static void launch_mae_loss_bwd(const float* pred, const float* img, const float* mask, TD* dpred,
+                                const float* gpp, int gpp_stride, float gscale_host, int norm_pix, int has_cls,
+                                int B, int C, int H, int W, int p, hipStream_t st) {
+    const int P = C * p * p;
+    const long long rows = (long long)B * ((H / p) * (W / p) + has_cls);
+    dim3 grid((unsigned)((rows + 3) / 4)), block(256);
+    if (P <= 64 * 4)
+        hipLaunchKernelGGL((mae_loss_kernel<1, TD>), grid, block, 0, st, pred, img, mask, (float*)nullptr, dpred,
+                           gpp, gscale_host, norm_pix, has_cls, B, C, H, W, p, gpp_stride);
+    else if (P <= 64 * 12)
+        hipLaunchKernelGGL((mae_loss_kernel<3, TD>), grid, block, 0, st, pred, img, mask, (float*)nullptr, dpred,
+                           gpp, gscale_host, norm_pix, has_cls, B, C, H, W, p, gpp_stride);
+    else
+        hipLaunchKernelGGL((mae_loss_kernel<4, TD>), grid, block, 0, st, pred, img, mask, (float*)nullptr, dpred,
+                           gpp, gscale_host, norm_pix, has_cls, B, C, H, W, p, gpp_stride);
+}
+extern "C" int ssl4gie_mae_loss_bwd(const float* pred, const float* img, const float* mask, void* dpred,
+                                    int dpred_dtype, const float* gpp, int gpp_stride, float gscale_host,
+                                    int norm_pix, int has_cls, int B, int C, int H, int W, int p,
+                                    void* stream) {
+    REQUIRE(pred && img && mask && dpred && B >= 0 && C > 0 && p > 0 && H % p == 0 && W % p == 0);
+    REQUIRE(has_cls == 0 || has_cls == 1);
+    REQUIRE(dpred_dtype == SSL4GIE_F32 || dpred_dtype == SSL4GIE_BF16);
+    REQUIRE(gpp_stride == 1 || (gpp_stride == 0 && gpp));
+    const int P = C * p * p;
+    REQUIRE(P <= 64 * 16 && P % 4 == 0);
+    if (B == 0) return 0;
+    hipStream_t st = (hipStream_t)stream;
+    if (dpred_dtype == SSL4GIE_BF16)
+        launch_mae_loss_bwd(pred, img, mask, (bf16_t*)dpred, gpp, gpp_stride, gscale_host, norm_pix, has_cls, B, C,
+                            H, W, p, st);
+    else
+        launch_mae_loss_bwd(pred, img, mask, (float*)dpred, gpp, gpp_stride, gscale_host, norm_pix, has_cls, B, C,
+                            H, W, p, st);
     LAUNCH_CHECK();
     return 0;
 }
diff --git a/ssl4gie_amd/csrc/optim_ops.hip b/ssl4gie_amd/csrc/optim_ops.hip
--- a/ssl4gie_amd/csrc/optim_ops.hip
+++ b/ssl4gie_amd/csrc/optim_ops.hip
@@ -19,6 +19,16 @@
     while (s + 1 < S && seg_start[s + 1] <= i) ++s;
     return s;
 }
+template <bool CTL>
+DEVI void adamw_update(float& p, float& m, float& v, float g, float lr, float wd, float b1, float b2, float eps,
+                       float step, float rsqrt_bc2) {
+    const float keep = __builtin_fmaf(-lr, wd, 1.f);
+    const float mj = CTL ? __builtin_fmaf(b1, m, (1.f - b1) * g) : __builtin_fmaf(1.f - b1, g, b1 * m);
+    const float vj = __builtin_fmaf(b2, v, (1.f - b2) * g * g);
+    const float q = step * mj / __builtin_fmaf(sqrtf(vj), rsqrt_bc2, eps);
+    p = __builtin_fmaf(keep, p, -q);
+    m = mj; v = vj;
+}
 }
 
 template <bool CTL>
@@ -27,7 +37,8 @@
     const long long* __restrict__ seg_start, const float* __restrict__ seg_lr,
     const float* __restrict__ seg_wd, int S, float b1, float b2, float eps, float bc1, float rsqrt_bc2,
     long long n, bf16_t* __restrict__ lp, long long lo, const float* __restrict__ ctl,
-    const int* __restrict__ applied, int skip) {
+    const int* __restrict__ applied, int skip, const float* __restrict__ seg_tiled,
+    const long long* __restrict__ window) {
     __shared__ float bc[2];
     float coef = 1.f;
     if (CTL) {
@@ -39,12 +50,13 @@
             bc[1] = 1.f / sqrtf(1.f - powf(b2, t));
         }
     }
-    const long long first = lo + (long long)blockIdx.x * blockDim.x * 4;
+    const long long first = window ? window[blockIdx.x] : lo + (long long)blockIdx.x * blockDim.x * 4;
     const long long i = first + threadIdx.x * 4;
     const int s = block_seg(seg_start, S, i < n ? i : n - 4, first);
     if (i >= n) return;
     const float lr = seg_lr[s];
     if (lr < 0.f) return;
+    if (seg_tiled && seg_tiled[s] != 0.f) return;
     if (CTL) { bc1 = bc[0]; rsqrt_bc2 = bc[1]; }
     const float wd = seg_wd[s];
     f32x4 pp = ld4(p + i), mm = ld4(m + i), vv = ld4(v + i);
@@ -53,16 +65,116 @@
     const float step = lr / bc1;
 #pragma unroll
     for (int j = 0; j < 4; ++j) {
-        float x = pp[j] * (1.f - lr * wd);
-        const float mj = b1 * mm[j] + (1.f - b1) * gg[j];
-        const float vj = b2 * vv[j] + (1.f - b2) * gg[j] * gg[j];
-        x -= step * mj / (sqrtf(vj) * rsqrt_bc2 + eps);
-        pp[j] = x; mm[j] = mj; vv[j] = vj;
+        float pj = pp[j], mj = mm[j], vj = vv[j];
+        adamw_update<CTL>(pj, mj, vj, gg[j], lr, wd, b1, b2, eps, step, rsqrt_bc2);
+        pp[j] = pj; mm[j] = mj; vv[j] = vj;
     }
     st4(p + i, pp);
     st4(m + i, mm);
     st4(v + i, vv);
     if (lp) st4(lp + i, pp);
+}
+template <bool CTL>
+__global__ __launch_bounds__(256, 4) void adamw_arena_tiled_kernel(
+    float* __restrict__ p, const float* __restrict__ g, float* __restrict__ m, float* __restrict__ v,
+    const long long* __restrict__ seg_start, const float* __restrict__ seg_lr,
+    const float* __restrict__ seg_wd, int S, float b1, float b2, float eps, float bc1, float rsqrt_bc2,
+    bf16_t* __restrict__ lp, bf16_t* __restrict__ lpt, const long long* __restrict__ mat_off,
+    const int* __restrict__ mat_rows, const int* __restrict__ mat_cols, const int* __restrict__ tile_start,
+    int M, const float* __restrict__ ctl, const int* __restrict__ applied, int skip) {
+    __shared__ float tile[64][65];
+    __shared__ float bc[2];
+    float coef = 1.f;
+    if (CTL) {
+        if (skip && ctl[2] != 0.f) return;
+        coef = ctl[1];
+    }
+    const int t = blockIdx.x;
+    int lo = 0, hi = M;
+    while (hi - lo > 1) {
+        const int mid = (lo + hi) >> 1;
+        if (tile_start[mid] <= t) lo = mid; else hi = mid;
+    }
+    const long long off = mat_off[lo];
+    const int s = find_seg(seg_start, S, off);
+    const float lr = seg_lr[s];
+    if (lr < 0.f) return;
+    if (CTL) {
+        if (threadIdx.x == 0) {
+            const float tt = (float)(*applied + 1);
+            bc[0] = 1.f - powf(b1, tt);
+            bc[1] = 1.f / sqrtf(1.f - powf(b2, tt));
+        }
+        __syncthreads();
+        bc1 = bc[0]; rsqrt_bc2 = bc[1];
+    }
+    const float wd = seg_wd[s], step = lr / bc1;
+    const int R = mat_rows[lo], Cc = mat_cols[lo], lt = t - tile_start[lo];
+    const int tiles_c = (Cc + 63) >> 6;
+    const int r0 = (lt / tiles_c) * 64, c0 = (lt % tiles_c) * 64;
+    const int tx = threadIdx.x & 15, ty = threadIdx.x >> 4;
+    const bool vec = Cc % 4 == 0, vec_t = R % 4 == 0;
+    const int c = c0 + 4 * tx;
+#pragma unroll 1
+    for (int h = 0; h < 2; ++h) {
+        f32x4 pp[2], gg[2], mm[2], vv[2];
+#pragma unroll
+        for (int k = 0; k < 2; ++k) {
+            const int r = r0 + ty + 16 * (2 * h + k);
+            const size_t e = (size_t)off + (size_t)r * Cc + c;
+            pp[k] = gg[k] = mm[k] = vv[k] = f32x4{0.f, 0.f, 0.f, 0.f};
+            if (r < R) {
+                if (vec && c < Cc) {
+                    pp[k] = ld4(p + e); gg[k] = ld4(g + e); mm[k] = ld4(m + e); vv[k] = ld4(v + e);
+                } else {
+#pragma unroll
+                    for (int j = 0; j < 4; ++j)
+                        if (c + j < Cc) {
+                            pp[k][j] = p[e + j]; gg[k][j] = g[e + j]; mm[k][j] = m[e + j]; vv[k][j] = v[e + j];
+                        }
+                }
+            }
+        }
+#pragma unroll
+        for (int k = 0; k < 2; ++k) {
+            const int i = 2 * h + k, r = r0 + ty + 16 * i;
+            const size_t e = (size_t)off + (size_t)r * Cc + c;
+            if (CTL) gg[k] *= coef;
+#pragma unroll
+            for (int j = 0; j < 4; ++j) {
+                float pj = pp[k][j], mj = mm[k][j], vj = vv[k][j];
+                adamw_update<CTL>(pj, mj, vj, gg[k][j], lr, wd, b1, b2, eps, step, rsqrt_bc2);
+                pp[k][j] = pj; mm[k][j] = mj; vv[k][j] = vj;
+                tile[ty + 16 * i][4 * tx + j] = pj;
+            }
+            if (r < R) {
+                if (vec && c < Cc) {
+                    st4(p + e, pp[k]); st4(m + e, mm[k]); st4(v + e, vv[k]); st4(lp + e, pp[k]);
+                } else {
+#pragma unroll
+                    for (int j = 0; j < 4; ++j)
+                        if (c + j < Cc) {
+                            p[e + j] = pp[k][j]; m[e + j] = mm[k][j]; v[e + j] = vv[k][j];
+                            lp[e + j] = f2bf(pp[k][j]);
+                        }
+                }
+            }
+        }
+    }
+    __syncthreads();
+#pragma unroll
+    for (int i = 0; i < 4; ++i) {
+        const int cc = c0 + ty + 16 * i, r = r0 + 4 * tx;
+        if (cc < Cc) {
+            const f32x4 o = {tile[4 * tx][ty + 16 * i], tile[4 * tx + 1][ty + 16 * i],
+                             tile[4 * tx + 2][ty + 16 * i], tile[4 * tx + 3][ty + 16 * i]};
+            bf16_t* d = lpt + (size_t)off + (size_t)cc * R + r;
+            if (vec_t && r < R) st4(d, o);
+            else
+#pragma unroll
+                for (int j = 0; j < 4; ++j) if (r + j < R) d[j] = f2bf(o[j]);
+        }
+    }
 }
 __global__ void adamw_advance_kernel(int* __restrict__ applied, const float* __restrict__ ctl, int skip) {
     if (!(skip && ctl[2] != 0.f)) *applied += 1;
@@ -247,7 +359,7 @@
     hipLaunchKernelGGL(adamw_arena_kernel<false>, dim3((unsigned)(((hi - lo) / 4 + 255) / 256)), dim3(256), 0,
                        (hipStream_t)stream, p, g, m, v, seg_start, seg_lr, seg_wd, S, beta1, beta2, eps,
                        bc1, 1.f / sqrtf(bc2), hi, (bf16_t*)lp_bf16, lo, (const float*)nullptr,
-                       (const int*)nullptr, 0);
+                       (const int*)nullptr, 0, (const float*)nullptr, (const long long*)nullptr);
     LAUNCH_CHECK();
     return 0;
 }
@@ -263,8 +375,73 @@
         hipLaunchKernelGGL(adamw_arena_kernel<true>, dim3((unsigned)(((hi - lo) / 4 + 255) / 256)), dim3(256),
                            0, (hipStream_t)stream, p, g, m, v, seg_start, seg_lr, seg_wd, S, beta1, beta2,
                            eps, 0.f, 0.f, hi, (bf16_t*)lp_bf16, lo, ctl, (const int*)applied,
+                           skip_nonfinite != 0, (const float*)nullptr, (const long long*)nullptr);
+        LAUNCH_CHECK();
+    }
+    if (advance) {
+        hipLaunchKernelGGL(adamw_advance_kernel, dim3(1), dim3(1), 0, (hipStream_t)stream, applied, ctl,
                            skip_nonfinite != 0);
         LAUNCH_CHECK();
+    }
+    return 0;
+}
+extern "C" int ssl4gie_adamw_arena_lp_tiled(float* p, const float* g, float* m, float* v,
+                                            const long long* seg_start, const float* seg_lr,
+                                            const float* seg_wd, const float* seg_mat, int S, float beta1,
+                                            float beta2, float eps, int step, long long n, void* lp_bf16,
+                                            void* lpt_bf16, const long long* mat_off, const int* mat_rows,
+                                            const int* mat_cols, const int* tile_start, int M,
+                                            int total_tiles, const long long* window, int n_windows,
+                                            void* stream) {
+    REQUIRE(p && g && m && v && seg_start && seg_lr && seg_wd && seg_mat && S > 0 && step > 0 && n >= 0 &&
+            n % 4 == 0 && lp_bf16 && lpt_bf16 && M >= 0 && total_tiles >= 0 && n_windows >= 0);
+    REQUIRE(M == 0 || (mat_off && mat_rows && mat_cols && tile_start && total_tiles > 0));
+    REQUIRE(n_windows == 0 || window);
+    if (n == 0) return 0;
+    const float bc1 = 1.f - powf(beta1, (float)step), bc2 = 1.f - powf(beta2, (float)step);
+    if (M > 0) {
+        hipLaunchKernelGGL(adamw_arena_tiled_kernel<false>, dim3((unsigned)total_tiles), dim3(256), 0,
+                           (hipStream_t)stream, p, g, m, v, seg_start, seg_lr, seg_wd, S, beta1, beta2, eps, bc1,
+                           1.f / sqrtf(bc2), (bf16_t*)lp_bf16, (bf16_t*)lpt_bf16, mat_off, mat_rows, mat_cols,
+                           tile_start, M, (const float*)nullptr, (const int*)nullptr, 0);
+        LAUNCH_CHECK();
+    }
+    if (n_windows > 0) {
+        hipLaunchKernelGGL(adamw_arena_kernel<false>, dim3((unsigned)n_windows), dim3(256), 0, (hipStream_t)stream, p,
+                           g, m, v, seg_start, seg_lr, seg_wd, S, beta1, beta2, eps, bc1, 1.f / sqrtf(bc2), n,
+                           (bf16_t*)lp_bf16, 0LL, (const float*)nullptr, (const int*)nullptr, 0, seg_mat, window);
+        LAUNCH_CHECK();
+    }
+    return 0;
+}
+extern "C" int ssl4gie_adamw_arena_lp_tiled_ctl(float* p, const float* g, float* m, float* v,
+                                                const long long* seg_start, const float* seg_lr,
+                                                const float* seg_wd, const float* seg_mat, int S,
+                                                float beta1, float beta2, float eps, int* applied,
+                                                long long n, void* lp_bf16, void* lpt_bf16,
+                                                const long long* mat_off, const int* mat_rows,
+                                                const int* mat_cols, const int* tile_start, int M,
+                                                int total_tiles, const long long* window, int n_windows,
+                                                const float* ctl, int skip_nonfinite, int advance,
+                                                void* stream) {
+    REQUIRE(p && g && m && v && seg_start && seg_lr && seg_wd && seg_mat && S > 0 && applied && ctl && n >= 0 &&
+            n % 4 == 0 && lp_bf16 && lpt_bf16 && M >= 0 && total_tiles >= 0 && n_windows >= 0);
+    REQUIRE(M == 0 || (mat_off && mat_rows && mat_cols && tile_start && total_tiles > 0));
+    REQUIRE(n_windows == 0 || window);
+    if (n > 0) {
+        if (M > 0) {
+            hipLaunchKernelGGL(adamw_arena_tiled_kernel<true>, dim3((unsigned)total_tiles), dim3(256), 0,
+                               (hipStream_t)stream, p, g, m, v, seg_start, seg_lr, seg_wd, S, beta1, beta2, eps,
+                               0.f, 0.f, (bf16_t*)lp_bf16, (bf16_t*)lpt_bf16, mat_off, mat_rows, mat_cols,
+                               tile_start, M, ctl, (const int*)applied, skip_nonfinite != 0);
+            LAUNCH_CHECK();
+        }
+        if (n_windows > 0) {
+            hipLaunchKernelGGL(adamw_arena_kernel<true>, dim3((unsigned)n_windows), dim3(256), 0, (hipStream_t)stream,
+                               p, g, m, v, seg_start, seg_lr, seg_wd, S, beta1, beta2, eps, 0.f, 0.f, n,
+                               (bf16_t*)lp_bf16, 0LL, ctl, (const int*)applied, skip_nonfinite != 0, seg_mat, window);
+            LAUNCH_CHECK();
+        }
     }
     if (advance) {
         hipLaunchKernelGGL(adamw_advance_kernel, dim3(1), dim3(1), 0, (hipStream_t)stream, applied, ctl,
diff --git a/ssl4gie_amd/engine.py b/ssl4gie_amd/engine.py
--- a/ssl4gie_amd/engine.py
+++ b/ssl4gie_amd/engine.py
@@ -99,6 +99,14 @@
         self._lp_flat_stamp = weights_epoch()
         self._lp_flat_versions = [p._version for p in self.params]
 
+    def lp_pair_for_update(self):
+        self.lp_flat_for_update()
+        return self._lp, self._lpt, self._lp_tab + self._vec_tab
+
+    def lp_pair_is_current(self):
+        self.lp_flat_is_current()
+        self._lpt_stamp = self._lp_flat_stamp
+
     def _refresh_lp(self):
         L = _lib.load()
         if getattr(self, "_lp", None) is None:
@@ -114,13 +122,21 @@
                             torch.tensor([m[1] for m in mats], dtype=torch.int32, device=dev),
                             torch.tensor([m[2] for m in mats], dtype=torch.int32, device=dev),
                             torch.tensor(starts, dtype=torch.int32, device=dev), len(mats), starts[-1])
+            wins, end = [], 0
+            for p, o in zip(self.params, self.offsets):
+                if p.ndim < 2:
+                    pos, hi = max(o, end), o + _align(p.numel(), 64)
+                    while pos < hi:
+                        wins.append(pos)
+                        pos = end = pos + 1024
+            self._vec_tab = (torch.tensor(wins, dtype=torch.int64, device=dev), len(wins))
         flat_ok = getattr(self, "_lp_flat_stamp", None) == weights_epoch() and \
             getattr(self, "_lp_flat_versions", None) == [p._version for p in self.params]
         if not flat_ok:
             _lib.check(L.ssl4gie_cast(ops.ptr(self.data), ops.ptr(self._lp), _lib.BF16, self.numel,
                                       ops.stream()), "cast(arena)")
         off, rows, cols, ts, S, total = self._lp_tab
-        if S:
+        if S and not (flat_ok and getattr(self, "_lpt_stamp", None) == weights_epoch()):
             _lib.check(L.ssl4gie_cast_transpose_batch(ops.ptr(self.data), ops.ptr(self._lpt), ops.ptr(off),
                                                       ops.ptr(rows), ops.ptr(cols), ops.ptr(ts), S, total,
                                                       ops.stream()), "cast_transpose_batch")
@@ -305,6 +321,7 @@
     lp: LPCache
     on_block_grads: Optional[Callable[[int], None]] = None
     drop: Optional[tuple] = None
+    handoff: Optional["LpHandoff"] = None
 
 
 def _block_params(blk):
@@ -413,7 +430,13 @@
             dx = torch.zeros_like(x0)
         dx = dx.contiguous()
         pending_tap = tap_g.pop(depth - 1, None)
-        dx, dx_lp = ops.add_cast(dx, pending_tap, want_f32=True, lp_dtype=lp)
+        handed = None
+        if cfg.handoff is not None:
+            handed = cfg.handoff.take(gouts[0], lp)
+        if handed is not None and pending_tap is None:
+            dx_lp = handed
+        else:
+            dx, dx_lp = ops.add_cast(dx, pending_tap, want_f32=True, lp_dtype=lp)
         nojoin = lp is not None and depth > 1
         if nojoin:
             ring = [ctx.ws, torch.empty_like(ctx.ws)]
@@ -481,7 +504,7 @@
 
 def run_blocks(blocks: Sequence[nn.Module], x: torch.Tensor, heads: int, eps: float, dtype,
                sink: GradSink, taps: Sequence[int] = (), lp: LPCache = None,
-               on_block_grads=None, drop_scales: Optional[torch.Tensor] = None):
+               on_block_grads=None, drop_scales: Optional[torch.Tensor] = None, handoff=None):
     params: List[torch.Tensor] = []
     for b in blocks:
         params += _block_params(b)
@@ -494,7 +517,7 @@
         if any(r > 0.0 for r in rates):
             drop = (draw_drop_scales(rates, x.shape[0], x.device), tuple(r > 0.0 for r in rates))
     cfg = StackCfg(heads=heads, eps=eps, dtype=dtype, taps=tuple(taps), need_bwd=need, sink=sink,
-                   lp=lp or _GLOBAL_LP, on_block_grads=on_block_grads, drop=drop)
+                   lp=lp or _GLOBAL_LP, on_block_grads=on_block_grads, drop=drop, handoff=handoff)
     outs = BlockStackFn.apply(x, cfg, *params)
     return outs[0], list(outs[1:])
 
@@ -502,11 +525,11 @@
 class LayerNormFn(torch.autograd.Function):
 
     @staticmethod
-    def forward(ctx, x, gamma, beta, eps, out_dtype, sink):
+    def forward(ctx, x, gamma, beta, eps, out_dtype, sink, handoff=None):
         x = x.contiguous()
         y, mean, rstd = ops.layernorm_fwd(x, gamma.detach(), beta.detach(), eps, out_dtype)
         ctx.save_for_backward(x, gamma, beta, mean, rstd)
-        ctx.sink = sink
+        ctx.sink, ctx.handoff = sink, handoff
         return y
 
     @staticmethod
@@ -516,9 +539,39 @@
         if tg is None or tb is None:
             tg = tg if tg is not None else torch.empty_like(gamma)
             tb = tb if tb is not None else torch.empty_like(beta)
-        dx, _, _, _ = ops.layernorm_bwd(dy.contiguous(), x, gamma.detach(), mean, rstd,
-                                        dgamma=tg, dbeta=tb, accumulate=acc)
-        return dx, rets[0], rets[1], None, None, None
+        h = ctx.handoff if (_LN_HANDOFF and dy.dtype != torch.float32) else None
+        dx, dx_lp, _, _ = ops.layernorm_bwd(dy.contiguous(), x, gamma.detach(), mean, rstd, want_lp=h is not None,
+                                            dgamma=tg, dbeta=tb, accumulate=acc)
+        if h is not None:
+            h.put(dx, dx_lp)
+        return dx, rets[0], rets[1], None, None, None, None
+
+
+_LN_HANDOFF = True
+
+
+def set_ln_handoff(on: bool) -> bool:
+    global _LN_HANDOFF
+    prev, _LN_HANDOFF = _LN_HANDOFF, bool(on)
+    return prev
+
+
+class LpHandoff:
+
+    __slots__ = ("dx", "dx_lp")
+
+    def __init__(self):
+        self.dx = self.dx_lp = None
+
+    def put(self, dx, dx_lp):
+        self.dx, self.dx_lp = dx, dx_lp
+
+    def take(self, g, lp_dtype):
+        dx, dx_lp, self.dx, self.dx_lp = self.dx, self.dx_lp, None, None
+        if dx is None or g is None or dx_lp.dtype != lp_dtype or g.data_ptr() != dx.data_ptr() or \
+                g.shape != dx.shape or g.dtype != dx.dtype or not g.is_contiguous() or g._version != dx._version:
+            return None
+        return dx_lp
 
 
 class GradJoin:
@@ -617,10 +670,14 @@
     def backward(ctx, dy, *unused):
         if dy is None:
             return (None,) * 9
-        x2, weight, bias = ctx.saved_tensors
+        x2, weight, bias = ctx.saved_tensors[:3]
         dy2 = dy.contiguous().view(-1, dy.shape[-1])
         if dy2.dtype != ctx.dtype:
             _, dy2 = ops.add_cast(dy2, None, want_f32=False, lp_dtype=ctx.dtype)
+        return LinearFn._backward_lp(ctx, dy2, x2, weight, bias) + (None,) * 6
+
+    @staticmethod
+    def _backward_lp(ctx, dy2, x2, weight, bias):
         (tw, tb), acc, rets = ctx.sink.plan([weight, bias])
         dx = None
         if ctx.needs_input_grad[0]:
@@ -641,7 +698,7 @@
                 ops.linear_bwd_weight(dy2, x2, out=tw, accumulate=acc, bias_out=tb)
         elif tb is not None:
             ops.colsum(dy2, out=tb, accumulate=acc)
-        return dx, rets[0], rets[1], None, None, None, None, None, None
+        return dx, rets[0], rets[1]
 
 
 class MatmulNTFn(torch.autograd.Function):
@@ -786,8 +843,43 @@
     @staticmethod
     def backward(ctx, gpp):
         pred_full, imgs, mask = ctx.saved_tensors
-        dpred = ops.mae_loss_bwd(pred_full, imgs, mask, ctx.p, ctx.norm_pix, gpp.contiguous())
+        dpred = ops.mae_loss_bwd(pred_full, imgs, mask, ctx.p, ctx.norm_pix, gpp)
         return dpred, None, None, None, None
+
+
+class PredLossFn(torch.autograd.Function):
+
+    @staticmethod
+    def forward(ctx, h, weight, bias, imgs, mask, p, norm_pix, dtype, sink, lp):
+        shp = h.shape
+        x2 = h.contiguous().view(-1, shp[-1])
+        assert x2.dtype == dtype
+        w, wt = lp.get(weight, dtype)
+        full = ops.linear_fwd(x2, w, bias.detach() if bias is not None else None,
+                              out_dtype=torch.float32).view(*shp[:-1], w.shape[0])
+        per_patch = ops.mae_loss_fwd(full, imgs, mask, p, norm_pix)
+        ctx.save_for_backward(x2, weight, bias, full, imgs, mask)
+        ctx.wlp, ctx.wt, ctx.sink, ctx.dtype, ctx.shp = w, wt, sink, dtype, shp
+        ctx.join = ctx.join_role = None
+        ctx.p, ctx.norm_pix = p, norm_pix
+        ctx.set_materialize_grads(False)
+        return per_patch, full
+
+    @staticmethod
+    def backward(ctx, gpp, dfull):
+        if gpp is None and dfull is None:
+            return (None,) * 10
+        x2, weight, bias, full, imgs, mask = ctx.saved_tensors
+        if gpp is not None and dfull is None:
+            dy2 = ops.mae_loss_bwd(full, imgs, mask, ctx.p, ctx.norm_pix, gpp, out_dtype=ctx.dtype)
+        else:
+            dy2 = dfull.contiguous()
+            if gpp is not None:
+                dy2 = ops.mae_loss_bwd(full, imgs, mask, ctx.p, ctx.norm_pix, gpp) + dy2
+            if dy2.dtype != ctx.dtype:
+                _, dy2 = ops.add_cast(dy2, None, want_f32=False, lp_dtype=ctx.dtype)
+        dy2 = dy2.view(-1, dy2.shape[-1])
+        return LinearFn._backward_lp(ctx, dy2, x2, weight, bias) + (None,) * 7
 
 
 class EngineModule(nn.Module):
@@ -860,19 +952,19 @@
     def lp_cache(self) -> LPCache:
         return self._root.lp_cache if self._root is not None else self._lp
 
-    def _ln(self, x, norm: nn.LayerNorm, out_dtype=None):
+    def _ln(self, x, norm: nn.LayerNorm, out_dtype=None, handoff=None):
         return LayerNormFn.apply(x, norm.weight, norm.bias, norm.eps, out_dtype or self.dtype_,
-                                 self.sink())
+                                 self.sink(), handoff)
 
     def _linear(self, x, lin: nn.Linear, out_dtype=None):
         return LinearFn.apply(x, lin.weight, lin.bias, self.dtype_, out_dtype or self.dtype_,
                               self.sink(), self._lp)
 
-    def _blocks(self, blocks, x, heads, eps, taps=(), drop_scales=None):
+    def _blocks(self, blocks, x, heads, eps, taps=(), drop_scales=None, handoff=None):
         sink = self.sink()
         hook = None
         if sink.tracker is not None:
             blist = list(blocks)
             hook = lambda i: sink.note_done(_block_params(blist[i]))
         return run_blocks(blocks, x, heads, eps, self.dtype_, sink, taps=taps, lp=self._lp,
-                          on_block_grads=hook, drop_scales=drop_scales)
+                          on_block_grads=hook, drop_scales=drop_scales, handoff=handoff)
diff --git a/ssl4gie_amd/ops.py b/ssl4gie_amd/ops.py
--- a/ssl4gie_amd/ops.py
+++ b/ssl4gie_amd/ops.py
@@ -510,15 +510,23 @@
     return per_patch
 
 
-def mae_loss_bwd(pred, img, mask, p, norm_pix, gpp, gscale_host=1.0):
-    _dev(pred, img, mask, gpp)
+def mae_loss_bwd(pred, img, mask, p, norm_pix, gpp, gscale_host=1.0, out_dtype=torch.float32):
+    assert gpp is None or gpp.shape == mask.shape
+    gpp_stride = 1
+    if gpp is not None:
+        if gpp.numel() > 1 and all(s == 0 for s in gpp.stride()):
+            gpp_stride = 0
+        else:
+            gpp = gpp.contiguous()
+    _dev(pred, img, mask, gpp if gpp_stride else None)
     _f32(pred, img, mask, gpp)
-    assert gpp is None or gpp.shape == mask.shape
+    if gpp is not None and not gpp.is_cuda:
+        raise RuntimeError("ssl4gie_amd ops need tensors on the HIP device (no CPU fallback)")
     B, Cc, H, W, has_cls = _loss_geom(pred, img, mask, p)
-    dpred = torch.empty_like(pred)
-    _lib.check(_lib.load().ssl4gie_mae_loss(ptr(pred), ptr(img), ptr(mask), 0, ptr(dpred),
-                                            ptr(gpp), float(gscale_host), int(norm_pix), has_cls,
-                                            B, Cc, H, W, p, stream()), "mae_loss(bwd)")
+    dpred = torch.empty(pred.shape, dtype=out_dtype, device=pred.device)
+    _lib.check(_lib.load().ssl4gie_mae_loss_bwd(ptr(pred), ptr(img), ptr(mask), ptr(dpred), code(out_dtype),
+                                                ptr(gpp), gpp_stride, float(gscale_host), int(norm_pix), has_cls,
+                                                B, Cc, H, W, p, stream()), "mae_loss(bwd)")
     return dpred
 
 
diff --git a/ssl4gie_amd/optim.py b/ssl4gie_amd/optim.py
--- a/ssl4gie_amd/optim.py
+++ b/ssl4gie_amd/optim.py
@@ -193,6 +193,7 @@
         self._seen = {}
         self._hooked = False
         self._lp = None
+        self._pair = None
         self.last_grad_norm = self.last_found_inf = None
 
     def _state_buffers(self):
@@ -274,8 +275,16 @@
         assert self._tables_key == saved and group_of is not None
         return tuple(self._dev) + (n,)
 
+    def _launch_tiled(self, a, st):
+        start, lr, wd, mat, S = self._tables
+        lp, lpt, (off, rows, cols, ts, M, total, win, nwin) = self._pair
+        _lib.check(_lib.load().ssl4gie_adamw_arena_lp_tiled(
+            ptr(a.data), ptr(a.grad), ptr(self.exp_avg), ptr(self.exp_avg_sq), ptr(start), ptr(lr), ptr(wd), ptr(mat),
+            S, self.betas[0], self.betas[1], self.eps, self.step_count + 1, a.numel, ptr(lp), ptr(lpt), ptr(off),
+            ptr(rows), ptr(cols), ptr(ts), M, total, ptr(win), nwin, st), "adamw_arena_lp_tiled")
+
     def _step_ctl(self, a, clip_grad, skip_nonfinite):
-        start, lr, wd, _, S = self._tables
+        start, lr, wd, mat, S = self._tables
         dev = a.data.device
         if self._dev_steps is None:
             self._dev_steps = torch.full((1,), self._host_steps, dtype=torch.int32, device=dev)
@@ -291,6 +300,14 @@
                 self._ctl_plain = torch.zeros(4, device=dev)
                 self._ctl_plain[1] = 1.0
             ctl = self._ctl_plain
+        if self._pair is not None:
+            lp, lpt, (off, rows, cols, ts, M, total, win, nwin) = self._pair
+            _lib.check(_lib.load().ssl4gie_adamw_arena_lp_tiled_ctl(
+                ptr(a.data), ptr(a.grad), ptr(self.exp_avg), ptr(self.exp_avg_sq), ptr(start), ptr(lr), ptr(wd),
+                ptr(mat), S, self.betas[0], self.betas[1], self.eps, ptr(self._dev_steps), a.numel, ptr(lp), ptr(lpt),
+                ptr(off), ptr(rows), ptr(cols), ptr(ts), M, total, ptr(win), nwin, ptr(ctl), int(bool(skip_nonfinite)),
+                1, stream()), "adamw_arena_lp_tiled_ctl")
+            return
         _lib.check(_lib.load().ssl4gie_adamw_arena_range_ctl(
             ptr(a.data), ptr(a.grad), ptr(self.exp_avg), ptr(self.exp_avg_sq), ptr(start), ptr(lr), ptr(wd), S,
             self.betas[0], self.betas[1], self.eps, ptr(self._dev_steps), 0, a.numel, ptr(self._lp), ptr(ctl),
@@ -313,9 +330,13 @@
                                "changed between steps after part of this step was already applied")
         self._tables = tables
         self._lp = a.lp_flat_for_update() if a.data.is_cuda else None
+        self._pair = a.lp_pair_for_update() if (self._lp is not None and not self._overlap and not self._done) else None
         if ctl_path or self._dev_steps is not None:
             assert not self._done, "in-backward updates and the device-side step count do not mix"
             self._step_ctl(a, clip_grad, skip_nonfinite)
+        elif self._pair is not None:
+            self._launch_tiled(a, stream())
+            self.step_count += 1
         else:
             st = stream()
             pos = 0
@@ -328,8 +349,11 @@
             self.step_count += 1
         self._done, self._seen, self._tables = [], {}, None
         bump_weights_epoch(touched=[p for g in self.param_groups for p in g["params"]])
-        if self._lp is not None:
+        if self._pair is not None:
+            a.lp_pair_is_current()
+        elif self._lp is not None:
             a.lp_flat_is_current()
+        self._pair = None
 
 
 class ArenaLARS(_ArenaOptimizer):
```

Result: no change. 11980 images/sec (median of 2 runs) (+0.1%).
